# feiyuhuahuo/Yolact_minimal

Measured on AMD Instinct MI355X. Metric: img/s res101_coco 544x544 inference (bs=1/GPU, 4 requests in flight), higher is better.
Workload: dtype f32; 1 GPU; res101_coco 544x544 (the reference's "550-class" size) bs=1 inference: forward + nms + after_nms(480x640) per image, 4 independent bs=1 requests in flight on 4 HIP streams; global_batch=1, parallelism=replicas x1 (inference does not shard), weights=seeded random init, post_inputs=synthetic dense head outputs (17.8k candidates), requests_in_flight=4

## Files before the change

### include/yolact_hip.h

```cpp
#ifndef YOLACT_HIP_H
#define YOLACT_HIP_H

#include <stddef.h>
#include <stdint.h>

#ifdef __cplusplus
extern "C" {
#endif

#define YM_OK 0
#define YM_EINVAL (-1)
#define YM_ENOSPC (-2)
#define YM_ELAUNCH (-3)

#define YM_ACT_NONE 0
#define YM_ACT_RELU 1
#define YM_ACT_TANH 2
#define YM_ACT_GELU 3

typedef void* ym_stream_t;

int ym_abi_version(void);
const char* ym_last_error(void);


int ym_nchw_to_nhwc4(const float* in, float* out, int B, int C, int H, int W, ym_stream_t s);

int ym_pack_conv_weight(const float* w_oihw, float* w_packed, int Cout, int Cin, int KH, int KW,
                        int cin_pad, int k_pad, ym_stream_t s);

int ym_fold_bn(const float* gamma, const float* beta, const float* mean, const float* var, float eps,
               float* scale, float* shift, int C, ym_stream_t s);


typedef struct {
    int n_begin, n_end;
    float* out;
    int64_t batch_stride;
    int32_t pitch;
    int32_t act;
} ym_conv_seg;

typedef struct {
    const float* in;
    const float* weight;
    const float* scale;
    const float* shift;
    const float* residual;
    int32_t B, H, W, Cin, Cout, KH, KW, stride, pad, Ho, Wo, k_pad;
    int32_t nseg;
    ym_conv_seg seg[3];
    int32_t tile_m, tile_n;
    int32_t ksplit;
    int32_t kwaves;
    int32_t transposed;
    int32_t stages;
    double* bn_sum;
    double* bn_sumsq;
    int32_t* tile_counters;
    int32_t nlevels;
    int32_t level_h[5];
    int32_t level_w[5];
    int32_t tail_tiles;
    int32_t tail_ksplit;
    int32_t mma;
    int32_t bnb_relu;
    const float* bnb_y;
    const float* bnb_out;
    const float* bnb_mean;
    const float* bnb_invstd;
    const float* bnb_gamma;
    const float* bnb_beta;
    int32_t grid_wgs;
    int32_t bn_ordered;
} ym_conv_desc;

size_t ym_sizeof_conv_desc(void);
size_t ym_conv2d_workspace_bytes(const ym_conv_desc* d);
int ym_conv2d_tile_counters(const ym_conv_desc* d);
int ym_conv2d_fuses_bn_stats(const ym_conv_desc* d);
int ym_conv2d_effective_plan(const ym_conv_desc* d, int32_t out[8]);
int ym_conv2d_bn_partial_rows(const ym_conv_desc* d);
int ym_bn_partials_finish(const void* part, int rows, int C, void* sums, ym_stream_t s);
int64_t ym_unordered_sum_launches(void);
int ym_conv2d_fwd(const ym_conv_desc* d, void* workspace, size_t workspace_bytes, ym_stream_t s);

size_t ym_layernorm_bwd_workspace_bytes(int C);
int ym_layernorm_bwd(const float* dy, const float* x, const float* gamma, float eps, int64_t M, int C, float* dx, float* dgamma,
                     float* dbeta, void* workspace, size_t workspace_bytes, ym_stream_t s);
int ym_patch_merge_layernorm_bwd(const float* dy, const float* x, int B, int H, int W, int C, const float* gamma, float eps,
                                 float* dx, float* dgamma, float* dbeta, void* workspace, size_t workspace_bytes, ym_stream_t s);
int ym_drop_path_add(const float* res, const float* y, const float* rnd, float keep, float* out, int B, int64_t per_sample,
                     ym_stream_t s);
int ym_drop_path_bwd(const float* dout, const float* rnd, float keep, float* dy, int B, int64_t per_sample, ym_stream_t s);
int ym_gelu_fwd(const float* z, float* out, int64_t n, ym_stream_t s);
int ym_gelu_bwd(const float* dy, const float* z, float* dz, int64_t n, ym_stream_t s);
int ym_swin_window_attention_bwd(const float* qkv, const float* qkv_bias, const float* rel_bias_table, const float* dout, int B,
                                 int H, int W, int C, int heads, int window, int shift, float* dqkv, float* dqkv_bias_pad,
                                 float* dtable, ym_stream_t s);
int ym_adamw_step(float* param, const float* grad, float* exp_avg, float* exp_avg_sq, int64_t n, float lr, float beta1,
                  float beta2, float eps, float weight_decay, int step, ym_stream_t s);

typedef struct {
    int32_t H, W, mirror, cx, cy, cw, ch, q, px, py, r, S, final_mode, fx, fy, has_brightness, has_contrast;
    float brightness, contrast, saturation, hue, mean[3], std[3];
} ym_aug_plan;
int ym_train_aug_image(const void* img_hwc_bgr, int is_u8, const ym_aug_plan* plan, float* out_chw, ym_stream_t s);
int ym_train_aug_masks(const void* masks, int is_u8, const int32_t* keep, int k, const ym_aug_plan* plan, float* out,
                       ym_stream_t s);

size_t ym_mask_iou_workspace_bytes(int n, int g, int64_t P);
int ym_mask_iou(const float* masks_a, int n, const float* masks_b, int g, int64_t P, float* iou, void* workspace,
                size_t workspace_bytes, ym_stream_t s);
int ym_box_iou(const float* boxes_a, int n, const float* boxes_b, int g, float* iou, ym_stream_t s);
int ym_match_detections(const float* iou_box, const float* iou_mask, const int32_t* pred_cls, const int32_t* gt_cls, int n,
                        int g, const double* thresholds, int T, int num_classes, uint8_t* matched, ym_stream_t s);

int ym_rle_encode(const float* masks, int n, int H, int W, uint32_t* counts, int cap_runs, int32_t* nruns, uint8_t* str,
                  int cap_str, int32_t* str_len, void* workspace, size_t workspace_bytes, ym_stream_t s);

size_t ym_ann_to_mask_workspace_bytes(int n, int H, int W);
int ym_poly_to_mask(const double* xy, const int32_t* poly_off, const int32_t* ann_off, int n, int H, int W, uint8_t* masks,
                    void* workspace, size_t workspace_bytes, ym_stream_t s);
int ym_runs_to_mask(const uint32_t* counts, const int32_t* run_off, int n, int H, int W, uint8_t* masks, void* workspace,
                    size_t workspace_bytes, ym_stream_t s);


int ym_pack_conv_weight_dgrad(const float* w_oihw, float* w_packed, int Cout, int Cin, int KH, int KW, int cout_pad,
                              ym_stream_t s);

typedef struct {
    const float* src;
    float* dst;
    int32_t cout, cin, kh, kw, pad_a, pad_b, rows, kind;
    uint32_t first_chunk;
    uint32_t reserved;
} ym_pack_item;
int ym_pack_conv_weights_batch(const ym_pack_item* items_dev, int n_items, int total_chunks, ym_stream_t s);

typedef struct {
    const float* x;
    const float* dy;
    float* dw;
    int32_t B, H, W, Cin, Cin_real, Cout, Cout_real, KH, KW, stride, pad, Ho, Wo;
    int32_t msplit;
    int32_t accumulate;
    int32_t row_end[2];
    float* dw_seg[2];
    int32_t lds_buffers;
} ym_wgrad_desc;
size_t ym_conv2d_wgrad_workspace_bytes(const ym_wgrad_desc* d);
int ym_conv2d_wgrad(const ym_wgrad_desc* d, void* workspace, size_t workspace_bytes, ym_stream_t s);
typedef struct {
    const float* slabs;
    float* dw;
    uint32_t first_block;
    uint32_t blocks;
    uint32_t plan[14];
} ym_wgrad_reduce_item;
int ym_conv2d_wgrad_slabs(const ym_wgrad_desc* d, void* workspace, size_t workspace_bytes, ym_wgrad_reduce_item* item, ym_stream_t s);
int ym_wgrad_reduce_batch(const ym_wgrad_reduce_item* items_dev, int n_items, uint32_t total_blocks, ym_stream_t s);

size_t ym_bn_train_fwd_workspace_bytes(int64_t M, int C);
int ym_bn_train_fwd(const float* y, int64_t M, int C, const float* gamma, const float* beta, float eps, float momentum,
                    float* running_mean, float* running_var, const float* residual, int relu, float* out,
                    float* save_mean, float* save_invstd, void* workspace, size_t workspace_bytes, ym_stream_t s);
int ym_bn_train_fwd_stats(const float* y, int64_t M, int C, const float* gamma, const float* beta, float eps,
                          float momentum, float* running_mean, float* running_var, const float* residual, int relu,
                          float* out, float* save_mean, float* save_invstd, const void* stats, ym_stream_t s);

size_t ym_bn_train_bwd_workspace_bytes(int64_t M, int C);
int ym_bn_train_bwd(const float* dout, const float* out, const float* y, int64_t M, int C, const float* gamma,
                    const float* beta, const float* save_mean, const float* save_invstd, int relu, float* dy, float* dres,
                    float* dgamma, float* dbeta, void* workspace, size_t workspace_bytes, ym_stream_t s);

int ym_bn_train_bwd_apply(const float* dout, const float* out, const float* y, int64_t M, int C, const float* gamma,
                          const float* beta, const float* save_mean, const float* save_invstd, int relu, float* dy, float* dres,
                          float* dgamma, float* dbeta, const void* stats, ym_stream_t s);

int ym_head_grad_gather(const float* dclass, const float* dbox, const float* dcoef, const float* coef, int B, int N, int nc, int cd,
                        int na, int nlev, const int32_t* lev_row, const int32_t* lev_anchor, int pitch, const float* g_scale,
                        float* dz, ym_stream_t s);
int ym_scatter3(const float* src, float* d0, int n0, float* d1, int n1, float* d2, int n2, int accumulate, ym_stream_t s);

int ym_act_bias_bwd(const float* dy, const float* y, int64_t M, int C, int act, float* dz, float* dbias, void* workspace,
                    size_t workspace_bytes, ym_stream_t s);

size_t ym_mask_loss_workspace_bytes(void);
int ym_mask_loss_fwd_bwd(const float* proto, const float* coef_pos, const float* box_pos, const int32_t* gt_idx,
                         const float* gt_masks_ds, const int64_t* anchor_idx, int n, int Hp, int Wp, float wscale, float gscale,
                         double* loss_accum, float* dproto, float* dcoef_full, void* workspace, size_t workspace_bytes,
                         ym_stream_t s);
typedef struct {
    const float* proto;
    const float* coef_full;
    const float* anchor_box;
    const int64_t* anchor_gt;
    const float* gt_masks_ds;
    const int64_t* anchor_idx;
    int32_t n;
    float wscale;
    const int32_t* n_dev;
    float* dproto;
    float* dcoef_full;
} ym_mask_loss_item;
size_t ym_mask_loss_batch_workspace_bytes(int B);
int ym_mask_loss_batch(const ym_mask_loss_item* items, int B, int Hp, int Wp, float gscale, const int32_t* total_pos_dev,
                       double* loss_accum, void* workspace, size_t workspace_bytes, ym_stream_t s);

int ym_match_anchors(const float* gt_boxes_cls, int g, const float* anchors, int N, float pos_thre, float neg_thre,
                     float* offsets, int64_t* conf, float* anchor_box, int64_t* anchor_gt, void* workspace,
                     size_t workspace_bytes, ym_stream_t s);

int ym_match_anchors_batch(const float* const* gt_boxes_cls, const int32_t* g, int B, const float* anchors, int N, float pos_thre,
                           float neg_thre, float* offsets, int64_t* conf, float* anchor_box, int64_t* anchor_gt, void* workspace,
                           size_t workspace_bytes, ym_stream_t s);

size_t ym_loss_workspace_bytes(int B, int N);
int ym_class_box_loss(const float* class_p, const float* box_p, const float* offsets, const int64_t* conf, int B, int N, int C,
                      float conf_alpha, float bbox_alpha, int neg_pos_ratio, float* dclass, float* dbox, int32_t* num_pos,
                      double* loss_c, double* loss_b, void* workspace, size_t workspace_bytes, ym_stream_t s);

int ym_select_positives(const int64_t* conf, const float* keys, int B, int N, int cap, const int32_t* num_pos, int64_t* idx,
                        ym_stream_t s);

int ym_semantic_loss(const float* seg_nhwc, int P, int pitch, int num_classes, const float* gt_masks_ds, const int64_t* gt_cls,
                     int gt_cls_stride, int g, float coeff, float* dseg, double* loss_accum, ym_stream_t s);
int ym_semantic_loss_batch(const float* seg_nhwc, int B, int P, int pitch, int num_classes, const float* const* gt_masks_ds,
                           const int64_t* const* gt_cls, int gt_cls_stride, const int32_t* g, float coeff, float* dseg,
                           double* loss_accum, ym_stream_t s);

int ym_maxpool3x3s2_bwd(const float* x, const float* dy, float* dx, int B, int H, int W, int C, ym_stream_t s);
int ym_maxpool3x3s2_fwd_idx(const float* in, float* out, uint8_t* idx, int B, int H, int W, int C, ym_stream_t s);
int ym_maxpool3x3s2_bwd_idx(const uint8_t* idx, const float* dy, float* dx, int B, int H, int W, int C, ym_stream_t s);
int ym_bilinear2x_bwd(const float* dy, float* dx, int B, int H, int W, int C, int align_corners, ym_stream_t s);

int ym_sgd_step(float* param, const float* grad, float* momentum_buf, int64_t n, float lr, float momentum,
                float weight_decay, int first_step, ym_stream_t s);


int ym_maxpool3x3s2_fwd(const float* in, float* out, int B, int H, int W, int C, ym_stream_t s);
int ym_stem_conv_bn_relu_maxpool(const float* img_nchw, const float* w_packed, const float* scale, const float* shift, float* out,
                                 int B, int H, int W, int k_pad, ym_stream_t s);

int ym_bilinear2x_fwd(const float* in, float* out, int B, int H, int W, int C, int align_corners, ym_stream_t s);

int ym_softmax_rows(const float* in, float* out, int64_t rows, int C, ym_stream_t s);


int ym_layernorm(const float* x, const float* gamma, const float* beta, float eps, float* out, int64_t M, int C,
                 ym_stream_t s);

int ym_patch_merge_layernorm(const float* x, int B, int H, int W, int C, const float* gamma, const float* beta, float eps,
                             float* out, ym_stream_t s);

int ym_swin_window_attention(const float* qkv, const float* qkv_bias, const float* rel_bias_table, int B, int H, int W, int C,
                             int heads, int window, int shift, float* out, ym_stream_t s);


int ym_val_preprocess(const void* img_hwc_bgr, int is_uint8, int H, int W, int S, const float* mean_bgr,
                      const float* std_bgr, float* out_chw_rgb, ym_stream_t s);


typedef struct {
    int32_t num_anchors;
    int32_t num_classes;
    int32_t coef_dim;
    int32_t top_k;
    int32_t max_det;
    float score_thre;
    float iou_thre;
    float img_size;
} ym_nms_cfg;

size_t ym_nms_workspace_bytes(const ym_nms_cfg* cfg);

int ym_detect_fast_nms(const float* class_pred, const float* box_pred, const float* coef_pred,
                       const float* anchors, const ym_nms_cfg* cfg, int32_t* out_count, int64_t* out_ids,
                       float* out_scores, float* out_boxes, float* out_coefs, void* workspace,
                       size_t workspace_bytes, ym_stream_t s);

size_t ym_nms_batch_workspace_bytes(const ym_nms_cfg* cfg, int B);
int ym_detect_fast_nms_batch(const float* class_pred, const float* box_pred, const float* coef_pred, const float* anchors,
                             const ym_nms_cfg* cfg, int B, int32_t* out_count, int64_t* out_ids, float* out_scores,
                             float* out_boxes, float* out_coefs, void* workspace, size_t workspace_bytes, ym_stream_t s);

int ym_detect_greedy_nms(const float* class_pred, const float* box_pred, const float* coef_pred,
                         const float* anchors, const ym_nms_cfg* cfg, int32_t* out_count, int64_t* out_ids,
                         float* out_scores, float* out_boxes, float* out_coefs, void* workspace,
                         size_t workspace_bytes, ym_stream_t s);

size_t ym_greedy_nms_batch_workspace_bytes(const ym_nms_cfg* cfg, int B);
int ym_detect_greedy_nms_batch(const float* class_pred, const float* box_pred, const float* coef_pred, const float* anchors,
                               const ym_nms_cfg* cfg, int B, int32_t* out_count, int64_t* out_ids, float* out_scores,
                               float* out_boxes, float* out_coefs, void* workspace, size_t workspace_bytes, ym_stream_t s);

int ym_expf_cr(const float* x, float* y, int64_t n, ym_stream_t s);

size_t ym_greedy_nms_workspace_bytes(int n);
int ym_greedy_nms(const float* dets, int n, float thresh, uint8_t* keep_mask, int32_t* out_count,
                  void* workspace, size_t workspace_bytes, ym_stream_t s);

int ym_mask_assemble(const float* proto, const float* coefs, const float* boxes, int n, int Hp, int Wp,
                     int K, int do_crop, float* out, ym_stream_t s);

int ym_mask_resize_binarize(const float* masks, int n, int Hp, int Wp, int img_h, int img_w, float* out,
                            ym_stream_t s);

int ym_boxes_to_pixels(float* boxes_f, int32_t* boxes_px, int n, float S, ym_stream_t s);

size_t ym_after_nms_batch_workspace_bytes(int max_det, int Hp, int Wp, int img_h, int img_w);
int ym_after_nms_batch(const float* proto, const float* coefs, float* boxes, const int32_t* counts, int B, int max_det, int Hp,
                       int Wp, int K, int img_h, int img_w, int do_crop, float* masks, int32_t* boxes_px, void* workspace,
                       size_t workspace_bytes, ym_stream_t s);

#define YM_DRAW_HIDE_MASK 1
#define YM_DRAW_HIDE_BBOX 2
#define YM_DRAW_HIDE_SCORE 4
#define YM_DRAW_REAL_TIME 8
#define YM_DRAW_FONT_ADVANCE 12
#define YM_DRAW_FONT_HEIGHT 14
#define YM_DRAW_NAME_STRIDE 40
#define YM_DRAW_LABEL_MAX 44
#define YM_DRAW_MAX_DET 512
size_t ym_draw_workspace_bytes(int B, int max_det);
int ym_draw_detections_batch(const uint8_t* img, const float* masks, const int64_t* ids, const float* scores, const int32_t* boxes_px,
                             const int32_t* counts, int B, int max_det, int H, int W, const uint8_t* palette, int palette_n,
                             int num_classes, const char* names, int num_names, const uint16_t* font, int flags, float visual_thre,
                             const char* fps_text, uint8_t* out, uint8_t* cutout_total, void* workspace, size_t workspace_bytes,
                             ym_stream_t s);

int ym_draw_cutout_objects(const uint8_t* img, const float* masks, int n, int H, int W, uint8_t* out, ym_stream_t s);


int ym_after_nms_batch_packed(const float* proto, const float* coefs, float* boxes, const int32_t* counts, int B, int max_det, int Hp,
                              int Wp, int K, int img_h, int img_w, int do_crop, uint64_t* mask_bits, int32_t* boxes_px,
                              void* workspace, size_t workspace_bytes, ym_stream_t s);
int ym_pack_masks(const void* masks, int is_u8, int n, int H, int W, uint64_t* bits, ym_stream_t s);
int ym_unpack_masks(const uint64_t* bits, int n, int H, int W, float* masks, ym_stream_t s);

#define YM_RAGGED_MAX_IMAGES 32
#define YM_RAGGED_ALIGN_BYTES 256
typedef struct ym_ragged_image {
    int32_t img_h, img_w;
    int64_t offset;
} ym_ragged_image;
size_t ym_after_nms_ragged_workspace_bytes(const ym_ragged_image* images, int B, int max_det, int Hp, int Wp);
int ym_after_nms_ragged(const float* proto, const float* coefs, float* boxes, const int32_t* counts, int B, int max_det, int Hp,
                        int Wp, int K, const ym_ragged_image* images, int do_crop, float* masks, int32_t* boxes_px, void* workspace,
                        size_t workspace_bytes, ym_stream_t s);
int ym_after_nms_ragged_packed(const float* proto, const float* coefs, float* boxes, const int32_t* counts, int B, int max_det, int Hp,
                               int Wp, int K, const ym_ragged_image* images, int do_crop, uint64_t* mask_bits, int32_t* boxes_px,
                               void* workspace, size_t workspace_bytes, ym_stream_t s);

size_t ym_mask_iou_packed_workspace_bytes(int n, int g, int64_t words);
int ym_mask_iou_packed(const uint64_t* bits_a, int n, const uint64_t* bits_b, int g, int64_t words, float* iou, void* workspace,
                       size_t workspace_bytes, ym_stream_t s);
int ym_rle_encode_packed(const uint64_t* bits, int n, int H, int W, uint32_t* counts, int cap_runs, int32_t* nruns, uint8_t* str,
                         int cap_str, int32_t* str_len, void* workspace, size_t workspace_bytes, ym_stream_t s);
int ym_draw_detections_batch_packed(const uint8_t* img, const uint64_t* mask_bits, const int64_t* ids, const float* scores,
                                    const int32_t* boxes_px, const int32_t* counts, int B, int max_det, int H, int W,
                                    const uint8_t* palette, int palette_n, int num_classes, const char* names, int num_names,
                                    const uint16_t* font, int flags, float visual_thre, const char* fps_text, uint8_t* out,
                                    uint8_t* cutout_total, void* workspace, size_t workspace_bytes, ym_stream_t s);
int ym_draw_cutout_objects_packed(const uint8_t* img, const uint64_t* mask_bits, int n, int H, int W, uint8_t* out, ym_stream_t s);

#define YM_EVAL_MAX_DET 1024
#define YM_EVAL_MAX_THRESHOLDS 16
#define YM_EVAL_AP_ROWS_PER_PASS 1024
int ym_eval_match_log(const int64_t* ids, const float* scores, const int32_t* count, int n, const float* iou_box,
                      const float* iou_mask, const float* gt, int g, const double* thresholds, int T, int num_classes,
                      float* log_score, int32_t* log_class, uint32_t* log_flags, int64_t log_offset, int64_t* gt_count,
                      int32_t* class_rows, ym_stream_t s);
size_t ym_eval_ap_workspace_bytes(int64_t rows);
int ym_eval_ap(const uint32_t* log_flags, const int64_t* order, int64_t rows, const int64_t* seg, const int64_t* gt_count, int T,
               int num_classes, double* ap, uint8_t* empty, void* workspace, size_t workspace_bytes, ym_stream_t s);

#define YM_COCO_MAX_GT 512
#define YM_COCO_AREAS 4
#define YM_COCO_WORDS_PER_ROW 8
#define YM_COCO_ROWS_PER_PASS 1024
int ym_coco_iou_box(const double* dt_xywh, int n, const double* gt_xywh, int g, const uint8_t* iscrowd, double* iou, ym_stream_t s);
int ym_coco_iou_mask_packed(const uint64_t* bits_d, int n, const uint64_t* bits_g, int g, int64_t words, const uint8_t* iscrowd,
                            double* iou, int32_t* area_d, ym_stream_t s);
// ... 17 lines not shown
```

### yolact_minimal_amd/csrc/conv_common.h

```cpp
#pragma once
#include <cstdlib>
#include "ym_common.h"

namespace ymk {

constexpr int BK = 32;

struct FastDiv {
    unsigned mg, sh, d;
    __host__ static FastDiv make(unsigned d) {
        if (d == 0) d = 1;
        unsigned s = 0;
        while ((1ull << s) < d) ++s;
        return FastDiv{(unsigned)(((1ull << 32) * ((1ull << s) - d)) / d + 1), s, d};
    }
    __device__ __forceinline__ unsigned div(unsigned x) const { return (__umulhi(x, mg) + x) >> sh; }
    __device__ __forceinline__ void divmod(unsigned x, unsigned& q, unsigned& r) const { q = div(x); r = x - q * d; }
};

typedef int i32x4_t __attribute__((ext_vector_type(4)));
constexpr unsigned OOB = 0xFFFFFFF0u;
__device__ __forceinline__ f32x4 buf_ld16(__amdgpu_buffer_rsrc_t r, unsigned byte_off) {
    return __builtin_bit_cast(f32x4, __builtin_amdgcn_raw_buffer_load_b128(r, (int)byte_off, 0, 0));
}
__device__ __forceinline__ f32x4 buf_ld16_s(__amdgpu_buffer_rsrc_t r, unsigned byte_off, int soffset) {
    return __builtin_bit_cast(f32x4, __builtin_amdgcn_raw_buffer_load_b128(r, (int)byte_off, soffset, 0));
}
template <int I> struct IC { static constexpr int value = I; };
template <int I, int N, class F>
__device__ __forceinline__ void static_for(F&& f) {
    if constexpr (I < N) { f(IC<I>{}); static_for<I + 1, N>(f); }
}
constexpr int AUX_SC1 = 16;
__device__ __forceinline__ f32x4 buf_ld16_sc1(__amdgpu_buffer_rsrc_t r, unsigned byte_off) {
    return __builtin_bit_cast(f32x4, __builtin_amdgcn_raw_buffer_load_b128(r, (int)byte_off, 0, AUX_SC1));
}
__device__ __forceinline__ void buf_st16_sc1(__amdgpu_buffer_rsrc_t r, unsigned byte_off, f32x4 v) {
    __builtin_amdgcn_raw_buffer_store_b128(__builtin_bit_cast(i32x4_t, v), r, (int)byte_off, 0, AUX_SC1);
}

struct SegDev {
    float* out;
    long long bstride;
    int n0, n1, pitch, act;
};

struct ConvP {
    const float* in;
    const float* w;
    const float* scale;
    const float* shift;
    const float* residual;
    float* ws;
    double* bn_sum;
    double* bn_sumsq;
    const float* bnb_y;
    const float* bnb_out;
    const float* bnb_mean;
    const float* bnb_invstd;
    const float* bnb_gamma;
    const float* bnb_beta;
    int bnb_relu;
    int bn_ordered;
    int* counters;
    int B, H, W, Cin, Cout, KH, KW, stride, pad, Ho, Wo, Kpad;
    int M, HoWo, nkt, ksplit, kt_per_split, tiles_m, tiles_n;
    int main_blocks, main_tiles, tail_split, tail_ktps;
    FastDiv fd_ksplit, fd_tail, fd_tiles_n, fd_howo, fd_wo, fd_cin, fd_kw;
    int nlev;
    int lev_h[5], lev_w[5], lev_m[6], lev_pix[6];
    int cls;
    int M_pix;
    int cls_tile0[5];
    int cls_rows[4];
    int cls_w[4];
    FastDiv cls_fd_hw[4], cls_fd_w[4];
    int cls_kh0[4], cls_kw0[4], cls_nkw[4];
    int cls_nkt[4], cls_ktps[4], cls_tail_ktps[4];
    int n_groups;
    FastDiv fd_grp, fd_gn, fd_gn_last;
    long long* trace;
    const int* trace_epoch;
    int trace_ring;
    int trace_stride;
    int trace_rt;
    int* trace_hw;
    unsigned in_bytes, w_bytes, ws_bytes;
    int total_items;
    int nseg;
    int vec;
    SegDev seg[3];
};

__device__ __forceinline__ void ym_tile_decode(const ConvP& p, int id, int& tile_m, int& tile_n) {
    const unsigned g = p.fd_grp.div((unsigned)id);
    const unsigned r = (unsigned)id - g * p.fd_grp.d;
    const bool last = (int)g == p.n_groups - 1;
    const unsigned w = last ? p.fd_gn_last.d : p.fd_gn.d;
    const unsigned tm = last ? p.fd_gn_last.div(r) : p.fd_gn.div(r);
    tile_m = (int)tm;
    tile_n = (int)(g * p.fd_gn.d + (r - tm * w));
}

inline void ym_set_tile_order(ConvP& p, int groups, bool allow_model) {
    const int tn = p.tiles_n > 0 ? p.tiles_n : 1, tm = p.tiles_m > 0 ? p.tiles_m : 1;
    static const char* env = getenv("YM_TILE_GROUPS");
    if (groups <= 0) {
        const double a = (double)p.in_bytes, w = (double)p.w_bytes;
        if (env && env[0] == 'l') groups = (allow_model && w > a) ? tn : 1;
        else if (env && atoi(env) > 0) groups = allow_model ? atoi(env) : 1;
        else {
            groups = 1;
            double best = a + 8.0 * w;
            const bool small = a + w <= 8.0 * 1024 * 1024;
            if (allow_model && !small && w > a) groups = tn;
            for (int g = 2; g <= 8 && allow_model && small; g *= 2) {
                if (tn < g) break;
                const double t = g * a + (8.0 / g) * w;
                if (t < 0.95 * best) { best = t; groups = g; }
            }
        }
    }
    if (groups > tn) groups = tn;
    const int gw = (tn + groups - 1) / groups;
    p.n_groups = (tn + gw - 1) / gw;
    p.fd_gn = FastDiv::make((unsigned)gw);
    p.fd_gn_last = FastDiv::make((unsigned)(tn - (p.n_groups - 1) * gw));
    p.fd_grp = FastDiv::make((unsigned)(tm * gw));
}

#ifdef YM_TRACE
__device__ __forceinline__ size_t ym_trace_region(const ConvP& p) {
    if (!p.trace_epoch) return 0;
    const unsigned e = (unsigned)__hip_atomic_load(p.trace_epoch, __ATOMIC_RELAXED, __HIP_MEMORY_SCOPE_AGENT);
    return (size_t)(e % (unsigned)p.trace_ring) * (p.trace_stride ? (unsigned)p.trace_stride : gridDim.x);
}
#define YM_STAMP(i) do { if ((i) == 3) __builtin_amdgcn_s_waitcnt(0); if (p.trace && threadIdx.x == 0) { const size_t reg_ = ym_trace_region(p); p.trace[(reg_ + blockIdx.x) * 4 + (i)] = (long long)((p.trace_epoch || p.trace_rt) ? __builtin_amdgcn_s_memrealtime() : __builtin_amdgcn_s_memtime()) | ((i) == 0 ? (long long)(__builtin_amdgcn_s_getreg(0x1814) & 15) << 60 : 0ll); if ((i) == 0 && p.trace_hw) p.trace_hw[reg_ + blockIdx.x] = (int)__builtin_amdgcn_s_getreg(0xF804); } } while (0)
#else
#define YM_STAMP(i) do { } while (0)
#endif


__device__ __forceinline__ void row_to_image_pixel(const ConvP& p, int m, int& b, int& pix) {
    if (p.nlev > 0) {
        int base = 0, hw = p.lev_h[0] * p.lev_w[0], pix0 = 0;
#pragma unroll
        for (int q = 1; q < 5; ++q)
            if (q < p.nlev && m >= p.lev_m[q]) { base = p.lev_m[q]; hw = p.lev_h[q] * p.lev_w[q]; pix0 = p.lev_pix[q]; }
        const int local = m - base;
        b = local / hw;
        pix = pix0 + (local - b * hw);
    } else {
        b = (int)p.fd_howo.div((unsigned)m);
        pix = m - b * p.HoWo;
    }
}

__device__ __forceinline__ void epilogue_store(const ConvP& p, int m, int n, float acc) {
    float v = acc;
    v = __builtin_fmaf(v, p.scale ? p.scale[n] : 1.f, p.shift ? p.shift[n] : 0.f);
    if (p.residual) v += p.residual[(size_t)m * p.Cout + n];
    int b, pix;
    row_to_image_pixel(p, m, b, pix);
#pragma unroll
    for (int s = 0; s < 3; ++s) {
        if (s < p.nseg && n >= p.seg[s].n0 && n < p.seg[s].n1) {
            const SegDev& g = p.seg[s];
            g.out[(size_t)b * g.bstride + (size_t)pix * g.pitch + (n - g.n0)] = ym_apply_act(v, g.act);
        }
    }
}


enum ConvFamily { CONV_IGEMM, CONV_WAVE, CONV_WAVE_DMA, CONV_WS, CONV_PERS };
struct Plan {
    int bm, bn, ksplit, kt_per_split, tiles_m, tiles_n, nkt, M;
    int tail_tiles, tail_split, tail_ktps;
    int cls, M_pix, cls_tile0[5], cls_rows[4], cls_w[4], cls_hw[4], cls_kh0[4], cls_kw0[4], cls_nkw[4], cls_nkt[4];
    int kwaves;
    int family;
    int ring = 2;
    int mode = 0, spl = 0;
    bool dl = false, pf = false, pyramid = false;
    int grid_wgs;
    int pers_grid;
    bool pers_defer;
    bool vec, counters, fuses_bn;
    int bn_rows;
    int slots() const { return tail_tiles > 0 && tail_split > ksplit ? tail_split : ksplit; }
    size_t ws_bytes(int cout) const {
        const size_t u = ksplit > 1 ? (size_t)ksplit * M * cout * sizeof(float) : 0;
        const size_t t = tail_tiles > 0 ? (size_t)tail_tiles * tail_split * bm * bn * sizeof(float) : 0;
        return u > t ? u : t;
    }
    int grid() const { return (tiles_m * tiles_n - tail_tiles) * ksplit + tail_tiles * (tail_tiles > 0 ? tail_split : 0); }
    int stages() const {
        return ring + (family == CONV_PERS ? 40 : family == CONV_WS ? 50 : family == CONV_WAVE_DMA ? 20 : dl ? (pf ? 30 : 20) : 0);
    }
};

}

int ym_conv_plan(const ym_conv_desc* d, bool ws_aligned, ymk::Plan* pl);
int ym_cu_count();
int ym_launch_conv_wave(const ymk::ConvP& p, int tm, int tn, int kwaves, int ring, int waves_per_block, hipStream_t st);
int ym_launch_conv_pers(const ymk::ConvP& p, int bm, int bn, int mode, int ns, bool defer, int grid, hipStream_t st);
size_t ym_conv_pers_lds_bytes(int bm, int bn, int ns, bool defer);
int ym_launch_conv_ws(const ymk::ConvP& p, int bm, int bn, int nstg, int grid_wgs, hipStream_t st);
int ym_conv_ws_partial_rows(int M, int Cout, int bm, int bn, int nkt, int nstg, int grid_wgs);
size_t ym_conv_ws_lds_bytes(int bm, int bn, int nkt, int nstg);
```

### yolact_minimal_amd/csrc/conv_mfma.hip

```cpp
#include <stdlib.h>
#include <type_traits>
#include "conv_common.h"

using namespace ymk;

namespace {

constexpr int PITCH = 36;

template <int BM, int BN, int MODE, int NS, bool DL = false, bool PF = false, bool RG = false, int SPL = 0>
__global__ __launch_bounds__(256) void conv_igemm_f32(const ConvP p) {
    static_assert(SPL == 0 || (SPL <= 3 && !DL && !PF && (NS == 2 || NS == 3) && MODE != 1), "split-bf16: register staging, Cin % 32 == 0");
    constexpr int LB = SPL ? 2 : NS;
    constexpr int TM = BM / 64, TN = BN / 64;
    constexpr int AR = BM / 32, BR = BN / 32;
    constexpr int BP = 40;
    constexpr int RP = SPL ? (SPL * BP) / 2 : (DL ? 32 : PITCH);
    extern __shared__ __attribute__((aligned(16))) float smem[];
    float* As = smem;
    float* Bs = smem + LB * BM * RP;

    const int tid = threadIdx.x;
    const int lane = tid & 63, wave = __builtin_amdgcn_readfirstlane(tid >> 6);
    const int wm = wave >> 1, wn = wave & 1;
// ... 513 lines not shown
                        const f32x4 v = *reinterpret_cast<const f32x4*>(C + row * CP + col4 * 4);
                        if (fused) buf_st16_sc1(rs_ws, base + (unsigned)row * rs, v);
                        else *reinterpret_cast<f32x4*>(p.ws + (size_t)ks * slice + n + (size_t)m * p.Cout) = v;
                    }
                }
            }
            if (!fused) return;
            int& s_last = *reinterpret_cast<int*>(smem);
            asm volatile("s_waitcnt vmcnt(0)" ::: "memory");
            __syncthreads();
            if (tid == 0) {
                int* cnt = p.counters + tile_m * p.tiles_n + tile_n;
                const int old = __hip_atomic_fetch_add(cnt, 1, __ATOMIC_RELAXED, __HIP_MEMORY_SCOPE_AGENT);
                s_last = old == nks - 1;
                if (s_last) __hip_atomic_store(cnt, 0, __ATOMIC_RELAXED, __HIP_MEMORY_SCOPE_AGENT);
            }
            __syncthreads();
            if (!s_last) { YM_STAMP(3); return; }
        }
        if (n < p.Cout) {
            f32x4 sc = pre_sc, sh = pre_sh;
            if (!direct) {
                if (p.scale) sc = *reinterpret_cast<const f32x4*>(p.scale + n);
                if (p.shift) sh = *reinterpret_cast<const f32x4*>(p.shift + n);
            }
            const int act = p.seg[0].act;
            float* outb = p.seg[0].out + n;
            const bool fwd_stats = p.bn_sum != nullptr && p.bnb_y == nullptr;
            const float* resb = (p.residual && !(direct && PRE_RES)) ? p.residual + n : nullptr;
#pragma unroll
            for (int rk = 0; rk < BM / RPP; ++rk) {
                const int row = row0 + rk * RPP;
                const int m = out_row(row);
                if (m >= 0) {
                    f32x4 v;
                    if (nks > 1) {
                        const unsigned off = ws0 + (unsigned)row * rs;
                        v = buf_ld16_sc1(rs_ws, off);
                        int s2 = 1;
                        for (; s2 + 3 < nks; s2 += 4) {
                            const f32x4 a = buf_ld16_sc1(rs_ws, off + (unsigned)s2 * sb), b = buf_ld16_sc1(rs_ws, off + (unsigned)(s2 + 1) * sb);
                            const f32x4 c = buf_ld16_sc1(rs_ws, off + (unsigned)(s2 + 2) * sb), d = buf_ld16_sc1(rs_ws, off + (unsigned)(s2 + 3) * sb);
                            v += a; v += b; v += c; v += d;
                        }
                        for (; s2 < nks; ++s2) v += buf_ld16_sc1(rs_ws, off + (unsigned)s2 * sb);
                    } else if (epi_abl) {
                        v = f32x4{acc[0][0][(4 * rk) & 15], acc[0][0][(4 * rk + 1) & 15], acc[0][0][(4 * rk + 2) & 15], acc[0][0][(4 * rk + 3) & 15]};
                    } else {
                        v = *reinterpret_cast<const f32x4*>(C + row * CP + col4 * 4);
                    }
                    v = __builtin_elementwise_fma(v, sc, sh);
                    if (direct && PRE_RES) v += pre_res[PRE_RES ? rk : 0];
                    else if (resb) v += *reinterpret_cast<const f32x4*>(resb + (size_t)m * p.Cout);
#pragma unroll
                    for (int e = 0; e < 4; ++e) v[e] = ym_apply_act(v[e], act);
                    *reinterpret_cast<f32x4*>(outb + (size_t)m * p.Cout) = v;
                    if (fwd_stats) {
#pragma unroll
                        for (int e = 0; e < 4; ++e) { const double dv = v[e]; bsum[e] += dv; bsq[e] += dv * dv; }
                    }
                }
            }
            if (p.bnb_y) {
                const f32x4 b_mu = *reinterpret_cast<const f32x4*>(p.bnb_mean + n), b_is = *reinterpret_cast<const f32x4*>(p.bnb_invstd + n);
                f32x4 b_g = {1.f, 1.f, 1.f, 1.f}, b_bt = {0.f, 0.f, 0.f, 0.f};
                const bool remask = p.bnb_relu && !p.bnb_out;
                if (remask) { b_g = *reinterpret_cast<const f32x4*>(p.bnb_gamma + n); b_bt = *reinterpret_cast<const f32x4*>(p.bnb_beta + n); }
                constexpr int NR = BM / RPP, UR = 2;
#pragma unroll 1
                for (int rk0 = 0; rk0 < NR; rk0 += UR) {
                    f32x4 dv[UR], yy[UR], o[UR];
                    int mrow[UR];
#pragma unroll
                    for (int u = 0; u < UR; ++u) {
                        const int m = mrow[u] = out_row(row0 + (rk0 + u) * RPP);
                        const size_t off = (size_t)(m >= 0 ? m : 0) * p.Cout + n;
                        dv[u] = *reinterpret_cast<const f32x4*>(p.seg[0].out + off);
                        yy[u] = *reinterpret_cast<const f32x4*>(p.bnb_y + off);
                        if (p.bnb_out) o[u] = *reinterpret_cast<const f32x4*>(p.bnb_out + off);
                    }
#pragma unroll
                    for (int u = 0; u < UR; ++u) {
                        if (mrow[u] < 0) continue;
                        if (!p.bnb_out) {
#pragma unroll
                            for (int e = 0; e < 4; ++e) o[u][e] = remask ? bn_affine(yy[u][e], b_mu[e], b_is[e], b_g[e], b_bt[e]) : 1.f;
                        }
#pragma unroll
                        for (int e = 0; e < 4; ++e) {
                            const double dd = o[u][e] > 0.f ? dv[u][e] : 0.f;
                            bsum[e] += dd;
                            bsq[e] += dd * (double)((yy[u][e] - b_mu[e]) * b_is[e]);
                        }
                    }
                }
            }
        }
        if (p.bn_sum) {
            __syncthreads();
            double* R = reinterpret_cast<double*>(smem);
#pragma unroll
            for (int e = 0; e < 4; ++e) {
                R[((row0 * BN) + col4 * 4 + e) * 2 + 0] = bsum[e];
                R[((row0 * BN) + col4 * 4 + e) * 2 + 1] = bsq[e];
            }
            __syncthreads();
            if (tid < BN && n0 + tid < p.Cout) {
                double S = 0.0, Q = 0.0;
#pragma unroll
                for (int r = 0; r < RPP; ++r) { S += R[(r * BN + tid) * 2]; Q += R[(r * BN + tid) * 2 + 1]; }
                if (p.bn_ordered) {
                    double* row = p.bn_sum + (size_t)tile_m * 2 * p.Cout;
                    row[n0 + tid] = S;
                    row[p.Cout + n0 + tid] = Q;
                } else {
                    atomicAdd(p.bn_sum + n0 + tid, S);
                    atomicAdd(p.bn_sumsq + n0 + tid, Q);
                }
            }
        }
        YM_STAMP(3);
        return;
    }
    int* rowinfo = reinterpret_cast<int*>(smem);
    __syncthreads();
    if (tid < BM) {
        int b = 0, pix = 0;
        if (m0 + tid < p.M) row_to_image_pixel(p, m0 + tid, b, pix);
        rowinfo[2 * tid] = b;
        rowinfo[2 * tid + 1] = pix;
    }
    __syncthreads();
#pragma unroll
    for (int j = 0; j < TN; ++j) {
        const int n = n0 + wn * (BN / 2) + j * 32 + frag_row;
        const bool n_ok = n < p.Cout;
        float sc = 1.f, sh = 0.f;
        float* optr = nullptr;
        long long obs = 0;
        int opitch = 0, oact = 0;
        if (n_ok) {
            if (p.scale) sc = p.scale[n];
            if (p.shift) sh = p.shift[n];
#pragma unroll
            for (int s = 0; s < 3; ++s) {
                if (s < p.nseg && n >= p.seg[s].n0 && n < p.seg[s].n1) {
                    optr = p.seg[s].out + (n - p.seg[s].n0);
                    obs = p.seg[s].bstride; opitch = p.seg[s].pitch; oact = p.seg[s].act;
                }
            }
        }
#pragma unroll
        for (int i = 0; i < TM; ++i) {
            const int mb = m0 + wm * (BM / 2) + i * 32 + 4 * khalf;
            if (p.ksplit > 1) {
#pragma unroll
                for (int r = 0; r < 16; ++r) {
                    const int m = mb + (r & 3) + 8 * (r >> 2);
                    if (n_ok && m < p.M) p.ws[((size_t)ks * p.M + m) * p.Cout + n] = acc[i][j][r];
                }
            } else if (optr) {
#pragma unroll
                for (int r = 0; r < 16; ++r) {
                    const int m = mb + (r & 3) + 8 * (r >> 2);
                    if (m < p.M) {
                        float v = __builtin_fmaf(acc[i][j][r], sc, sh);
                        if (p.residual) v += p.residual[(size_t)m * p.Cout + n];
                        const int row = m - m0;
                        optr[(size_t)rowinfo[2 * row] * obs + (size_t)rowinfo[2 * row + 1] * opitch] = ym_apply_act(v, oact);
                    }
                }
            }
            __builtin_amdgcn_sched_barrier(0);
        }
    }
}

__global__ __launch_bounds__(256) void conv_splitk_reduce(const ConvP p) {
    const size_t total = (size_t)p.M * p.Cout;
    if (p.vec) {
        const size_t total4 = total / 4;
        const int act = p.seg[0].act;
        for (size_t q = (size_t)blockIdx.x * 256 + threadIdx.x; q < total4; q += (size_t)gridDim.x * 256) {
            const size_t e = q * 4;
            f32x4 v = *reinterpret_cast<const f32x4*>(p.ws + e);
            for (int s = 1; s < p.ksplit; ++s) v += *reinterpret_cast<const f32x4*>(p.ws + (size_t)s * total + e);
            const int n = (int)(e % p.Cout);
            f32x4 sc = {1.f, 1.f, 1.f, 1.f}, sh = {0.f, 0.f, 0.f, 0.f};
            if (p.scale) sc = *reinterpret_cast<const f32x4*>(p.scale + n);
            if (p.shift) sh = *reinterpret_cast<const f32x4*>(p.shift + n);
            v = __builtin_elementwise_fma(v, sc, sh);
            if (p.residual) v += *reinterpret_cast<const f32x4*>(p.residual + e);
#pragma unroll
            for (int k = 0; k < 4; ++k) v[k] = ym_apply_act(v[k], act);
            *reinterpret_cast<f32x4*>(p.seg[0].out + e) = v;
        }
        return;
    }
    for (size_t e = (size_t)blockIdx.x * 256 + threadIdx.x; e < total; e += (size_t)gridDim.x * 256) {
        float v = 0.f;
        for (int s = 0; s < p.ksplit; ++s) v += p.ws[(size_t)s * total + e];
        const int m = (int)(e / p.Cout), n = (int)(e - (size_t)m * p.Cout);
        epilogue_store(p, m, n, v);
    }
}

template <int BM, int BN, int MODE, int NS = 2, bool DL = false, bool PF = false, bool RG = false, int SPL = 0>
void launch(const ConvP& p, int grid, hipStream_t st) {
    size_t lds = SPL ? (size_t)2 * (BM + BN) * SPL * 80 : (size_t)NS * (BM + BN) * (DL ? 32 : PITCH) * sizeof(float);
    const size_t epi = (size_t)BM * (BN + 4) * sizeof(float);
    if (lds < epi) lds = epi;
    static YmLdsAttr attr = {};
    (void)ym_ensure_dyn_lds(attr, reinterpret_cast<const void*>(conv_igemm_f32<BM, BN, MODE, NS, DL, PF, RG, SPL>), lds, "conv_igemm_f32");
    hipLaunchKernelGGL((conv_igemm_f32<BM, BN, MODE, NS, DL, PF, RG, SPL>), dim3(grid), dim3(256), lds, st, p);
}

bool launch_igemm(const ConvP& p, const Plan& pl, int grid, hipStream_t st) {
#define YM_V(BM_, BN_, MODE_, NS_, DL_, PF_, RG_, SPL_)                                                                               \
    if (pl.bm == BM_ && pl.bn == BN_ && pl.mode == MODE_ && pl.ring == NS_ && pl.dl == DL_ && pl.pf == PF_ && pl.pyramid == RG_ && \
        pl.spl == SPL_) { launch<BM_, BN_, MODE_, NS_, DL_, PF_, RG_, SPL_>(p, grid, st); return true; }
    YM_V(128, 128, 0, 2, 0, 0, 0, 0)
    YM_V(128, 128, 0, 2, 1, 0, 0, 0)
    YM_V(128, 128, 0, 3, 1, 0, 0, 0)
    YM_V(128,  64, 0, 2, 0, 0, 0, 0)
    YM_V(128,  64, 0, 3, 0, 0, 0, 0)
    YM_V(128,  64, 0, 2, 1, 0, 0, 0)
    YM_V(128,  64, 0, 3, 1, 0, 0, 0)
    YM_V( 64, 128, 0, 2, 0, 0, 0, 0)
    YM_V( 64, 128, 0, 3, 0, 0, 0, 0)
    YM_V( 64, 128, 0, 2, 1, 0, 0, 0)
    YM_V( 64, 128, 0, 3, 1, 0, 0, 0)
    YM_V( 64,  64, 0, 2, 0, 0, 0, 0)
    YM_V( 64,  64, 0, 3, 0, 0, 0, 0)
    YM_V( 64,  64, 0, 2, 1, 0, 0, 0)
    YM_V( 64,  64, 0, 3, 1, 0, 0, 0)
    YM_V( 64,  64, 0, 4, 1, 0, 0, 0)
    YM_V( 64,  64, 0, 3, 1, 1, 0, 0)
    YM_V( 64,  64, 0, 4, 1, 1, 0, 0)
    YM_V(128, 128, 2, 2, 0, 0, 0, 0)
    YM_V(128, 128, 2, 2, 1, 0, 0, 0)
    YM_V(128, 128, 2, 3, 1, 0, 0, 0)
    YM_V(128,  64, 2, 2, 0, 0, 0, 0)
    YM_V(128,  64, 2, 2, 1, 0, 0, 0)
    YM_V(128,  64, 2, 3, 1, 0, 0, 0)
    YM_V( 64, 128, 2, 2, 0, 0, 0, 0)
    YM_V( 64, 128, 2, 2, 1, 0, 0, 0)
    YM_V( 64, 128, 2, 3, 1, 0, 0, 0)
    YM_V( 64,  64, 2, 2, 0, 0, 0, 0)
    YM_V( 64,  64, 2, 3, 0, 0, 0, 0)
    YM_V( 64,  64, 2, 2, 1, 0, 0, 0)
    YM_V( 64,  64, 2, 3, 1, 0, 0, 0)
    YM_V(128,  64, 1, 2, 0, 0, 0, 0)
    YM_V(128, 128, 0, 2, 0, 0, 1, 0)
    YM_V(128,  64, 0, 2, 0, 0, 1, 0)
    YM_V( 64, 128, 0, 2, 0, 0, 1, 0)
    YM_V( 64,  64, 0, 2, 0, 0, 1, 0)
    YM_V(128, 128, 0, 2, 0, 0, 0, 2)
    YM_V(128, 128, 0, 3, 0, 0, 0, 2)
    YM_V(128,  64, 0, 2, 0, 0, 0, 2)
    YM_V(128,  64, 0, 3, 0, 0, 0, 2)
    YM_V( 64, 128, 0, 2, 0, 0, 0, 2)
    YM_V( 64, 128, 0, 3, 0, 0, 0, 2)
    YM_V( 64,  64, 0, 2, 0, 0, 0, 2)
    YM_V( 64,  64, 0, 3, 0, 0, 0, 2)
    YM_V(128, 128, 0, 2, 0, 0, 0, 3)
    YM_V(128, 128, 0, 3, 0, 0, 0, 3)
    YM_V(128,  64, 0, 2, 0, 0, 0, 3)
    YM_V(128,  64, 0, 3, 0, 0, 0, 3)
    YM_V( 64, 128, 0, 2, 0, 0, 0, 3)
    YM_V( 64, 128, 0, 3, 0, 0, 0, 3)
    YM_V( 64,  64, 0, 2, 0, 0, 0, 3)
    YM_V( 64,  64, 0, 3, 0, 0, 0, 3)
    YM_V(128, 128, 2, 2, 0, 0, 0, 2)
    YM_V(128, 128, 2, 3, 0, 0, 0, 2)
    YM_V(128,  64, 2, 2, 0, 0, 0, 2)
    YM_V(128,  64, 2, 3, 0, 0, 0, 2)
    YM_V( 64, 128, 2, 2, 0, 0, 0, 2)
    YM_V( 64, 128, 2, 3, 0, 0, 0, 2)
    YM_V( 64,  64, 2, 2, 0, 0, 0, 2)
    YM_V( 64,  64, 2, 3, 0, 0, 0, 2)
    YM_V(128, 128, 2, 2, 0, 0, 0, 3)
    YM_V(128, 128, 2, 3, 0, 0, 0, 3)
    YM_V(128,  64, 2, 2, 0, 0, 0, 3)
    YM_V(128,  64, 2, 3, 0, 0, 0, 3)
    YM_V( 64, 128, 2, 2, 0, 0, 0, 3)
    YM_V( 64, 128, 2, 3, 0, 0, 0, 3)
    YM_V( 64,  64, 2, 2, 0, 0, 0, 3)
    YM_V( 64,  64, 2, 3, 0, 0, 0, 3)
#undef YM_V
    return false;
}

int fill_params(const ym_conv_desc* d, const Plan& pl, void* workspace, ConvP& p) {
    const size_t need = pl.ws_bytes(d->Cout);
    p.in = d->in; p.w = d->weight; p.scale = d->scale; p.shift = d->shift; p.residual = d->residual;
    p.ws = (float*)workspace;
    p.B = d->B; p.H = d->H; p.W = d->W; p.Cin = d->Cin; p.Cout = d->Cout; p.KH = d->KH; p.KW = d->KW;
    p.stride = d->stride; p.pad = d->pad; p.Ho = d->Ho; p.Wo = d->Wo; p.Kpad = d->k_pad;
    {
        const unsigned long long ib = (d->nlevels ? (unsigned long long)pl.M : (unsigned long long)d->B * d->H * d->W) * d->Cin * 4ull, wb = (unsigned long long)d->Cout * d->k_pad * 4ull;
        YM_REQUIRE(ib < 0xFFFFFFF0ull && wb < 0x7FFFFFF0ull, "conv: input must be < 4 GiB and the packed weight < 2 GiB (32-bit buffer offsets)");
        p.in_bytes = (unsigned)ib; p.w_bytes = (unsigned)wb;
    }
    p.nlev = d->nlevels;
    {
        int m_acc = 0, pix_acc = 0;
        for (int l = 0; l < 5; ++l) {
            const bool on = l < d->nlevels;
            p.lev_h[l] = on ? d->level_h[l] : 1; p.lev_w[l] = on ? d->level_w[l] : 1;
            p.lev_m[l] = m_acc; p.lev_pix[l] = pix_acc;
            if (on) { m_acc += d->B * d->level_h[l] * d->level_w[l]; pix_acc += d->level_h[l] * d->level_w[l]; }
        }
        p.lev_m[5] = m_acc; p.lev_pix[5] = pix_acc;
    }
    p.M = pl.M; p.HoWo = d->Ho * d->Wo; p.nkt = pl.nkt; p.ksplit = pl.ksplit; p.kt_per_split = pl.kt_per_split;
    p.M_pix = pl.M_pix; p.cls = pl.cls;
    for (int c = 0; c < 4; ++c) {
        const bool on = pl.cls != 0;
        p.cls_tile0[c] = on ? pl.cls_tile0[c] : 0; p.cls_rows[c] = on ? pl.cls_rows[c] : 0; p.cls_w[c] = on ? pl.cls_w[c] : 1;
        p.cls_fd_hw[c] = FastDiv::make((unsigned)(on ? pl.cls_hw[c] : 1)); p.cls_fd_w[c] = FastDiv::make((unsigned)(on ? pl.cls_w[c] : 1));
        p.cls_kh0[c] = on ? pl.cls_kh0[c] : 0; p.cls_kw0[c] = on ? pl.cls_kw0[c] : 0; p.cls_nkw[c] = on ? pl.cls_nkw[c] : 1;
        p.cls_nkt[c] = on ? pl.cls_nkt[c] : 0;
        p.cls_ktps[c] = on ? ym_cdiv(pl.cls_nkt[c], pl.ksplit) : 0;
        p.cls_tail_ktps[c] = on && pl.tail_tiles > 0 ? ym_cdiv(pl.cls_nkt[c], pl.tail_split) : 0;
    }
    p.cls_tile0[4] = pl.cls ? pl.cls_tile0[4] : 0;
    p.tiles_m = pl.tiles_m; p.tiles_n = pl.tiles_n; p.nseg = d->nseg;
    for (int i = 0; i < 3; ++i) {
        if (i < d->nseg) {
            p.seg[i].out = d->seg[i].out; p.seg[i].bstride = d->seg[i].batch_stride; p.seg[i].n0 = d->seg[i].n_begin;
            p.seg[i].n1 = d->seg[i].n_end; p.seg[i].pitch = d->seg[i].pitch; p.seg[i].act = d->seg[i].act;
        } else {
            p.seg[i] = SegDev{nullptr, 0, 0, 0, 0, 0};
        }
    }
    YM_REQUIRE(pl.tail_tiles == 0 || ((uintptr_t)workspace & 15) == 0, "conv: tail split needs a 16-byte aligned workspace");
    p.vec = pl.vec;
    p.bn_sum = d->bn_sum; p.bn_sumsq = d->bn_sumsq; p.bn_ordered = (d->bn_sum && d->bn_ordered) ? 1 : 0;
    p.bnb_y = d->bnb_y; p.bnb_out = d->bnb_out; p.bnb_mean = d->bnb_mean; p.bnb_invstd = d->bnb_invstd;
    p.bnb_gamma = d->bnb_gamma; p.bnb_beta = d->bnb_beta; p.bnb_relu = d->bnb_relu;
    p.trace = nullptr; p.trace_epoch = nullptr; p.trace_ring = 0; p.trace_stride = 0; p.trace_rt = 0; p.trace_hw = nullptr;
#ifdef YM_TRACE
    if (const char* e = getenv("YM_TRACE_PTR")) p.trace = (long long*)strtoull(e, nullptr, 10);
    if (const char* e = getenv("YM_TRACE_EPOCH_PTR")) p.trace_epoch = (const int*)strtoull(e, nullptr, 10);
    if (const char* e = getenv("YM_TRACE_RING")) p.trace_ring = atoi(e);
    if (const char* e = getenv("YM_TRACE_GRID")) p.trace_stride = atoi(e);
    if (const char* e = getenv("YM_TRACE_REALTIME")) p.trace_rt = atoi(e);
    if (const char* e = getenv("YM_TRACE_HW_PTR")) p.trace_hw = (int*)strtoull(e, nullptr, 10);
    if (p.trace_ring <= 0) p.trace_epoch = nullptr;
    if (const char* e = getenv("YM_PERS_ABL")) { if (!d->bn_sum) p.bnb_relu = atoi(e); }
#endif
    p.counters = pl.counters ? d->tile_counters : nullptr;
    YM_REQUIRE(!pl.cls || (p.vec && (pl.slots() == 1 || p.counters)), "conv(dgrad, stride 2): the class-ordered plan needs a 16-byte aligned workspace");
    YM_REQUIRE(pl.tail_tiles == 0 || p.counters, "conv: tail_tiles needs a plain NHWC output (vector epilogue) and a workspace < 4 GiB");
    p.main_tiles = pl.tiles_m * pl.tiles_n - pl.tail_tiles;
    p.main_blocks = p.main_tiles * pl.ksplit;
    p.tail_split = pl.tail_tiles > 0 ? pl.tail_split : 1;
    p.tail_ktps = pl.tail_tiles > 0 ? pl.tail_ktps : pl.nkt;
    p.fd_ksplit = FastDiv::make((unsigned)pl.ksplit); p.fd_tail = FastDiv::make((unsigned)p.tail_split);
    p.fd_tiles_n = FastDiv::make((unsigned)pl.tiles_n);
    ym_set_tile_order(p, 0, pl.tail_tiles == 0);
    p.fd_howo = FastDiv::make((unsigned)(d->Ho * d->Wo));
    p.fd_wo = FastDiv::make((unsigned)d->Wo); p.fd_cin = FastDiv::make((unsigned)d->Cin); p.fd_kw = FastDiv::make((unsigned)d->KW);
    p.ws_bytes = (unsigned)(need < 0xFFFFFFF0ull ? need : 0);
    p.total_items = pl.grid();
    if (d->bn_sum) {
        YM_REQUIRE((d->bn_sumsq || d->bn_ordered) && ((uintptr_t)d->bn_sum & 7) == 0 && pl.fuses_bn,
                   "conv: bn_sum given but this configuration cannot fuse the statistics (ask ym_conv2d_fuses_bn_stats)");
    }
    if (d->bnb_y) {
        YM_REQUIRE(d->bn_sum && d->bnb_mean && d->bnb_invstd && (!d->bnb_relu || d->bnb_out || (d->bnb_gamma && d->bnb_beta)),
                   "conv: bnb_y needs bn_sum / bn_sumsq, bnb_mean, bnb_invstd and (with bnb_relu) bnb_out or bnb_gamma + bnb_beta");
        YM_REQUIRE(d->Cout % 4 == 0 && ((uintptr_t)d->bnb_y & 15) == 0 && ((uintptr_t)d->bnb_out & 15) == 0,
                   "conv: bnb_y / bnb_out must be 16-byte aligned [M][Cout] tensors");
    }
    YM_REQUIRE(pl.family != CONV_WAVE_DMA || (size_t)pl.M * d->Cout * 4 < 0xFFFFFFF0ull, "conv(wave, DMA ring): the output must be < 4 GiB");
    if (pl.family == CONV_IGEMM && d->mma != 0) {
        YM_REQUIRE(d->mma == 3 || d->mma == 6, "conv: mma must be 0 (f32 MFMA), 3 (bf16x3) or 6 (bf16x6), got %d", d->mma);
        YM_REQUIRE(d->nlevels == 0 && d->Cin % 32 == 0, "conv: split-bf16 mode needs Cin %% 32 == 0 and a single-size input");
    }
    return YM_OK;
}

int launch_plan(const ConvP& p, const Plan& pl, hipStream_t st) {
    switch (pl.family) {
        case CONV_WAVE: case CONV_WAVE_DMA: return ym_launch_conv_wave(p, pl.bm, pl.bn, pl.kwaves, pl.ring, pl.grid_wgs, st);
        case CONV_WS: return ym_launch_conv_ws(p, pl.bm, pl.bn, pl.ring, pl.grid_wgs, st);
        case CONV_PERS: return ym_launch_conv_pers(p, pl.bm, pl.bn, pl.mode, pl.ring, pl.pers_defer, pl.pers_grid, st);
    }
    if (!launch_igemm(p, pl, pl.grid(), st)) {
        ym_set_error("conv: no conv_igemm_f32<%d, %d, %d, %d, %d, %d, %d, %d> is built (planner bug)", pl.bm, pl.bn, pl.mode, pl.ring, pl.dl, pl.pf, pl.pyramid, pl.spl);
        return YM_EINVAL;
    }
    int rc = ym_check_launch("conv_igemm_f32");
    if (rc == YM_OK && pl.ksplit > 1 && !p.counters) {
        const size_t total = (size_t)p.M * p.Cout;
        int rgrid = (int)((total / (p.vec ? 4 : 1) + 255) / 256);
        if (rgrid > 2048) rgrid = 2048;
        hipLaunchKernelGGL(conv_splitk_reduce, dim3(rgrid), dim3(256), 0, st, p);
        rc = ym_check_launch("conv_splitk_reduce");
    }
    return rc;
}

}

extern "C" size_t ym_sizeof_conv_desc(void) { return sizeof(ym_conv_desc); }

extern "C" size_t ym_conv2d_workspace_bytes(const ym_conv_desc* d) {
    Plan pl;
    return ym_conv_plan(d, true, &pl) == YM_OK ? pl.ws_bytes(d->Cout) : 0;
}

extern "C" int ym_conv2d_tile_counters(const ym_conv_desc* d) {
    Plan pl;
    return ym_conv_plan(d, true, &pl) == YM_OK && pl.slots() > 1 ? pl.tiles_m * pl.tiles_n : 0;
}

extern "C" int ym_conv2d_fuses_bn_stats(const ym_conv_desc* d) {
    Plan pl;
    return ym_conv_plan(d, true, &pl) == YM_OK && pl.fuses_bn ? 1 : 0;
}

extern "C" int ym_conv2d_bn_partial_rows(const ym_conv_desc* d) {
    Plan pl;
    return ym_conv_plan(d, true, &pl) == YM_OK ? pl.bn_rows : 0;
}

extern "C" int ym_conv2d_effective_plan(const ym_conv_desc* d, int32_t out[8]) {
    Plan pl;
    YM_REQUIRE(out, "conv: effective_plan needs an output row");
    if (int rc = ym_conv_plan(d, true, &pl)) return rc;
    const bool tail = pl.tail_tiles > 0;
    const int32_t row[8] = {pl.bm, pl.bn, pl.ksplit, d->kwaves, pl.stages(), tail ? pl.tail_tiles : 0, tail ? pl.tail_split : 0, pl.grid_wgs};
    for (int i = 0; i < 8; ++i) out[i] = row[i];
    return YM_OK;
}

extern "C" int ym_conv2d_fwd(const ym_conv_desc* d, void* workspace, size_t workspace_bytes, ym_stream_t s) {
    Plan pl;
    if (int rc = ym_conv_plan(d, ((uintptr_t)workspace & 15) == 0, &pl)) return rc;
    const size_t need = pl.ws_bytes(d->Cout);
    if (need > workspace_bytes || (need && !workspace)) {
        ym_set_error("conv: workspace %zu B < %zu B needed (ksplit %d)", workspace_bytes, need, pl.ksplit);
        return YM_ENOSPC;
    }
    ConvP p;
    if (int rc = fill_params(d, pl, workspace, p)) return rc;
    if (d->bn_sum && !d->bn_ordered) ym_note_unordered_sum();
    return launch_plan(p, pl, (hipStream_t)s);
}
```

### yolact_minimal_amd/csrc/conv_planner.hip

```cpp
#include <stdlib.h>
#include "conv_common.h"

using namespace ymk;

int ym_cu_count() {
    static int cus = 0;
    if (cus == 0) {
        int dev = 0, n = 0;
        if (hipGetDevice(&dev) != hipSuccess || hipDeviceGetAttribute(&n, hipDeviceAttributeMultiprocessorCount, dev) != hipSuccess || n <= 0) n = 256;
        cus = n;
    }
    return cus;
}

namespace {

bool vec_epilogue(const ym_conv_desc* d) {
    const ym_conv_seg& g = d->seg[0];
    const bool aligned = (((uintptr_t)g.out | (uintptr_t)d->residual | (uintptr_t)d->scale | (uintptr_t)d->shift) & 15) == 0;
    const bool rows_in_order = d->nlevels ? g.batch_stride == 0
                                          : g.batch_stride == (int64_t)d->Ho * d->Wo * d->Cout;
    return d->nseg == 1 && g.n_begin == 0 && g.n_end == d->Cout && g.pitch == d->Cout && rows_in_order && d->Cout % 4 == 0 && aligned;
}

int plan_tiles(const ym_conv_desc* d, Plan* pl, bool allow_cls) {
    YM_REQUIRE(d && d->in && d->weight, "conv: null descriptor / pointer");
    YM_REQUIRE(d->B > 0 && d->H > 0 && d->W > 0 && d->Cout > 0, "conv: bad shape");
    YM_REQUIRE(d->Cin == 4 || d->Cin % 32 == 0, "conv: Cin must be 4 (stem) or a multiple of 32, got %d", d->Cin);
    YM_REQUIRE(d->k_pad % BK == 0 && d->k_pad >= d->KH * d->KW * d->Cin, "conv: k_pad %d invalid", d->k_pad);
    if (d->transposed) {
        YM_REQUIRE(d->stride == 1 || d->stride == 2, "conv(dgrad): stride must be 1 or 2");
        YM_REQUIRE(d->Cin % 32 == 0 && d->kwaves == 0, "conv(dgrad): dy channels must be padded to a multiple of 32; workgroup kernel only");
        YM_REQUIRE(d->H == (d->Ho + 2 * d->pad - d->KH) / d->stride + 1 && d->W == (d->Wo + 2 * d->pad - d->KW) / d->stride + 1,
                   "conv(dgrad): H/W (dy) inconsistent with Ho/Wo (dx)");
    } else if (d->nlevels == 0) {
        YM_REQUIRE(d->Ho == (d->H + 2 * d->pad - d->KH) / d->stride + 1 && d->Wo == (d->W + 2 * d->pad - d->KW) / d->stride + 1,
                   "conv: Ho/Wo inconsistent with H/W/K/stride/pad");
    }
    long long M_levels = 0;
    if (d->nlevels != 0) {
        YM_REQUIRE(d->nlevels >= 1 && d->nlevels <= 5, "conv: nlevels must be 0..5");
        YM_REQUIRE(!d->transposed && d->kwaves == 0 && d->Cin % 32 == 0 && d->stride == 1 && d->KH == d->KW && (d->KH & 1) &&
                   d->pad == d->KH / 2, "conv(pyramid): stride 1, odd square filter, pad = K/2, Cin %% 32 == 0, workgroup kernel");
        for (int l = 0; l < d->nlevels; ++l) {
            YM_REQUIRE(d->level_h[l] > 0 && d->level_w[l] > 0, "conv(pyramid): bad level %d", l);
            M_levels += (long long)d->B * d->level_h[l] * d->level_w[l];
        }
    }
    YM_REQUIRE(d->nseg >= 1 && d->nseg <= 3, "conv: nseg must be 1..3");
    for (int s = 0; s < d->nseg; ++s)
        YM_REQUIRE(d->seg[s].out && d->seg[s].n_end > d->seg[s].n_begin && d->seg[s].n_end <= d->Cout,
                   "conv: bad segment %d", s);
    const long long M = d->nlevels ? M_levels : (long long)d->B * d->Ho * d->Wo;
    YM_REQUIRE(M * (long long)d->Cout < (1ll << 31) && (d->nlevels ? M : (long long)d->B * d->H * d->W) * d->Cin < (1ll << 31) * 1ll,
               "conv: tensor too large for 32-bit indexing");
    pl->M = (int)M;
    pl->M_pix = (int)M;
    pl->cls = 0;
    pl->nkt = d->k_pad / BK;
    pl->tail_tiles = 0; pl->tail_split = 0; pl->tail_ktps = 0;
    int bm = d->tile_m, bn = d->tile_n;
    if (bm == 0 || bn == 0) {
        const int cand[3][2] = {{128, 128}, {128, 64}, {64, 64}};
        bm = 64; bn = 64;
        for (int c = 0; c < 3; ++c) {
            const long long wgs = (long long)ym_cdiv(pl->M, cand[c][0]) * ym_cdiv(d->Cout, cand[c][1]);
            if (wgs >= 512) { bm = cand[c][0]; bn = cand[c][1]; break; }
        }
        if (d->Cin == 4) { bm = 128; bn = 64; }
    }
    pl->family = CONV_IGEMM;
    if (d->stages >= 52 && d->stages <= 54) {
        const bool shape_ok = (bm == 64 && bn == 256) || (bm == 128 && bn == 128) || (bm == 256 && bn == 64);
        const int act = d->seg[0].act;
        const bool ok = shape_ok && d->KH == 1 && d->KW == 1 && d->stride == 1 && d->pad == 0 && d->Cin % 32 == 0 && d->k_pad == d->Cin &&
                        d->nlevels == 0 && d->kwaves == 0 && d->mma == 0 && d->bnb_y == nullptr && vec_epilogue(d) &&
                        (act == YM_ACT_NONE || act == YM_ACT_RELU) && (size_t)bn * d->Cin * 4 <= (64u << 10) &&
                        ym_conv_ws_lds_bytes(bm, bn, pl->nkt, d->stages - 50) <= (160u << 10) && (unsigned long long)M * d->Cout * 4ull < 0xFFFFFFF0ull &&
                        (unsigned long long)M * d->Cin * 4ull < 0xFFFFFFF0ull;
        if (ok) {
            pl->bm = bm; pl->bn = bn; pl->tiles_m = ym_cdiv(pl->M, bm); pl->tiles_n = ym_cdiv(d->Cout, bn);
            pl->ksplit = 1; pl->kt_per_split = pl->nkt;
            pl->family = CONV_WS; pl->ring = d->stages - 50;
            return YM_OK;
        }
        bm = 64; bn = 64;
    }
    if (d->kwaves > 0) {
        YM_REQUIRE(d->Cin != 4, "conv: the wave-private kernel does not support the stem (Cin == 4)");
        YM_REQUIRE((bm == 32 || bm == 64) && (bn == 32 || bn == 64), "conv(wave): tile must be 32/64, got %dx%d", bm, bn);
        const bool dma = d->stages >= 22 && d->stages <= 24;
        pl->family = dma ? CONV_WAVE_DMA : CONV_WAVE;
        pl->ring = dma ? d->stages - 20 : 0;
        pl->bm = bm; pl->bn = bn; pl->tiles_m = ym_cdiv(pl->M, bm); pl->tiles_n = ym_cdiv(d->Cout, bn);
        pl->ksplit = 1; pl->kt_per_split = pl->nkt;
        if (d->tail_tiles > 0 && d->tail_ksplit > 1 && dma && bm == 32 && bn == 32 && d->kwaves == 4 &&
            (d->grid_wgs == 0 || d->grid_wgs == 4) && d->tile_counters && vec_epilogue(d)) {
            YM_REQUIRE(d->tail_tiles <= pl->tiles_m * pl->tiles_n, "conv(wave): tail_tiles %d > %d output tiles", d->tail_tiles, pl->tiles_m * pl->tiles_n);
            int ts = d->tail_ksplit > pl->nkt ? pl->nkt : d->tail_ksplit;
            if (ts > 8) ts = 8;
            pl->tail_ktps = ym_cdiv(pl->nkt, ts);
            pl->tail_split = ym_cdiv(pl->nkt, pl->tail_ktps);
            pl->tail_tiles = pl->tail_split > 1 ? d->tail_tiles : 0;
        }
        return YM_OK;
    }
    YM_REQUIRE((bm == 128 || bm == 64) && (bn == 128 || bn == 64), "conv: tile must be 64/128");
    YM_REQUIRE(d->Cin != 4 || (bm == 128 && bn == 64), "conv: stem mode supports the 128x64 tile only");
    pl->bm = bm; pl->bn = bn;
    {
        static int on = -1;
        if (on < 0) { const char* e = getenv("YM_DGRAD_CLASSES"); on = e ? atoi(e) : 1; }
        if (on && allow_cls && d->transposed && d->stride == 2 && d->nlevels == 0 && vec_epilogue(d)) {
            int t0 = 0, nkt_max = 0, nt_max = 0;
            for (int c = 0; c < 4; ++c) {
                const int ph = c >> 1, pw = c & 1;
                const int hc = (d->Ho - ph + 1) / 2, wc = (d->Wo - pw + 1) / 2;
                const int kh0 = (ph + d->pad) & 1, kw0 = (pw + d->pad) & 1;
                const int nkh = kh0 < d->KH ? (d->KH - kh0 + 1) / 2 : 0, nkw = kw0 < d->KW ? (d->KW - kw0 + 1) / 2 : 0;
                pl->cls_tile0[c] = t0;
                pl->cls_rows[c] = d->B * hc * wc;
                pl->cls_w[c] = wc > 0 ? wc : 1;
                pl->cls_hw[c] = hc * wc > 0 ? hc * wc : 1;
                pl->cls_kh0[c] = kh0; pl->cls_kw0[c] = kw0; pl->cls_nkw[c] = nkw > 0 ? nkw : 1;
                pl->cls_nkt[c] = nkh * nkw * (d->Cin / BK);
                if (pl->cls_nkt[c] > nkt_max) nkt_max = pl->cls_nkt[c];
                t0 += ym_cdiv(pl->cls_rows[c], bm);
                if (ym_cdiv(pl->cls_rows[c], bm) > nt_max) nt_max = ym_cdiv(pl->cls_rows[c], bm);
            }
            pl->cls_tile0[4] = t0;
            pl->cls = 1;
            pl->M = 4 * nt_max * bm;
            pl->nkt = nkt_max > 0 ? nkt_max : 1;
        }
    }
    pl->tiles_m = ym_cdiv(pl->M, bm);
    pl->tiles_n = ym_cdiv(d->Cout, bn);
    int ks = d->ksplit;
    if (ks <= 0) {
        ks = 1;
        const int wgs = pl->tiles_m * pl->tiles_n;
        if (wgs < 256) {
            ks = ym_cdiv(512, wgs);
            const int max_ks = pl->nkt / 4 > 0 ? pl->nkt / 4 : 1;
            if (ks > max_ks) ks = max_ks;
            if (ks > 16) ks = 16;
        }
    }
    if (ks > pl->nkt) ks = pl->nkt;
    if (ks < 1) ks = 1;
    pl->kt_per_split = ym_cdiv(pl->nkt, ks);
    pl->ksplit = ym_cdiv(pl->nkt, pl->kt_per_split);
    if (d->tail_tiles > 0 && d->tail_ksplit > 1 && vec_epilogue(d)) {
        YM_REQUIRE(d->tile_counters && pl->ksplit == 1 && d->Cin != 4, "conv: tail_tiles needs tile_counters, ksplit <= 1 and Cin %% 32 == 0");
        YM_REQUIRE(d->tail_tiles <= pl->tiles_m * pl->tiles_n, "conv: tail_tiles %d > %d output tiles", d->tail_tiles, pl->tiles_m * pl->tiles_n);
        int ts = d->tail_ksplit > pl->nkt ? pl->nkt : d->tail_ksplit;
        pl->tail_ktps = ym_cdiv(pl->nkt, ts);
        pl->tail_split = ym_cdiv(pl->nkt, pl->tail_ktps);
        pl->tail_tiles = pl->tail_split > 1 ? d->tail_tiles : 0;
    }
    if (pl->cls && pl->slots() > 1 && (!d->tile_counters || pl->ws_bytes(d->Cout) >= 0xFFFFFFF0ull)) return plan_tiles(d, pl, false);
    return YM_OK;
}

void plan_variant(const ym_conv_desc* d, Plan* pl) {
    const bool t64 = pl->bm == 64 && pl->bn == 64;
    const int act = d->seg[0].act;
    int stages = d->stages;
    if (stages >= 52 && stages <= 54) stages = 22;
    if (stages >= 42 && stages <= 48) {
        const int ns = stages - 40;
        if (pl->vec && t64 && d->Cin % 32 == 0 && d->nlevels == 0 && d->mma == 0 && !pl->cls && (act == YM_ACT_NONE || act == YM_ACT_RELU) &&
            (pl->slots() == 1 || pl->counters) && d->bn_sum == nullptr && (ns == 2 || ns == 3 || ns == 4 || ns == 6 || ns == 8)) {
            static int defer = -1;
            if (defer < 0) { const char* e = getenv("YM_PERS_DEFER"); defer = e ? atoi(e) : 1; }
            int per_cu = (int)((160u << 10) / ym_conv_pers_lds_bytes(64, 64, ns, defer != 0));
            if (per_cu > 4) per_cu = 4;
            if (per_cu < 1) per_cu = 1;
            int g = d->grid_wgs > 0 ? d->grid_wgs : ym_cu_count() * per_cu;
            if (g > pl->grid()) g = pl->grid();
            if (g >= 8 && g < pl->grid()) g &= ~7;
            pl->family = CONV_PERS; pl->ring = ns; pl->pers_grid = g; pl->pers_defer = defer != 0;
            pl->mode = d->transposed ? 2 : 0;
            return;
        }
        stages = ns >= 4 && t64 && !d->transposed ? 24 : (ns == 2 ? 22 : 23);
    }
    pl->mode = d->transposed ? 2 : (d->Cin == 4 ? 1 : 0);
    pl->pyramid = d->nlevels > 0;
    if (d->mma != 0) {
        pl->spl = d->mma == 3 ? 2 : 3;
        pl->ring = stages == 3 ? 3 : 2;
    } else if (!pl->pyramid && pl->mode != 1) {
        const bool has3 = pl->mode == 0 ? !(pl->bm == 128 && pl->bn == 128) : t64;
        if (pl->mode == 0 && t64 && (stages == 24 || stages == 33 || stages == 34)) { pl->dl = true; pl->pf = stages > 30; pl->ring = stages % 10; }
        else if (stages == 22 || stages == 23) { pl->dl = true; pl->ring = stages - 20; }
        else if (stages == 3 && has3) pl->ring = 3;
    }
}

}

int ym_conv_plan(const ym_conv_desc* d, bool ws_aligned, Plan* pl) {
    *pl = Plan{};
    if (int rc = plan_tiles(d, pl, true)) return rc;
    pl->kwaves = d->kwaves;
    pl->vec = vec_epilogue(d) && ws_aligned;
    pl->counters = pl->vec && pl->slots() > 1 && (d->kwaves == 0 || pl->tail_tiles > 0) && pl->ws_bytes(d->Cout) < 0xFFFFFFF0ull && d->tile_counters;
    pl->fuses_bn = pl->vec && (pl->slots() == 1 || pl->counters) && d->kwaves == 0;
    if (pl->family == CONV_IGEMM) plan_variant(d, pl);
    pl->grid_wgs = pl->family == CONV_IGEMM || pl->family == CONV_WAVE ? 0 : d->grid_wgs;
    pl->bn_rows = !pl->fuses_bn ? 0 : pl->family != CONV_WS ? pl->tiles_m
                : ym_conv_ws_partial_rows(pl->M, d->Cout, pl->bm, pl->bn, pl->nkt, pl->ring, d->grid_wgs);
    return YM_OK;
}
```

### yolact_minimal_amd/csrc/conv_wave.hip

```cpp
#include "conv_common.h"

using namespace ymk;

namespace {

constexpr int waitcnt_vm(int vm) { return (vm & 15) | ((vm >> 4) << 14) | (7 << 4) | (15 << 8); }

template <int N>
struct Frag {
    f32x4 v[N][4];
};

template <int TM, int TN, int KW, int WPB>
__device__ __forceinline__ void wave_tile_finish(const ConvP& p, float* slabs, f32x16 (&acc)[TM][TN], int wave, int lane, bool tile_ok,
                                                 int tile_local, int kslice, int m0, int n0) {
    constexpr int WM = 32 * TM, WN = 32 * TN;
    constexpr int CP = WN + 4;
    const int frag_row = lane & 31, khalf = lane >> 5;
    constexpr int C4_ = WN / 4, LANES_ = KW * 64, NPASS = (WM * C4_ + LANES_ - 1) / LANES_;
    f32x4 pre_res[NPASS];
    const bool pre = p.vec && p.residual != nullptr && tile_ok;
    if (pre) {
        const int lt_ = kslice * 64 + lane, col4_ = lt_ % C4_, row0_ = lt_ / C4_;
        const __amdgpu_buffer_rsrc_t rs_res = __builtin_amdgcn_make_buffer_rsrc((void*)p.residual, 0, (unsigned)((size_t)p.M * p.Cout * 4), 0x00020000);
#pragma unroll
        for (int k = 0; k < NPASS; ++k) {
            const int m = m0 + row0_ + k * (LANES_ / C4_), n = n0 + col4_ * 4;
            pre_res[k] = buf_ld16(rs_res, (row0_ + k * (LANES_ / C4_) < WM && m < p.M && n < p.Cout) ? (unsigned)(((size_t)m * p.Cout + n) * 4) : OOB);
        }
    }
    float* mine = slabs + (size_t)wave * WM * CP;
#pragma unroll
    for (int j = 0; j < TN; ++j)
#pragma unroll
        for (int i = 0; i < TM; ++i)
#pragma unroll
            for (int r = 0; r < 16; ++r)
                mine[(i * 32 + 4 * khalf + (r & 3) + 8 * (r >> 2)) * CP + j * 32 + frag_row] = acc[i][j][r];
    __syncthreads();
    if (!tile_ok) return;
    const float* slab0 = slabs + (size_t)(tile_local * KW) * WM * CP;
    constexpr int C4 = WN / 4;
    constexpr int LANES = KW * 64;
    const int lt = kslice * 64 + lane;
    if (p.vec) {
        const int col4 = lt % C4, row0 = lt / C4;
        const int n = n0 + col4 * 4;
        if (n < p.Cout) {
            f32x4 sc = {1.f, 1.f, 1.f, 1.f}, sh = {0.f, 0.f, 0.f, 0.f};
            if (p.scale) sc = *reinterpret_cast<const f32x4*>(p.scale + n);
            if (p.shift) sh = *reinterpret_cast<const f32x4*>(p.shift + n);
            const int act = p.seg[0].act;
#pragma unroll
            for (int k = 0; k < NPASS; ++k) {
                const int row = row0 + k * (LANES / C4);
                const int m = m0 + row;
                if (row >= WM || m >= p.M) break;
                f32x4 v = *reinterpret_cast<const f32x4*>(slab0 + row * CP + col4 * 4);
#pragma unroll
                for (int s = 1; s < KW; ++s) v += *reinterpret_cast<const f32x4*>(slab0 + (size_t)s * WM * CP + row * CP + col4 * 4);
                v = __builtin_elementwise_fma(v, sc, sh);
                if (p.residual) v += pre_res[k];
#pragma unroll
                for (int e = 0; e < 4; ++e) v[e] = ym_apply_act(v[e], act);
                *reinterpret_cast<f32x4*>(p.seg[0].out + (size_t)m * p.Cout + n) = v;
            }
        }
    } else {
        for (int e = lt; e < WM * WN; e += LANES) {
            const int row = e / WN, col = e - row * WN;
            const int m = m0 + row, n = n0 + col;
            if (m < p.M && n < p.Cout) {
                float v = slab0[row * CP + col];
#pragma unroll
                for (int s = 1; s < KW; ++s) v += slab0[(size_t)s * WM * CP + row * CP + col];
                epilogue_store(p, m, n, v);
            }
        }
    }
}

template <int TM, int TN, int KW, int WPB>
__global__ __launch_bounds__(WPB * 64) void conv_wave_f32(const ConvP p) {
    constexpr int TPB = WPB / KW;
    constexpr int WM = 32 * TM, WN = 32 * TN;
    constexpr int D = 3;
    extern __shared__ __attribute__((aligned(16))) float smem[];

    const int lane = threadIdx.x & 63;
    const int wave = __builtin_amdgcn_readfirstlane(threadIdx.x >> 6);
    const int tile_local = wave / KW, kslice = wave - tile_local * KW;
    const int frag_row = lane & 31, khalf = lane >> 5;

    const int bid = ym_xcd_remap(blockIdx.x, gridDim.x);
    const int tile = bid * TPB + tile_local;
    const int ntiles = p.tiles_m * p.tiles_n;
    const bool tile_ok = tile < ntiles;
    const int tile_m = tile_ok ? tile / p.tiles_n : 0, tile_n = tile_ok ? tile - tile_m * p.tiles_n : 0;
    const int m0 = tile_m * WM, n0 = tile_n * WN;

    int a_pix[TM], a_ih0[TM], a_iw0[TM];
#pragma unroll
    for (int i = 0; i < TM; ++i) {
        const int m = m0 + i * 32 + frag_row;
        if (tile_ok && m < p.M) {
            const int b = m / p.HoWo, rem = m - b * p.HoWo;
            const int oh = rem / p.Wo, ow = rem - oh * p.Wo;
            a_ih0[i] = oh * p.stride - p.pad;
            a_iw0[i] = ow * p.stride - p.pad;
            a_pix[i] = (b * p.H + a_ih0[i]) * p.W + a_iw0[i];
        } else {
            a_ih0[i] = -(1 << 20); a_iw0[i] = -(1 << 20); a_pix[i] = 0;
        }
    }
    const float* wrow[TN];
#pragma unroll
    for (int j = 0; j < TN; ++j) {
        const int n = n0 + j * 32 + frag_row;
        wrow[j] = (tile_ok && n < p.Cout) ? p.w + (size_t)n * p.Kpad + khalf * 4 : nullptr;
    }

    const int nt = tile_ok ? (p.nkt - kslice + KW - 1) / KW : 0;
    int kh, kw, c0;
    {
        const int k0 = kslice * BK;
        const int tap = k0 / p.Cin;
        c0 = k0 - tap * p.Cin;
        kh = tap / p.KW;
        kw = tap - kh * p.KW;
    }
    int kt_next = kslice;

    Frag<TM> fa[D];
    Frag<TN> fb[D];
    auto load_tile = [&](Frag<TM>& A, Frag<TN>& Bf) {
        const int tap_off = kh * p.W + kw;
#pragma unroll
        for (int i = 0; i < TM; ++i) {
            const int ih = a_ih0[i] + kh, iw = a_iw0[i] + kw;
            const bool ok = (unsigned)ih < (unsigned)p.H && (unsigned)iw < (unsigned)p.W;
            if (ok) {
                const float* src = p.in + (size_t)(a_pix[i] + tap_off) * p.Cin + c0 + khalf * 4;
#pragma unroll
                for (int g = 0; g < 4; ++g) A.v[i][g] = *reinterpret_cast<const f32x4*>(src + g * 8);
            } else {
#pragma unroll
                for (int g = 0; g < 4; ++g) A.v[i][g] = f32x4{0.f, 0.f, 0.f, 0.f};
            }
        }
#pragma unroll
        for (int j = 0; j < TN; ++j) {
            if (wrow[j]) {
                const float* src = wrow[j] + (size_t)kt_next * BK;
#pragma unroll
                for (int g = 0; g < 4; ++g) Bf.v[j][g] = *reinterpret_cast<const f32x4*>(src + g * 8);
            } else {
#pragma unroll
                for (int g = 0; g < 4; ++g) Bf.v[j][g] = f32x4{0.f, 0.f, 0.f, 0.f};
            }
        }
        kt_next += KW;
        c0 += BK * KW;
        while (c0 >= p.Cin) {
            c0 -= p.Cin;
            if (++kw == p.KW) { kw = 0; ++kh; }
        }
    };

    f32x16 acc[TM][TN];
#pragma unroll
    for (int i = 0; i < TM; ++i)
#pragma unroll
        for (int j = 0; j < TN; ++j)
#pragma unroll
            for (int r = 0; r < 16; ++r) acc[i][j][r] = 0.f;

    auto compute = [&](const Frag<TM>& A, const Frag<TN>& Bf) {
#pragma unroll
        for (int g = 0; g < 4; ++g)
#pragma unroll
            for (int s = 0; s < 4; ++s)
#pragma unroll
                for (int i = 0; i < TM; ++i)
#pragma unroll
                    for (int j = 0; j < TN; ++j)
                        acc[i][j] = __builtin_amdgcn_mfma_f32_32x32x2f32(A.v[i][g][s], Bf.v[j][g][s], acc[i][j], 0, 0, 0);
    };

#pragma unroll
    for (int s = 0; s < D - 1; ++s)
        if (s < nt) load_tile(fa[s], fb[s]);
    for (int t = 0; t < nt; t += D) {
#pragma unroll
        for (int u = 0; u < D; ++u) {
            if (t + u < nt) {
                if (t + u + D - 1 < nt) load_tile(fa[(u + D - 1) % D], fb[(u + D - 1) % D]);
                compute(fa[u], fb[u]);
            }
        }
    }

    wave_tile_finish<TM, TN, KW, WPB>(p, smem, acc, wave, lane, tile_ok, tile_local, kslice, m0, n0);
}

template <int TM, int TN, int KW, int NS, int WPB = 4>
__global__ __launch_bounds__(WPB * 64) void conv_wdma_f32(const ConvP p) {
    static_assert(WPB % KW == 0 && WPB <= 4, "the K waves of a tile share a workgroup");
    constexpr int TPB = WPB / KW;
    constexpr int WM = 32 * TM, WN = 32 * TN;
    constexpr int AR = 4 * TM, BR = 4 * TN;
    constexpr int RP = 32;
    constexpr int STAGE = (WM + WN) * RP;
    constexpr int D = NS - 1;
    static_assert(NS >= 2 && NS <= 4 && (AR + BR) * D < 64, "ring depth / vmcnt field");
    static_assert((size_t)STAGE >= (size_t)WM * (WN + 4), "the finished tile is staged in the wave's first ring stage");
    extern __shared__ __attribute__((aligned(16))) float smem[];

    const int lane = threadIdx.x & 63;
    const int wave = __builtin_amdgcn_readfirstlane(threadIdx.x >> 6);
    const int tile_local = wave / KW, kslice = wave - tile_local * KW;
    const int frag_row = lane & 31, khalf = lane >> 5;
    YM_STAMP(0);
    constexpr bool TAIL = TM * TN == 1 && KW == 4 && WPB == 4;
    const bool in_tail = TAIL && (int)blockIdx.x >= p.main_blocks;
    int tile, tslice = 0, tsplit = 1;
    if (in_tail) {
        unsigned q, r;
        p.fd_tail.divmod(blockIdx.x - (unsigned)p.main_blocks, q, r);
        tile = p.main_tiles + (int)q; tslice = (int)r; tsplit = p.tail_split;
    } else {
        tile = ym_xcd_remap(blockIdx.x, TAIL ? p.main_blocks : (int)gridDim.x) * TPB + tile_local;
    }
    const bool tile_ok = tile < p.tiles_m * p.tiles_n;
    int tile_m = 0, tile_n = 0;
    if (tile_ok) ym_tile_decode(p, tile, tile_m, tile_n);
    const int m0 = tile_m * WM, n0 = tile_n * WN;
    const __amdgpu_buffer_rsrc_t rs_in = __builtin_amdgcn_make_buffer_rsrc((void*)p.in, 0, p.in_bytes, 0x00020000);
    const __amdgpu_buffer_rsrc_t rs_w = __builtin_amdgcn_make_buffer_rsrc((void*)p.w, 0, p.w_bytes, 0x00020000);

    const int drow = lane >> 3;
    int a_pix[AR], a_ih0[AR], a_iw0[AR];
    unsigned a_off[AR], wrow[BR];
#pragma unroll
    for (int i = 0; i < AR; ++i) {
        const int m = m0 + 8 * i + drow;
        if (tile_ok && m < p.M) {
            unsigned ub, urem, uoh, uow;
            p.fd_howo.divmod((unsigned)m, ub, urem);
            p.fd_wo.divmod(urem, uoh, uow);
            a_ih0[i] = (int)uoh * p.stride - p.pad;
            a_iw0[i] = (int)uow * p.stride - p.pad;
            a_pix[i] = ((int)ub * p.H + a_ih0[i]) * p.W + a_iw0[i];
        } else {
            a_ih0[i] = -(1 << 20); a_iw0[i] = -(1 << 20); a_pix[i] = 0;
        }
    }
#pragma unroll
    for (int j = 0; j < BR; ++j) {
        const int n = n0 + 8 * j + drow;
        const int c4 = (lane & 7) ^ ((4 * j + (lane >> 4)) & 7);
        wrow[j] = (tile_ok && n < p.Cout) ? (unsigned)((n * p.Kpad + c4 * 4) * 4) : p.w_bytes;
    }

    const int k_lo = in_tail ? tslice * p.tail_ktps : 0, k_hi = in_tail ? min(p.nkt, k_lo + p.tail_ktps) : p.nkt;
    const int per = (k_hi - k_lo + KW - 1) / KW;
    const int kt_beg = k_lo + kslice * per, kt_end = tile_ok ? min(k_hi, kt_beg + per) : kt_beg;
    const int nt = max(0, kt_end - kt_beg);
    int kh, kw, c0;
    {
        unsigned tap, uc0, ukh, ukw;
        p.fd_cin.divmod((unsigned)(kt_beg * BK), tap, uc0);
        p.fd_kw.divmod(tap, ukh, ukw);
        c0 = (int)uc0; kh = (int)ukh; kw = (int)ukw;
    }
    bool tap_dirty = true;
    int ld_kt = kt_beg;
    float* ring = smem + (size_t)wave * NS * STAGE;

    auto dma_next = [&](int stage) __attribute__((always_inline)) {
        typedef __attribute__((address_space(3))) void* lds_ptr;
        if (tap_dirty) {
            tap_dirty = false;
#pragma unroll
            for (int i = 0; i < AR; ++i) {
                const int ih = a_ih0[i] + kh, iw = a_iw0[i] + kw;
                const bool ok = (unsigned)ih < (unsigned)p.H && (unsigned)iw < (unsigned)p.W;
                const int c4 = (lane & 7) ^ ((4 * i + (lane >> 4)) & 7);
                a_off[i] = (unsigned)(((a_pix[i] + kh * p.W + kw) * p.Cin + c4 * 4) * 4) | (ok ? 0u : OOB);
            }
        }
        float* a = ring + stage * STAGE;
        float* b = a + WM * RP;
        const int soff_a = c0 * 4, soff_b = ld_kt * BK * 4;
#pragma unroll
        for (int i = 0; i < AR; ++i)
            __builtin_amdgcn_raw_ptr_buffer_load_lds(rs_in, (lds_ptr)(a + 8 * i * RP), 16, (int)a_off[i], soff_a, 0, 0);
#pragma unroll
        for (int j = 0; j < BR; ++j) {
            const unsigned wo = wrow[j];
            __builtin_amdgcn_raw_ptr_buffer_load_lds(rs_w, (lds_ptr)(b + 8 * j * RP), 16, (int)wo, soff_b, 0, 0);
        }
        ++ld_kt;
        c0 += BK;
        if (c0 >= p.Cin) {
            c0 = 0;
            if (++kw == p.KW) { kw = 0; ++kh; }
            tap_dirty = true;
        }
    };

    typedef const __attribute__((address_space(3))) f32x4* lds_frag_ptr;
    lds_frag_ptr pa[4], pb[4];
#pragma unroll
    for (int g = 0; g < 4; ++g) {
        const int goff = ((2 * g + khalf) ^ ((frag_row >> 1) & 7)) * 4;
        pa[g] = (lds_frag_ptr)(ring + frag_row * RP + goff);
        pb[g] = (lds_frag_ptr)(ring + WM * RP + frag_row * RP + goff);
    }
    f32x16 acc[TM][TN];
#pragma unroll
    for (int i = 0; i < TM; ++i)
#pragma unroll
        for (int j = 0; j < TN; ++j)
#pragma unroll
            for (int r = 0; r < 16; ++r) acc[i][j][r] = 0.f;
    constexpr bool DUAL = TM * TN == 1;
    f32x16 acc_odd;
#pragma unroll
    for (int r = 0; r < 16; ++r) acc_odd[r] = 0.f;

    auto compute = [&](auto S) __attribute__((always_inline)) {
        constexpr int ST = decltype(S)::value;
#pragma unroll
        for (int g = 0; g < 4; ++g) {
            f32x4 fa[TM], fb[TN];
#pragma unroll
            for (int i = 0; i < TM; ++i) fa[i] = pa[g][(ST * STAGE + i * 32 * RP) / 4];
#pragma unroll
            for (int j = 0; j < TN; ++j) fb[j] = pb[g][(ST * STAGE + j * 32 * RP) / 4];
#pragma unroll
            for (int s4 = 0; s4 < 4; ++s4) {
                if constexpr (DUAL) {
                    if (s4 & 1) acc_odd = __builtin_amdgcn_mfma_f32_32x32x2f32(fa[0][s4], fb[0][s4], acc_odd, 0, 0, 0);
                    else acc[0][0] = __builtin_amdgcn_mfma_f32_32x32x2f32(fa[0][s4], fb[0][s4], acc[0][0], 0, 0, 0);
                } else {
#pragma unroll
                    for (int i = 0; i < TM; ++i)
#pragma unroll
                        for (int j = 0; j < TN; ++j)
                            acc[i][j] = __builtin_amdgcn_mfma_f32_32x32x2f32(fa[i][s4], fb[j][s4], acc[i][j], 0, 0, 0);
                }
            }
        }
    };

    constexpr int WAIT = waitcnt_vm((AR + BR) * D) & ~(15 << 8);
#pragma unroll
    for (int d = 0; d < D; ++d) dma_next(d);
#ifdef YM_TRACE
    if (p.trace) { __builtin_amdgcn_s_waitcnt(waitcnt_vm((AR + BR) * (D - 1))); YM_STAMP(1); }
#endif
#ifdef YM_TRACE
    const int abl = p.bnb_relu;
#endif
    auto tile_step = [&](auto S) __attribute__((always_inline)) {
        constexpr int ST = decltype(S)::value;
        __builtin_amdgcn_sched_barrier(0);
#ifdef YM_TRACE
        if (abl >= 1 && abl <= 3) {
            if (abl == 1) {
                dma_next((ST + D) % NS);
                __builtin_amdgcn_s_waitcnt(WAIT);
            } else if (abl == 2) {
                compute(S);
            } else {
                const f32x4 ra = {1.f, 2.f, 3.f, 4.f}, rb = {.5f, .25f, .125f, 1.f};
#pragma unroll
                for (int g = 0; g < 4; ++g)
#pragma unroll
                    for (int s4 = 0; s4 < 4; ++s4) {
                        if constexpr (DUAL) {
                            if (s4 & 1) acc_odd = __builtin_amdgcn_mfma_f32_32x32x2f32(ra[s4], rb[s4], acc_odd, 0, 0, 0);
                            else acc[0][0] = __builtin_amdgcn_mfma_f32_32x32x2f32(ra[s4], rb[s4], acc[0][0], 0, 0, 0);
                        } else {
#pragma unroll
                            for (int i = 0; i < TM; ++i)
#pragma unroll
                                for (int j = 0; j < TN; ++j)
                                    acc[i][j] = __builtin_amdgcn_mfma_f32_32x32x2f32(ra[s4], rb[s4], acc[i][j], 0, 0, 0);
                        }
                    }
            }
        } else
#endif
        {
            dma_next((ST + D) % NS);
            __builtin_amdgcn_s_waitcnt(WAIT);
            compute(S);
        }
    };
    int t = 0;
    for (; t + NS <= nt; t += NS) static_for<0, NS>([&](auto S) __attribute__((always_inline)) { tile_step(S); });
    static_for<0, NS - 1>([&](auto S) __attribute__((always_inline)) { if (t + decltype(S)::value < nt) tile_step(S); });
    if constexpr (DUAL) acc[0][0] += acc_odd;
    YM_STAMP(2);
    asm volatile("s_waitcnt vmcnt(0) lgkmcnt(0)" ::: "memory");
    __syncthreads();
    if constexpr (TAIL) {
        if (in_tail) {
            constexpr int CP = WN + 4;
            float* mine = smem + (size_t)wave * WM * CP;
#pragma unroll
            for (int r = 0; r < 16; ++r) mine[(4 * khalf + (r & 3) + 8 * (r >> 2)) * CP + frag_row] = acc[0][0][r];
            __syncthreads();
            const int lt = threadIdx.x, col4 = lt & 7, row = lt >> 3;
            const int n = n0 + col4 * 4, m = m0 + row;
            f32x4 v = *reinterpret_cast<const f32x4*>(smem + row * CP + col4 * 4);
#pragma unroll
            for (int w2 = 1; w2 < KW; ++w2) v += *reinterpret_cast<const f32x4*>(smem + (size_t)w2 * WM * CP + row * CP + col4 * 4);
            const __amdgpu_buffer_rsrc_t rs_ws = __builtin_amdgcn_make_buffer_rsrc((void*)p.ws, 0, p.ws_bytes, 0x00020000);
            const unsigned sb = WM * WN * 4;
            const unsigned ws0 = (unsigned)(tile - p.main_tiles) * (unsigned)tsplit * sb + (unsigned)(row * WN + col4 * 4) * 4;
            buf_st16_sc1(rs_ws, ws0 + (unsigned)tslice * sb, v);
            asm volatile("s_waitcnt vmcnt(0)" ::: "memory");
            __syncthreads();
            int* s_last = reinterpret_cast<int*>(smem);
            if (lt == 0) {
                int* cnt = p.counters + tile;
                const int old = __hip_atomic_fetch_add(cnt, 1, __ATOMIC_RELAXED, __HIP_MEMORY_SCOPE_AGENT);
                *s_last = old == tsplit - 1;
                if (old == tsplit - 1) __hip_atomic_store(cnt, 0, __ATOMIC_RELAXED, __HIP_MEMORY_SCOPE_AGENT);
            }
            __syncthreads();
            if (*s_last && m < p.M && n < p.Cout) {
                f32x4 part[8];
#pragma unroll
                for (int s2 = 0; s2 < 8; ++s2) part[s2] = buf_ld16_sc1(rs_ws, s2 < tsplit ? ws0 + (unsigned)s2 * sb : OOB);
                f32x4 sum = part[0];
#pragma unroll
                for (int s2 = 1; s2 < 8; ++s2) if (s2 < tsplit) sum += part[s2];
                f32x4 sc = {1.f, 1.f, 1.f, 1.f}, sh = {0.f, 0.f, 0.f, 0.f};
                if (p.scale) sc = *reinterpret_cast<const f32x4*>(p.scale + n);
                if (p.shift) sh = *reinterpret_cast<const f32x4*>(p.shift + n);
                sum = __builtin_elementwise_fma(sum, sc, sh);
                if (p.residual) sum += *reinterpret_cast<const f32x4*>(p.residual + (size_t)m * p.Cout + n);
                const int act = p.seg[0].act;
#pragma unroll
                for (int e = 0; e < 4; ++e) sum[e] = ym_apply_act(sum[e], act);
                *reinterpret_cast<f32x4*>(p.seg[0].out + (size_t)m * p.Cout + n) = sum;
            }
            YM_STAMP(3);
            return;
        }
    }
    wave_tile_finish<TM, TN, KW, WPB>(p, smem, acc, wave, lane, tile_ok, tile_local, kslice, m0, n0);
    YM_STAMP(3);
}

template <int TM, int TN, int KW, int WPB>
int launch(ConvP p, hipStream_t st) {
    constexpr int TPB = WPB / KW;
    p.tiles_m = ym_cdiv(p.M, 32 * TM);
    p.tiles_n = ym_cdiv(p.Cout, 32 * TN);
    p.ksplit = 1;
    const int grid = ym_cdiv(p.tiles_m * p.tiles_n, TPB);
    const size_t lds = (size_t)WPB * 32 * TM * (32 * TN + 4) * sizeof(float);
    static YmLdsAttr attr = {};
    if (int rc = ym_ensure_dyn_lds(attr, reinterpret_cast<const void*>(conv_wave_f32<TM, TN, KW, WPB>), lds, "conv_wave_f32")) return rc;
    hipLaunchKernelGGL((conv_wave_f32<TM, TN, KW, WPB>), dim3(grid), dim3(WPB * 64), lds, st, p);
    return ym_check_launch("conv_wave_f32");
}

template <int TM, int TN>
int dispatch_kw(const ConvP& p, int kwaves, hipStream_t st) {
    switch (kwaves) {
        case 1: return launch<TM, TN, 1, 4>(p, st);
        case 2: return launch<TM, TN, 2, 4>(p, st);
        case 4: return launch<TM, TN, 4, 4>(p, st);
        case 8:
            if constexpr (TM * TN < 4) return launch<TM, TN, 8, 8>(p, st);
            [[fallthrough]];
        default: ym_set_error("conv(wave): unsupported kwaves %d for a %dx%d wave tile", kwaves, 32 * TM, 32 * TN); return YM_EINVAL;
    }
}

template <int TM, int TN, int KW, int NS, int WPB>
int launch_dma(ConvP p, hipStream_t st) {
    constexpr int TPB = WPB / KW;
    p.tiles_m = ym_cdiv(p.M, 32 * TM);
    p.tiles_n = ym_cdiv(p.Cout, 32 * TN);
    p.fd_tiles_n = FastDiv::make((unsigned)p.tiles_n);
    ym_set_tile_order(p, 0, true);
    p.ksplit = 1;
    int grid = ym_cdiv(p.tiles_m * p.tiles_n, TPB);
    if (TM * TN == 1 && KW == 4 && WPB == 4) {
        p.main_blocks = p.main_tiles;
        grid = p.main_tiles + (p.tiles_m * p.tiles_n - p.main_tiles) * p.tail_split;
    }
    const size_t lds = (size_t)WPB * NS * (32 * TM + 32 * TN) * 32 * sizeof(float);
    static YmLdsAttr attr = {};
    if (int rc = ym_ensure_dyn_lds(attr, reinterpret_cast<const void*>(conv_wdma_f32<TM, TN, KW, NS, WPB>), lds, "conv_wdma_f32")) return rc;
    hipLaunchKernelGGL((conv_wdma_f32<TM, TN, KW, NS, WPB>), dim3(grid), dim3(WPB * 64), lds, st, p);
    return ym_check_launch("conv_wdma_f32");
}

template <int TM, int TN>
int dispatch_dma(const ConvP& p, int kwaves, int ns, int wpb, hipStream_t st) {
    if (wpb <= 0) wpb = 4;
#define YM_DMA_CASE(KW_, NS_, WPB_) if (kwaves == KW_ && ns == NS_ && wpb == WPB_) return launch_dma<TM, TN, KW_, NS_, WPB_>(p, st)
    YM_DMA_CASE(1, 2, 4); YM_DMA_CASE(1, 3, 4); YM_DMA_CASE(2, 2, 4); YM_DMA_CASE(2, 3, 4); YM_DMA_CASE(4, 2, 4); YM_DMA_CASE(4, 3, 4);
    YM_DMA_CASE(1, 2, 1); YM_DMA_CASE(1, 3, 1); YM_DMA_CASE(1, 2, 2); YM_DMA_CASE(1, 3, 2); YM_DMA_CASE(2, 2, 2); YM_DMA_CASE(2, 3, 2);
    if constexpr (TM * TN == 1) { YM_DMA_CASE(1, 4, 4); YM_DMA_CASE(2, 4, 4); YM_DMA_CASE(4, 4, 4); YM_DMA_CASE(1, 4, 1); YM_DMA_CASE(1, 4, 2); }
#undef YM_DMA_CASE
    ym_set_error("conv(wave, DMA ring): kwaves %d, ring of %d, %d waves per workgroup is not built for a %dx%d wave tile", kwaves, ns, wpb, 32 * TM, 32 * TN);
    return YM_EINVAL;
}

}

int ym_launch_conv_wave(const ConvP& p, int tm, int tn, int kwaves, int ring, int wpb, hipStream_t st) {
    if (ring > 0) {
        if (tm == 32 && tn == 32) return dispatch_dma<1, 1>(p, kwaves, ring, wpb, st);
        if (tm == 64 && tn == 32) return dispatch_dma<2, 1>(p, kwaves, ring, wpb, st);
        if (tm == 32 && tn == 64) return dispatch_dma<1, 2>(p, kwaves, ring, wpb, st);
        ym_set_error("conv(wave, DMA ring): tile must be 32x32, 64x32 or 32x64, got %dx%d", tm, tn);
        return YM_EINVAL;
    }
    if (tm == 32 && tn == 32) return dispatch_kw<1, 1>(p, kwaves, st);
    if (tm == 64 && tn == 32) return dispatch_kw<2, 1>(p, kwaves, st);
    if (tm == 32 && tn == 64) return dispatch_kw<1, 2>(p, kwaves, st);
    if (tm == 64 && tn == 64) return dispatch_kw<2, 2>(p, kwaves, st);
    ym_set_error("conv(wave): tile must be 32/64 x 32/64, got %dx%d", tm, tn);
    return YM_EINVAL;
}
```

### yolact_minimal_amd/engine.py

```python
import json
import os
import sys

import torch
import torch.nn as nn

from . import conv_launch, hip, plan_transfer
from .conv_plan import ConvPlan
from .hip import ACT_NONE, ACT_RELU, ACT_TANH, ACT_GELU


def _round_up(x, m):
    return (x + m - 1) // m * m


TUNED_PATH = os.environ.get('YM_TUNED_PATH', os.path.join(os.path.dirname(os.path.abspath(__file__)), 'tuned_gfx950.json'))
_tuned = None


def conv_mma():
    return int(os.environ.get('YM_CONV_MMA', '0') or 0)


def no_tuned():
    return os.environ.get('YM_NO_TUNED', '0') == '1'


def autotune_on():
    return os.environ.get('YM_AUTOTUNE', '0') == '1'


def user_cache_path():
    return os.environ.get('YM_TUNED_CACHE') or os.path.join(os.path.expanduser('~'), '.cache', 'yolact_minimal_amd', 'tuned_gfx950_user.json')


def tuned_table():
    global _tuned
    if _tuned is None:
        _tuned = {}
        if os.path.exists(TUNED_PATH) and not no_tuned():
            with open(TUNED_PATH) as f:
                _tuned = json.load(f)
            if autotune_on() and os.path.exists(user_cache_path()):
                try:
                    with open(user_cache_path()) as f:
                        _tuned.update({k: v for k, v in json.load(f).items() if isinstance(v, list)})
                except (OSError, ValueError) as e:
                    print(f'yolact_minimal_amd: ignoring {user_cache_path()}: {e}', file=sys.stderr)
    return _tuned


def _store_user_rows(rows):
    path = user_cache_path()
    os.makedirs(os.path.dirname(path), exist_ok=True)
    cur = {}
    if os.path.exists(path):
        try:
            with open(path) as f:
                cur = json.load(f)
        except (OSError, ValueError):
            cur = {}
    cur.update(rows)
    tmp = f'{path}.{os.getpid()}.tmp'
    with open(tmp, 'w') as f:
        json.dump(cur, f, indent=0, sort_keys=True)
    os.replace(tmp, path)


def record_rows(rows):
    tuned_table().update(rows)
    plan_transfer._index_cache.clear()
    if autotune_on():
        try:
            _store_user_rows(rows)
        except OSError as e:
            print(f'yolact_minimal_amd: could not write {user_cache_path()}: {e}', file=sys.stderr)


_build_mode = ['latency']


def _entry(sig, M=0, N=0, nkt=0, nseg=1, with_source=False):
    hit, src = conv_launch.entry(tuned_table(), sig, (M, N, nkt, nseg), _build_mode[0])
    return (hit, src) if with_source else hit


class _LinearAsConv:

    def __init__(self, lin):
        self.lin = lin
        self.in_channels, self.out_channels = lin.in_features, lin.out_features
        self.kernel_size, self.stride, self.padding = (1, 1), (1, 1), (0, 0)

    @property
    def weight(self):
        return self.lin.weight.reshape(self.out_channels, self.in_channels, 1, 1)

    @property
    def bias(self):
        return self.lin.bias


class _Conv:

    def __init__(self, name, convs, bn=None, act=ACT_NONE, stem=False):
        self.name = name
        self.convs = convs if isinstance(convs, (list, tuple)) else [convs]
        self.bn = bn
        self.act = act
        self.stem = stem
        c0 = self.convs[0]
        self.cin = c0.in_channels
        self.kh, self.kw = c0.kernel_size
        self.stride = c0.stride[0]
        self.pad = c0.padding[0]
        self.cout = sum(c.out_channels for c in self.convs)
        self.cin_pad = 4 if stem else self.cin
        self.k_pad = _round_up(self.kh * self.kw * self.cin_pad, 32)
        self.weight = self.scale = self.shift = None
        self.desc = None
        self.plan = ConvPlan()
        self.mma = 0
        self._hit = None
        self._shape = (0, 0, 0, 1)
        self.plan_source = 'heuristic'

    def refresh(self):
        packed = [hip.pack_conv_weight(c.weight.detach().float(), self.cin_pad, self.k_pad) for c in self.convs]
        self.weight = packed[0] if len(packed) == 1 else torch.cat(packed, 0).contiguous()
        if self.bn is not None:
            bn = self.bn
            self.scale, self.shift = hip.fold_bn(bn.weight.detach().float().contiguous(),
                                                 bn.bias.detach().float().contiguous(),
                                                 bn.running_mean.float().contiguous(),
                                                 bn.running_var.float().contiguous(), float(bn.eps))
        else:
            self.scale = None
            biases = [c.bias for c in self.convs]
            if all(b is None for b in biases):
                self.shift = None
            else:
                self.shift = torch.cat([b.detach().float() for b in biases]).contiguous()
        if self.desc is not None:
            self._bind_params()

    def _bind_params(self):
        d = self.desc
        d.weight = self.weight.data_ptr()
        d.scale = self.scale.data_ptr() if self.scale is not None else None
        d.shift = self.shift.data_ptr() if self.shift is not None else None

    def bind(self, x, segs, residual=None):
        b, h, w, cin = x.shape
        assert cin == self.cin_pad, (self.name, cin, self.cin_pad)
        ho = (h + 2 * self.pad - self.kh) // self.stride + 1
        wo = (w + 2 * self.pad - self.kw) // self.stride + 1
        d = self.desc = conv_launch.conv_desc(b, h, w, cin, self.cout, self.kh, self.kw, self.stride, self.pad, ho, wo, self.k_pad, segs)
        d.inp = x.data_ptr()
        d.residual = residual.data_ptr() if residual is not None else None
        self._bind_params()
        self.out_hw = (ho, wo)
        self.flops = 2.0 * b * ho * wo * self.cout * self.kh * self.kw * self.cin
        self.sig = plan_transfer.forward_key(b * ho * wo, self.cout, cin, self.kh, self.stride, len(segs), residual is not None)
        self._shape = (b * ho * wo, self.cout, self.k_pad // 32, len(segs))
        self._resolve(conv_mma())
        return ho, wo

    def _resolve(self, mma, bound=None, pyramid=False):
        d = self.desc
        self.plan, self.mma, self.plan_source, self._hit = conv_launch.infer_plan(
            tuned_table(), self.sig, self._shape, _build_mode[0], mma, not self.stem and d.Cin % 32 == 0 and d.nlevels == 0, self.plan,
            no_tuned(), pyramid, bound)
        self.plan.apply(d)
        d.mma = self.mma

    def apply_mma(self, mma):
        self._resolve(mma, (self._hit, self.plan_source))


def _bind_pyramid(layer, pyr, batch, shapes, segs):
    rows, cin = pyr.shape
    assert cin == layer.cin_pad and layer.stride == 1 and layer.pad == layer.kh // 2 and len(shapes) <= 5
    assert rows == sum(batch * h * w for h, w in shapes)
    d = layer.desc = conv_launch.conv_desc(batch, shapes[0][0], shapes[0][1], cin, layer.cout, layer.kh, layer.kw, 1, layer.pad,
                                           shapes[0][0], shapes[0][1], layer.k_pad, segs, levels=shapes)
    d.inp = pyr.data_ptr()
    layer._bind_params()
    layer.out_hw = shapes[0]
    layer.flops = 2.0 * rows * layer.cout * layer.kh * layer.kw * layer.cin
    layer.sig = plan_transfer.forward_key(rows, layer.cout, cin, layer.kh, 1, len(segs), levels=len(shapes))
    layer._shape = (rows, layer.cout, layer.k_pad // 32, len(segs))
    layer._resolve(0, pyramid=True)


class InferEngine:
    def __init__(self, net, batch, height, width, device, use_graph=None, mode='latency'):
        self.net = net
        self.mode = mode
        self.device = device
        self.B, self.H, self.W = batch, height, width
        self.num_classes = net.cfg.num_classes
        self.coef_dim = net.coef_dim
        self.na = len(net.cfg.aspect_ratios)
        if use_graph is None:
            use_graph = os.environ.get('YM_GRAPH', '1') != '0'
        self.use_graph = use_graph
        self.graph = None
        self.ops = []
        self.op_stream = {}
        self.op_deps = {}
        self._producers = {}
        self._cur_stream = 0
        self._side_streams = {}
        self._events = {}
        self.use_branches = os.environ.get('YM_BRANCHES', '0') == '1'
        self.convs = []
        self.fused_stem = None
        self._img = None
        self._weights_epoch = -1
        self._bufs = []
        hip.lib()
        prev, _build_mode[0] = _build_mode[0], mode
        try:
            with torch.cuda.device(device):
                self._build()
                if autotune_on() and not no_tuned():
                    self._autotune_missing()
        finally:
            _build_mode[0] = prev

    def _autotune_missing(self):
        have = {c.sig for c in self.convs if c.plan_source == 'table'}
        todo = {c.sig for c in self.convs} - have
        if not todo:
            return
        rows = self.autotune(iters=10, skip=have)
        for c in self.convs:
            if c.sig in rows:
                c.plan_source, c._hit = 'autotuned', ConvPlan.from_row(rows[c.sig])
        record_rows(rows)

    def _buf(self, *shape):
        t = torch.empty(*shape, device=self.device, dtype=torch.float32)
        self._bufs.append(t)
        return t

    def _add_op(self, kind, arg, inputs, outputs):
        idx = len(self.ops)
        self.ops.append((kind, arg))
        sid = self._cur_stream if self.use_branches else 0
        self.op_stream[idx] = sid
        deps = []
        for t in inputs:
            if t is None:
                continue
            for j in self._producers.get(t.data_ptr(), ()):
                if self.op_stream[j] != sid and j not in deps:
                    deps.append(j)
        if deps:
            self.op_deps[idx] = deps
        for t in outputs:
            self._producers.setdefault(t.data_ptr(), []).append(idx)
        return idx

    def _conv(self, layer, x, out=None, residual=None, segs=None, seg_outputs=None):
        b, h, w, _ = x.shape
        ho = (h + 2 * layer.pad - layer.kh) // layer.stride + 1
        wo = (w + 2 * layer.pad - layer.kw) // layer.stride + 1
        if segs is None:
            if out is None:
                out = self._buf(b, ho, wo, layer.cout)
            segs = [(0, layer.cout, out.data_ptr(), ho * wo * layer.cout, layer.cout, layer.act)]
        layer.refresh()
        layer.bind(x, segs, residual)
        self.convs.append(layer)
        self._add_op('conv', layer, [x, residual], seg_outputs if seg_outputs is not None else [out])
        return out

    def _build_swin(self):
        net, B = self.net, self.B
        bb = net.backbone
        ws = bb.window_size
        assert self.H % 4 == 0 and self.W % 4 == 0
        pe = bb.patch_embed
        x = self._conv(_Conv('backbone.patch_embed.proj', pe.proj, act=ACT_NONE, stem=True), self.x_in)
        self._add_op('layernorm', (x, pe.norm, x), [x], [x])
        feats = []
        for li, layer in enumerate(bb.layers):
            _, h, w, c = x.shape
            heads = bb.heads[li]
            for bi, blk in enumerate(layer.blocks):
                p = f'backbone.layers.{li}.blocks.{bi}'
                n1 = self._buf(B, h, w, c)
                self._add_op('layernorm', (x, blk.norm1, n1), [x], [n1])
                qkv = self._conv(_Conv(p + '.attn.qkv', _LinearAsConv(blk.attn.qkv)), n1)
                att = self._buf(B, h, w, c)
                self._add_op('attn', (qkv, blk.attn, att, (B, h, w, c, heads, ws, blk.shift_size)), [qkv], [att])
                x = self._conv(_Conv(p + '.attn.proj', _LinearAsConv(blk.attn.proj)), att, residual=x)
                n2 = self._buf(B, h, w, c)
                self._add_op('layernorm', (x, blk.norm2, n2), [x], [n2])
                hid = self._conv(_Conv(p + '.mlp.fc1', _LinearAsConv(blk.mlp.fc1), act=ACT_GELU), n2)
                x = self._conv(_Conv(p + '.mlp.fc2', _LinearAsConv(blk.mlp.fc2)), hid, residual=x)
            if li in bb.out_norm_indices:
                f = self._buf(B, h, w, c)
                self._add_op('layernorm', (x, getattr(bb, f'norm{li}'), f), [x], [f])
                feats.append(f)
            if layer.downsample is not None:
                ho, wo = (h + 1) // 2, (w + 1) // 2
                merged = self._buf(B, ho, wo, 4 * c)
                self._add_op('merge_ln', (x, layer.downsample.norm, merged), [x], [merged])
                x = self._conv(_Conv(f'backbone.layers.{li}.downsample.reduction', _LinearAsConv(layer.downsample.reduction)), merged)
        return feats

    def _build(self):
        net, B, H, W = self.net, self.B, self.H, self.W
        bb = net.backbone
        self.x_in = self._buf(B, H, W, 4)
        self.static_img = None
        if hasattr(bb, 'patch_embed'):
            c3, c4, c5 = self._build_swin()
        else:
            c3, c4, c5 = self._build_resnet()
        self._build_neck_and_heads(c3, c4, c5)

    def _build_resnet(self):
        net, B, H, W = self.net, self.B, self.H, self.W
        bb = net.backbone

        stem = _Conv('backbone.conv1', bb.conv1, bb.bn1, ACT_RELU, stem=True)
        conv1 = bb.conv1
        fusable = (conv1.out_channels == 64 and conv1.in_channels == 3 and tuple(conv1.kernel_size) == (7, 7) and
                   tuple(conv1.stride) == (2, 2) and tuple(conv1.padding) == (3, 3))
        if fusable and os.environ.get('YM_FUSED_STEM', '1') != '0':
            stem.refresh()
            ho, wo = (H + 6 - 7) // 2 + 1, (W + 6 - 7) // 2 + 1
            hp, wp = (ho + 2 - 3) // 2 + 1, (wo + 2 - 3) // 2 + 1
            stem.flops = 2.0 * B * ho * wo * stem.cout * stem.kh * stem.kw * stem.cin
            self.fused_stem = stem
            pooled = self._buf(B, hp, wp, 64)
            self._add_op('stem_pool', (stem, pooled), [], [pooled])
            x = pooled
        else:
            x = self._conv(stem, self.x_in)
            hp, wp = (x.shape[1] + 2 - 3) // 2 + 1, (x.shape[2] + 2 - 3) // 2 + 1
            pooled = self._buf(B, hp, wp, 64)
            self._add_op('maxpool', (x, pooled), [x], [pooled])
            x = pooled

        stage_outs = []
        for li, stage in enumerate(bb.layers):
            for bi, blk in enumerate(stage):
                p = f'backbone.layers.{li}.{bi}'
                y = self._conv(_Conv(p + '.conv1', blk.conv1, blk.bn1, ACT_RELU), x)
                y = self._conv(_Conv(p + '.conv2', blk.conv2, blk.bn2, ACT_RELU), y)
                if blk.downsample is not None:
                    skip = self._conv(_Conv(p + '.downsample', blk.downsample[0], blk.downsample[1], ACT_NONE), x)
                else:
                    skip = x
                x = self._conv(_Conv(p + '.conv3', blk.conv3, blk.bn3, ACT_RELU), y, residual=skip)
            stage_outs.append(x)
        return stage_outs[1:4]

    def _build_neck_and_heads(self, c3, c4, c5):
        net, B = self.net, self.B
        fpn = net.fpn
        p5_1 = self._conv(_Conv('fpn.lat_layers.2', fpn.lat_layers[2]), c5)
        u5 = self._buf(B, p5_1.shape[1] * 2, p5_1.shape[2] * 2, 256)
        self._add_op('bilinear', (p5_1, u5, False), [p5_1], [u5])
        assert u5.shape[1:3] == c4.shape[1:3], 'img_size must be divisible by 32 (reference config.py:75)'
        p4_1 = self._conv(_Conv('fpn.lat_layers.1', fpn.lat_layers[1]), c4, residual=u5)
        u4 = self._buf(B, p4_1.shape[1] * 2, p4_1.shape[2] * 2, 256)
        self._add_op('bilinear', (p4_1, u4, False), [p4_1], [u4])
        p3_1 = self._conv(_Conv('fpn.lat_layers.0', fpn.lat_layers[0]), c3, residual=u4)
        pyr_env = os.environ.get('YM_PYRAMID_HEAD', 'auto')
        pyramid = pyr_env == '1' or (pyr_env == 'auto' and B <= 2)
        h5, w5 = p5_1.shape[1:3]
        shapes = [tuple(p3_1.shape[1:3]), tuple(p4_1.shape[1:3]), (h5, w5), ((h5 + 1) // 2, (w5 + 1) // 2),
                  (((h5 + 1) // 2 + 1) // 2, ((w5 + 1) // 2 + 1) // 2)]
        rows = [B * h * w for h, w in shapes]
        pyr = self._buf(sum(rows), 256)
        views, r0 = [], 0
        for (h, w), n in zip(shapes, rows):
            views.append(pyr[r0:r0 + n].view(B, h, w, 256))
            r0 += n
        self._cur_stream = 1
        p5 = self._conv(_Conv('fpn.pred_layers.2', fpn.pred_layers[2][0], act=ACT_RELU), p5_1, out=views[2])
        p6 = self._conv(_Conv('fpn.downsample_layers.0', fpn.downsample_layers[0][0], act=ACT_RELU), p5, out=views[3])
        p7 = self._conv(_Conv('fpn.downsample_layers.1', fpn.downsample_layers[1][0], act=ACT_RELU), p6, out=views[4])
        self._cur_stream = 2
        p4 = self._conv(_Conv('fpn.pred_layers.1', fpn.pred_layers[1][0], act=ACT_RELU), p4_1, out=views[1])
        self._cur_stream = 0
        p3 = self._conv(_Conv('fpn.pred_layers.0', fpn.pred_layers[0][0], act=ACT_RELU), p3_1, out=views[0])
        levels = [p3, p4, p5, p6, p7]
        assert [tuple(lv.shape[1:3]) for lv in levels] == shapes
        level_stream = [3, 2, 1, 1, 1]

        pn = net.proto_net
        y = p3
        for i in (0, 2, 4):
            y = self._conv(_Conv(f'proto_net.proto1.{i}', pn.proto1[i], act=ACT_RELU), y)
        up = self._buf(B, y.shape[1] * 2, y.shape[2] * 2, 256)
        self._add_op('bilinear', (y, up, True), [y], [up])
        y = self._conv(_Conv('proto_net.proto2.0', pn.proto2[0], act=ACT_RELU), up)
        self.proto_out = self._conv(_Conv('proto_net.proto2.2', pn.proto2[2], act=ACT_RELU), y)

        hd = net.prediction_layers
        nc, cd, na = self.num_classes, self.coef_dim, self.na
        n_total = sum(lv.shape[1] * lv.shape[2] * na for lv in levels)
        assert n_total * 4 == len(net.anchors) or not isinstance(net.anchors, list), 'anchor count mismatch'
        self.n_anchors = n_total
        self.class_logits = self._buf(B, n_total, nc)
        self.class_pred = self._buf(B, n_total, nc)
        self.box_pred = self._buf(B, n_total, 4)
        self.coef_pred = self._buf(B, n_total, cd)
        c_conf, c_box, c_coef = na * nc, na * 4, na * cd
        if pyramid:
            self._cur_stream = 0
            up = _Conv('prediction_layers.upfeature@P3-7', hd.upfeature[0], act=ACT_RELU)
            xh = self._buf(sum(rows), 256)
            up.refresh()
            _bind_pyramid(up, pyr, B, shapes, [(0, 256, xh.data_ptr(), 0, 256, ACT_RELU)])
            self.convs.append(up)
            self._add_op('conv', up, levels, [xh])
            fused = _Conv('prediction_layers.conf|bbox|coef@P3-7', [hd.conf_layer, hd.bbox_layer, hd.coef_layer[0]])
            segs = [(0, c_conf, self.class_logits.data_ptr(), n_total * nc, c_conf, ACT_NONE),
                    (c_conf, c_conf + c_box, self.box_pred.data_ptr(), n_total * 4, c_box, ACT_NONE),
                    (c_conf + c_box, c_conf + c_box + c_coef, self.coef_pred.data_ptr(), n_total * cd, c_coef, ACT_TANH)]
            fused.refresh()
            _bind_pyramid(fused, xh, B, shapes, segs)
            self.convs.append(fused)
            self._add_op('conv', fused, [xh], [self.class_logits, self.box_pred, self.coef_pred])
        off = 0
        for li, lv in enumerate(levels if not pyramid else []):
            self._cur_stream = level_stream[li]
            xh = self._conv(_Conv(f'prediction_layers.upfeature@P{li + 3}', hd.upfeature[0], act=ACT_RELU), lv)
            fused = _Conv(f'prediction_layers.conf|bbox|coef@P{li + 3}', [hd.conf_layer, hd.bbox_layer, hd.coef_layer[0]])
            es = 4
            segs = [
                (0, c_conf, self.class_logits.data_ptr() + off * nc * es, n_total * nc, c_conf, ACT_NONE),
                (c_conf, c_conf + c_box, self.box_pred.data_ptr() + off * 4 * es, n_total * 4, c_box, ACT_NONE),
                (c_conf + c_box, c_conf + c_box + c_coef, self.coef_pred.data_ptr() + off * cd * es, n_total * cd,
                 c_coef, ACT_TANH),
            ]
            self._conv(fused, xh, segs=segs, seg_outputs=[self.class_logits, self.box_pred, self.coef_pred])
            off += lv.shape[1] * lv.shape[2] * na
        self._cur_stream = 0
        self._add_op('softmax', (self.class_logits, self.class_pred), [self.class_logits], [self.class_pred])

        self._alloc_workspaces()
        self.total_flops = sum(c.flops for c in self.convs) + (self.fused_stem.flops if self.fused_stem is not None else 0.0)
        self._weights_epoch = self.net._weights_epoch

    def _alloc_workspaces(self):
        sids = {self.op_stream.get(i, 0) for i, (kind, _) in enumerate(self.ops) if kind == 'conv'} | {0}
        fused = os.environ.get('YM_FUSED_SPLITK', '1') != '0'
        oldc = getattr(self, 'counters', {})
        self.counters = {sid: oldc[sid] if sid in oldc else torch.zeros(hip.TILE_COUNTERS, device=self.device, dtype=torch.int32)
                         for sid in sids}
        need = {sid: 256 for sid in sids}
        for i, (kind, arg) in enumerate(self.ops):
            if kind == 'conv':
                sid = self.op_stream.get(i, 0)
                arg.desc.tile_counters = self.counters[sid].data_ptr() if fused else None
                if not fused:
                    arg.desc.tail_tiles, arg.desc.tail_ksplit = 0, 0
                nb = hip.conv_workspace_bytes(arg.desc)
                need[sid] = max(need[sid], nb)
        need[0] = max(need.values())
        old = getattr(self, 'workspaces', {})
        self.workspaces = {sid: (old[sid] if sid in old and old[sid].numel() >= nb else
                                 torch.empty(nb, device=self.device, dtype=torch.uint8)) for sid, nb in need.items()}
        self.workspace = self.workspaces[0]

    def refresh_weights(self):
        for c in self.convs:
            c.refresh()
        if self.fused_stem is not None:
            self.fused_stem.refresh()
        self._weights_epoch = self.net._weights_epoch
        self.graph = None

    def retune(self):
        for c in self.convs:
            c.plan.apply(c.desc)
            c.desc.mma = c.mma
        self._alloc_workspaces()
        self.graph = None

    def set_mma(self, mma):
        prev, _build_mode[0] = _build_mode[0], self.mode
        try:
            for c in self.convs:
                c.apply_mma(mma)
        finally:
            _build_mode[0] = prev
        self.retune()

    def autotune(self, iters=10, verbose=False, mma=0, concurrent=False, skip=(), cus=256):
        results = {}
        self.autotune_detail = {}
        big_ws = torch.empty(1 << 28, device=self.device, dtype=torch.uint8)
        ev0, ev1 = torch.cuda.Event(enable_timing=True), torch.cuda.Event(enable_timing=True)
        ncopy = int(concurrent) if concurrent else 1
        if ncopy == 1 and concurrent:
            ncopy = 2
        if concurrent:
            from .pipeline import _stream_set
            sides = _stream_set(self.device, ncopy - 1)
            big_ws2 = [torch.empty(1 << 27, device=self.device, dtype=torch.uint8) for _ in sides]
            counters2 = [torch.zeros(hip.TILE_COUNTERS, device=self.device, dtype=torch.int32) for _ in sides]
            main = torch.cuda.current_stream(self.device)

        def launch(d, d2):
            hip.conv2d_fwd(d, big_ws)
            if concurrent:
                for i, side in enumerate(sides):
                    with torch.cuda.stream(side):
                        hip.conv2d_fwd(d2[i], big_ws2[i])

        def time_cfg(c, plan):
            d = c.desc
            plan.apply(d)
            d.mma = mma if (split_ok(c) and not plan.wave) else 0
            need = hip.conv_workspace_bytes(d)
            if need > big_ws.numel():
                return None
            d2 = None
            if concurrent:
                if need > big_ws2[0].numel():
                    return None
                d2 = [type(d).from_buffer_copy(d) for _ in sides]
                for i, dd in enumerate(d2):
                    if d.tile_counters:
                        dd.tile_counters = counters2[i].data_ptr()
            try:
                for _ in range(2):
                    launch(d, d2)
            except RuntimeError:
                return None
            best = 1e30
            for _ in range(3):
                torch.cuda.synchronize()
                ev0.record()
                for _ in range(iters):
                    launch(d, d2)
                if concurrent:
                    for side in sides:
                        main.wait_stream(side)
                ev1.record()
                torch.cuda.synchronize()
                best = min(best, ev0.elapsed_time(ev1) / iters * 1e3)
            return best

        def split_ok(c):
            return mma in (3, 6) and not c.stem and c.desc.Cin % 32 == 0 and c.desc.nlevels == 0

        seen = {}
        for c in self.convs:
            if mma and not split_ok(c):
                continue
            if c.sig + (f'_mma{mma}' if mma else '') in skip:
                continue
            if c.sig in seen:
                c.plan = seen[c.sig]
                c.mma = mma if (mma and not c.plan.wave) else 0
                continue
            d = c.desc
            M, nkt = d.B * d.Ho * d.Wo, d.k_pad // 32
            if d.nlevels:
                M = sum(d.B * d.level_h[l] * d.level_w[l] for l in range(d.nlevels))
            base = time_cfg(c, ConvPlan())
            cands, wave_cands = [], []
            tiles = [(128, 64)] if c.stem else [(128, 128), (128, 64), (64, 128), (64, 64)]
            for tm, tn in tiles:
                wgs = -(-M // tm) * -(-d.Cout // tn)
                for ks in (1, 2, 3, 4, 6, 8, 12, 16, 24):
                    if ks > 1 and (wgs >= 1024 or ks * 2 > nkt or wgs * ks > 8192):
                        continue
                    cands.append(ConvPlan(tm, tn, ks, 0, 2))
                    if (tm, tn) != (128, 128) and nkt // ks >= 3:
                        cands.append(ConvPlan(tm, tn, ks, 0, 3))
                    if not c.stem:
                        cands.append(ConvPlan(tm, tn, ks, 0, 22))
                        if nkt // ks >= 3:
                            cands.append(ConvPlan(tm, tn, ks, 0, 23))
                        if (tm, tn) == (64, 64) and nkt // ks >= 4:
                            cands.append(ConvPlan(tm, tn, ks, 0, 24))
                        if (tm, tn) == (64, 64) and nkt // ks >= 2:
                            cands.append(ConvPlan(tm, tn, ks, 0, 33))
                            cands.append(ConvPlan(tm, tn, ks, 0, 34))
                        if (tm, tn) == (64, 64) and d.nseg == 1 and d.tile_counters and c.act in (ACT_NONE, ACT_RELU):
                            cands.append(ConvPlan(tm, tn, ks, 0, 43))
                            cands.append(ConvPlan(tm, tn, ks, 0, 46))
                if not c.stem and d.nseg == 1 and d.tile_counters and cus < wgs <= hip.TILE_COUNTERS:
                    for r in sorted({wgs % cus, wgs % (2 * cus)} - {0}):
                        for ts in (2, 3, 4, 6, 8):
                            if ts * 2 > nkt or r * ts > 2048:
                                continue
                            for stg in ((2, 3, 22, 23) + ((33, 34) if (tm, tn) == (64, 64) else ()) if (tm, tn) != (128, 128) and nkt // ts >= 3 else (2, 22)):
                                cands.append(ConvPlan(tm, tn, 1, 0, stg, r, ts))
            if not c.stem:
                for tm, tn in ((32, 32), (64, 32), (32, 64), (64, 64)):
                    waves = -(-M // tm) * -(-d.Cout // tn)
                    for kwv in (1, 2, 4, 8):
                        if kwv > 1 and (waves >= 4096 or kwv > nkt):
                            continue
                        if kwv == 8 and tm * tn == 4096:
                            continue
                        if waves * kwv > 65536:
                            continue
                        cands.append(ConvPlan(tm, tn, 1, kwv))
                if d.Cin % 32 == 0 and d.nlevels == 0:
                    for tm, tn in ((32, 32), (64, 32), (32, 64)):
                        for kwv in (1, 2, 4):
                            if kwv <= nkt:
                                wave_cands.append(ConvPlan(tm, tn, 1, kwv, 22))
                                wave_cands += [ConvPlan(tm, tn, 1, kwv, 22, grid_wgs=wpb) for wpb in (1, 2) if wpb >= kwv and kwv < 4]
                    tiles32 = -(-M // 32) * -(-d.Cout // 32)
                    if cus < tiles32 <= hip.TILE_COUNTERS and d.nseg == 1 and d.tile_counters:
                        wave_cands += [ConvPlan(32, 32, 1, 4, 22, tiles32 % cus or cus, ts) for ts in (4, 6, 8) if ts * 2 <= nkt]
            if mma:
                cands = sorted({p._replace(stages=st) for p in cands for st in ((0, 3) if not p.wave else (0,))})
            best, p = base, ConvPlan()
            for cand in cands + ([] if mma else wave_cands):
                t = time_cfg(c, cand)
                if t is not None and t < best * 0.98:
                    best, p = t, cand
            c.plan = seen[c.sig] = p
            c.mma = mma if (mma and not p.wave) else 0
            results[c.sig + (f'_mma{mma}' if mma else '')] = p.to_row()
            self.autotune_detail[c.sig + (f'_mma{mma}' if mma else '')] = (round(best, 2), round(base, 2))
            if verbose:
                print(f'{c.sig:44s} default {base:8.1f} us -> {p.to_row()} {best:8.1f} us', flush=True)
        del big_ws
        self.retune()
        return results

    def _launch_one(self, kind, arg, ws):
        if kind == 'conv':
            hip.conv2d_fwd(arg.desc, ws)
        elif kind == 'maxpool':
            hip.maxpool3x3s2(arg[0], arg[1])
        elif kind == 'stem_pool':
            hip.stem_conv_bn_relu_maxpool(self._img, arg[0].weight, arg[0].scale, arg[0].shift, arg[1])
        elif kind == 'bilinear':
            hip.bilinear2x(arg[0], arg[1], arg[2])
        elif kind == 'softmax':
            hip.softmax_rows(arg[0], arg[1])
        elif kind == 'layernorm':
            hip.layernorm(arg[0], arg[1].weight.detach(), arg[1].bias.detach(), arg[1].eps, arg[2])
        elif kind == 'merge_ln':
            hip.patch_merge_layernorm(arg[0], arg[1].weight.detach(), arg[1].bias.detach(), arg[1].eps, arg[2])
        elif kind == 'attn':
            qkv, attn, out, (b, h, w, c, heads, win, shift) = arg
            hip.swin_window_attention(qkv, attn.qkv.bias.detach(), attn.relative_position_bias_table.detach(), b, h, w, c,
                                      heads, win, shift, out)

    def _launch_all(self, img):
        if self.fused_stem is None:
            hip.nchw_to_nhwc4(img, self.x_in)
        self._img = img
        main = torch.cuda.current_stream()
        needs_event = {j for deps in self.op_deps.values() for j in deps}
        used = set()
        for i, (kind, arg) in enumerate(self.ops):
            sid = self.op_stream.get(i, 0)
            if sid == 0:
                st = main
            else:
                st = self._side_streams.get(sid)
                if st is None:
                    st = self._side_streams[sid] = torch.cuda.Stream(device=self.device)
                used.add(sid)
            for j in self.op_deps.get(i, ()):
                st.wait_event(self._events[j])
            if sid == 0:
                self._launch_one(kind, arg, self.workspaces[0])
            else:
                with torch.cuda.stream(st):
                    self._launch_one(kind, arg, self.workspaces[sid])
            if i in needs_event:
                ev = self._events.get(i)
                if ev is None:
                    ev = self._events[i] = torch.cuda.Event()
                ev.record(st)
        for sid in used:
            main.wait_stream(self._side_streams[sid])

    def run(self, img):
        if img.dtype != torch.float32 or not img.is_contiguous():
            img = img.float().contiguous()
        if tuple(img.shape) != (self.B, 3, self.H, self.W):
            raise RuntimeError(f'engine built for {(self.B, 3, self.H, self.W)}, got {tuple(img.shape)}')
        if self._weights_epoch != self.net._weights_epoch:
            self.refresh_weights()
        if not self.use_graph:
            self._launch_all(img)
            return
        if self.graph is None:
            self.static_img = torch.empty_like(img)
            self.static_img.copy_(img)
            torch.cuda.synchronize()
            side = torch.cuda.Stream()
            side.wait_stream(torch.cuda.current_stream())
            with torch.cuda.stream(side):
                self._launch_all(self.static_img)
            torch.cuda.current_stream().wait_stream(side)
            torch.cuda.synchronize()
            try:
                g = torch.cuda.CUDAGraph()
                with torch.cuda.graph(g, capture_error_mode='thread_local'):
                    self._launch_all(self.static_img)
                self.graph = g
            except Exception as exc:
                import warnings
                warnings.warn(f'hipGraph capture failed ({exc!r}); replaying the plan eagerly')
                self.use_graph = False
                torch.cuda.synchronize()
                self._launch_all(img)
                return
        self.static_img.copy_(img)
        self.graph.replay()

    def outputs(self):
        return self.class_pred, self.box_pred, self.coef_pred, self.proto_out

    def forward(self, img):
        self.run(img)
        return tuple(t.clone() for t in self.outputs())
```

### yolact_minimal_amd/hip.py

```python
import ctypes
import os

import torch

_PKG = os.path.dirname(os.path.abspath(__file__))
LIB_PATH = os.environ.get('YM_LIB_PATH') or os.path.join(_PKG, 'libyolact_hip.so')

ACT_NONE, ACT_RELU, ACT_TANH, ACT_GELU = 0, 1, 2, 3
DRAW_HIDE_MASK, DRAW_HIDE_BBOX, DRAW_HIDE_SCORE, DRAW_REAL_TIME = 1, 2, 4, 8
DRAW_FONT_ADVANCE, DRAW_FONT_HEIGHT, DRAW_NAME_STRIDE, DRAW_LABEL_MAX, DRAW_MAX_DET = 12, 14, 40, 44, 512
EVAL_MAX_DET, EVAL_MAX_THRESHOLDS, EVAL_AP_ROWS_PER_PASS = 1024, 16, 1024
COCO_MAX_GT, COCO_AREAS, COCO_WORDS_PER_ROW, COCO_ROWS_PER_PASS = 512, 4, 8, 1024

ABI_SYMBOLS = (
    'ym_abi_version', 'ym_last_error', 'ym_nchw_to_nhwc4', 'ym_pack_conv_weight', 'ym_fold_bn',
    'ym_sizeof_conv_desc', 'ym_conv2d_workspace_bytes', 'ym_conv2d_tile_counters', 'ym_conv2d_fwd', 'ym_maxpool3x3s2_fwd', 'ym_stem_conv_bn_relu_maxpool', 'ym_bilinear2x_fwd',
    'ym_softmax_rows', 'ym_nms_workspace_bytes', 'ym_detect_fast_nms', 'ym_detect_greedy_nms',
    'ym_greedy_nms_workspace_bytes', 'ym_greedy_nms', 'ym_mask_assemble', 'ym_mask_resize_binarize',
    'ym_boxes_to_pixels', 'ym_expf_cr', 'ym_nms_batch_workspace_bytes', 'ym_detect_fast_nms_batch', 'ym_after_nms_batch_workspace_bytes',
    'ym_after_nms_batch', 'ym_head_grad_gather', 'ym_scatter3',
    'ym_greedy_nms_batch_workspace_bytes', 'ym_detect_greedy_nms_batch',
    'ym_pack_conv_weight_dgrad', 'ym_pack_conv_weights_batch', 'ym_conv2d_wgrad_workspace_bytes', 'ym_conv2d_wgrad', 'ym_conv2d_wgrad_slabs', 'ym_wgrad_reduce_batch', 'ym_bn_train_fwd',
    'ym_val_preprocess', 'ym_layernorm', 'ym_patch_merge_layernorm', 'ym_swin_window_attention',
    'ym_mask_loss_workspace_bytes', 'ym_mask_loss_fwd_bwd', 'ym_mask_loss_batch_workspace_bytes', 'ym_mask_loss_batch',
    'ym_mask_iou_workspace_bytes', 'ym_mask_iou', 'ym_box_iou', 'ym_match_detections', 'ym_rle_encode', 'ym_ann_to_mask_workspace_bytes', 'ym_poly_to_mask', 'ym_runs_to_mask', 'ym_train_aug_image', 'ym_train_aug_masks',
    'ym_layernorm_bwd_workspace_bytes', 'ym_layernorm_bwd', 'ym_patch_merge_layernorm_bwd', 'ym_gelu_fwd', 'ym_gelu_bwd',
    'ym_swin_window_attention_bwd', 'ym_adamw_step', 'ym_drop_path_add', 'ym_drop_path_bwd', 'ym_select_positives',
    'ym_match_anchors', 'ym_match_anchors_batch', 'ym_loss_workspace_bytes', 'ym_class_box_loss', 'ym_semantic_loss',
    'ym_semantic_loss_batch',
    'ym_draw_workspace_bytes', 'ym_draw_detections_batch', 'ym_draw_cutout_objects',
    'ym_after_nms_batch_packed', 'ym_pack_masks', 'ym_unpack_masks', 'ym_mask_iou_packed_workspace_bytes', 'ym_mask_iou_packed',
    'ym_rle_encode_packed', 'ym_draw_detections_batch_packed', 'ym_draw_cutout_objects_packed',
    'ym_bn_train_bwd_workspace_bytes', 'ym_bn_train_bwd', 'ym_bn_train_bwd_apply', 'ym_act_bias_bwd', 'ym_conv2d_fuses_bn_stats', 'ym_bn_train_fwd_stats', 'ym_maxpool3x3s2_bwd', 'ym_maxpool3x3s2_fwd_idx', 'ym_maxpool3x3s2_bwd_idx', 'ym_bilinear2x_bwd', 'ym_sgd_step',
    'ym_conv2d_bn_partial_rows', 'ym_conv2d_effective_plan', 'ym_bn_partials_finish', 'ym_unordered_sum_launches', 'ym_bn_train_fwd_workspace_bytes',
    'ym_eval_match_log', 'ym_eval_ap_workspace_bytes', 'ym_eval_ap',
    'ym_coco_iou_box', 'ym_coco_iou_mask_packed', 'ym_coco_match_log', 'ym_coco_accumulate_workspace_bytes', 'ym_coco_accumulate',
    'ym_after_nms_ragged_workspace_bytes', 'ym_after_nms_ragged', 'ym_after_nms_ragged_packed',
)


class ConvSeg(ctypes.Structure):
    _fields_ = [('n_begin', ctypes.c_int), ('n_end', ctypes.c_int), ('out', ctypes.c_void_p),
                ('batch_stride', ctypes.c_int64), ('pitch', ctypes.c_int32), ('act', ctypes.c_int32)]


class ConvDesc(ctypes.Structure):
    _fields_ = [('inp', ctypes.c_void_p), ('weight', ctypes.c_void_p), ('scale', ctypes.c_void_p),
                ('shift', ctypes.c_void_p), ('residual', ctypes.c_void_p),
                ('B', ctypes.c_int32), ('H', ctypes.c_int32), ('W', ctypes.c_int32), ('Cin', ctypes.c_int32),
                ('Cout', ctypes.c_int32), ('KH', ctypes.c_int32), ('KW', ctypes.c_int32),
                ('stride', ctypes.c_int32), ('pad', ctypes.c_int32), ('Ho', ctypes.c_int32),
                ('Wo', ctypes.c_int32), ('k_pad', ctypes.c_int32), ('nseg', ctypes.c_int32),
                ('seg', ConvSeg * 3), ('tile_m', ctypes.c_int32), ('tile_n', ctypes.c_int32),
                ('ksplit', ctypes.c_int32), ('kwaves', ctypes.c_int32), ('transposed', ctypes.c_int32),
                ('stages', ctypes.c_int32), ('bn_sum', ctypes.c_void_p), ('bn_sumsq', ctypes.c_void_p),
                ('tile_counters', ctypes.c_void_p), ('nlevels', ctypes.c_int32), ('level_h', ctypes.c_int32 * 5),
                ('level_w', ctypes.c_int32 * 5), ('tail_tiles', ctypes.c_int32), ('tail_ksplit', ctypes.c_int32), ('mma', ctypes.c_int32),
                ('bnb_relu', ctypes.c_int32), ('bnb_y', ctypes.c_void_p), ('bnb_out', ctypes.c_void_p),
                ('bnb_mean', ctypes.c_void_p), ('bnb_invstd', ctypes.c_void_p), ('bnb_gamma', ctypes.c_void_p),
                ('bnb_beta', ctypes.c_void_p), ('grid_wgs', ctypes.c_int32),
                ('bn_ordered', ctypes.c_int32)]


class WgradDesc(ctypes.Structure):
    _fields_ = [('x', ctypes.c_void_p), ('dy', ctypes.c_void_p), ('dw', ctypes.c_void_p),
                ('B', ctypes.c_int32), ('H', ctypes.c_int32), ('W', ctypes.c_int32), ('Cin', ctypes.c_int32),
                ('Cin_real', ctypes.c_int32), ('Cout', ctypes.c_int32), ('Cout_real', ctypes.c_int32),
                ('KH', ctypes.c_int32), ('KW', ctypes.c_int32), ('stride', ctypes.c_int32), ('pad', ctypes.c_int32),
                ('Ho', ctypes.c_int32), ('Wo', ctypes.c_int32), ('msplit', ctypes.c_int32), ('accumulate', ctypes.c_int32),
                ('row_end', ctypes.c_int32 * 2), ('dw_seg', ctypes.c_void_p * 2), ('lds_buffers', ctypes.c_int32)]


class WgradReduceItem(ctypes.Structure):
    _fields_ = [('slabs', ctypes.c_void_p), ('dw', ctypes.c_void_p), ('first_block', ctypes.c_uint32), ('blocks', ctypes.c_uint32),
                ('plan', ctypes.c_uint32 * 14)]


class AugPlanC(ctypes.Structure):
    _fields_ = [(n, ctypes.c_int32) for n in ('H', 'W', 'mirror', 'cx', 'cy', 'cw', 'ch', 'q', 'px', 'py', 'r', 'S', 'final_mode',
                                              'fx', 'fy', 'has_brightness', 'has_contrast')] + \
               [(n, ctypes.c_float) for n in ('brightness', 'contrast', 'saturation', 'hue')] + \
               [('mean', ctypes.c_float * 3), ('std', ctypes.c_float * 3)]


class PackItem(ctypes.Structure):
    _fields_ = [('src', ctypes.c_void_p), ('dst', ctypes.c_void_p)] + \
               [(n, ctypes.c_int32) for n in ('cout', 'cin', 'kh', 'kw', 'pad_a', 'pad_b', 'rows', 'kind')] + \
               [('first_chunk', ctypes.c_uint32), ('reserved', ctypes.c_uint32)]


class MaskLossItem(ctypes.Structure):
    _fields_ = [('proto', ctypes.c_void_p), ('coef_full', ctypes.c_void_p), ('anchor_box', ctypes.c_void_p),
                ('anchor_gt', ctypes.c_void_p), ('gt_masks_ds', ctypes.c_void_p), ('anchor_idx', ctypes.c_void_p),
                ('n', ctypes.c_int32), ('wscale', ctypes.c_float), ('n_dev', ctypes.c_void_p), ('dproto', ctypes.c_void_p),
                ('dcoef_full', ctypes.c_void_p)]


class NmsCfg(ctypes.Structure):
    _fields_ = [('num_anchors', ctypes.c_int32), ('num_classes', ctypes.c_int32), ('coef_dim', ctypes.c_int32),
                ('top_k', ctypes.c_int32), ('max_det', ctypes.c_int32), ('score_thre', ctypes.c_float),
                ('iou_thre', ctypes.c_float), ('img_size', ctypes.c_float)]


class RaggedImage(ctypes.Structure):
    _fields_ = [('img_h', ctypes.c_int32), ('img_w', ctypes.c_int32), ('offset', ctypes.c_int64)]


RAGGED_MAX_IMAGES = 32
RAGGED_ALIGN_BYTES = 256

_lib = None


def lib():
    global _lib
    if _lib is None:
        if not os.path.exists(LIB_PATH):
            raise RuntimeError(
                f'{LIB_PATH} is missing: build it with `python -c "import __graft_entry__ as g; g.build()"` '
                f'(or `make -C yolact_minimal_amd/csrc`). yolact_minimal_amd has no non-HIP fallback.')
        L = ctypes.CDLL(LIB_PATH)
        vp, i32, i64, f32, sz = ctypes.c_void_p, ctypes.c_int, ctypes.c_int64, ctypes.c_float, ctypes.c_size_t
        L.ym_abi_version.restype = ctypes.c_int
        L.ym_last_error.restype = ctypes.c_char_p
        L.ym_nchw_to_nhwc4.argtypes = [vp, vp, i32, i32, i32, i32, vp]
        L.ym_pack_conv_weight.argtypes = [vp, vp, i32, i32, i32, i32, i32, i32, vp]
        L.ym_fold_bn.argtypes = [vp, vp, vp, vp, f32, vp, vp, i32, vp]
        L.ym_sizeof_conv_desc.restype = sz
        if L.ym_sizeof_conv_desc() != ctypes.sizeof(ConvDesc):
            raise RuntimeError(f'libyolact_hip.so was built from a different ym_conv_desc ({L.ym_sizeof_conv_desc()} B) than '
                               f'yolact_minimal_amd/hip.py mirrors ({ctypes.sizeof(ConvDesc)} B): rebuild the library')
        L.ym_conv2d_workspace_bytes.argtypes = [ctypes.POINTER(ConvDesc)]
        L.ym_conv2d_workspace_bytes.restype = sz
        L.ym_conv2d_fwd.argtypes = [ctypes.POINTER(ConvDesc), vp, sz, vp]
        L.ym_conv2d_tile_counters.argtypes = [ctypes.POINTER(ConvDesc)]
        L.ym_maxpool3x3s2_fwd.argtypes = [vp, vp, i32, i32, i32, i32, vp]
        L.ym_stem_conv_bn_relu_maxpool.argtypes = [vp, vp, vp, vp, vp, i32, i32, i32, i32, vp]
        L.ym_bilinear2x_fwd.argtypes = [vp, vp, i32, i32, i32, i32, i32, vp]
        L.ym_softmax_rows.argtypes = [vp, vp, i64, i32, vp]
        L.ym_nms_workspace_bytes.argtypes = [ctypes.POINTER(NmsCfg)]
        L.ym_nms_workspace_bytes.restype = sz
        nms_args = [vp, vp, vp, vp, ctypes.POINTER(NmsCfg), vp, vp, vp, vp, vp, vp, sz, vp]
        L.ym_detect_fast_nms.argtypes = nms_args
        L.ym_detect_greedy_nms.argtypes = nms_args
        L.ym_greedy_nms_workspace_bytes.argtypes = [i32]
        L.ym_greedy_nms_workspace_bytes.restype = sz
        L.ym_greedy_nms.argtypes = [vp, i32, f32, vp, vp, vp, sz, vp]
        L.ym_mask_assemble.argtypes = [vp, vp, vp, i32, i32, i32, i32, i32, vp, vp]
        L.ym_mask_resize_binarize.argtypes = [vp, i32, i32, i32, i32, i32, vp, vp]
        L.ym_boxes_to_pixels.argtypes = [vp, vp, i32, f32, vp]
        L.ym_expf_cr.argtypes = [vp, vp, i64, vp]
        L.ym_nms_batch_workspace_bytes.argtypes = [ctypes.POINTER(NmsCfg), i32]
        L.ym_nms_batch_workspace_bytes.restype = sz
        L.ym_detect_fast_nms_batch.argtypes = [vp, vp, vp, vp, ctypes.POINTER(NmsCfg), i32, vp, vp, vp, vp, vp, vp, sz, vp]
        L.ym_greedy_nms_batch_workspace_bytes.argtypes = L.ym_nms_batch_workspace_bytes.argtypes
        L.ym_greedy_nms_batch_workspace_bytes.restype = sz
        L.ym_detect_greedy_nms_batch.argtypes = L.ym_detect_fast_nms_batch.argtypes
        L.ym_after_nms_batch_workspace_bytes.argtypes = [i32, i32, i32, i32, i32]
        L.ym_after_nms_batch_workspace_bytes.restype = sz
        L.ym_after_nms_batch.argtypes = [vp, vp, vp, vp, i32, i32, i32, i32, i32, i32, i32, i32, vp, vp, vp, sz, vp]
        L.ym_head_grad_gather.argtypes = [vp, vp, vp, vp, i32, i32, i32, i32, i32, i32, vp, vp, i32, vp, vp, vp]
        L.ym_scatter3.argtypes = [vp, vp, i32, vp, i32, vp, i32, i32, vp]
        L.ym_pack_conv_weight_dgrad.argtypes = [vp, vp, i32, i32, i32, i32, i32, vp]
        L.ym_pack_conv_weights_batch.argtypes = [vp, i32, i32, vp]
        L.ym_conv2d_wgrad_workspace_bytes.argtypes = [ctypes.POINTER(WgradDesc)]
        L.ym_conv2d_wgrad_workspace_bytes.restype = sz
        L.ym_conv2d_wgrad.argtypes = [ctypes.POINTER(WgradDesc), vp, sz, vp]
        L.ym_conv2d_wgrad_slabs.argtypes = [ctypes.POINTER(WgradDesc), vp, sz, ctypes.POINTER(WgradReduceItem), vp]
        L.ym_wgrad_reduce_batch.argtypes = [vp, i32, ctypes.c_uint32, vp]
        L.ym_bn_train_fwd.argtypes = [vp, i64, i32, vp, vp, f32, f32, vp, vp, vp, i32, vp, vp, vp, vp, sz, vp]
        L.ym_val_preprocess.argtypes = [vp, i32, i32, i32, i32, ctypes.POINTER(ctypes.c_float), ctypes.POINTER(ctypes.c_float), vp, vp]
        L.ym_layernorm.argtypes = [vp, vp, vp, f32, vp, i64, i32, vp]
        L.ym_patch_merge_layernorm.argtypes = [vp, i32, i32, i32, i32, vp, vp, f32, vp, vp]
        L.ym_swin_window_attention.argtypes = [vp, vp, vp, i32, i32, i32, i32, i32, i32, i32, vp, vp]
        L.ym_mask_loss_workspace_bytes.argtypes = []
        L.ym_mask_loss_workspace_bytes.restype = sz
        L.ym_mask_loss_fwd_bwd.argtypes = [vp, vp, vp, vp, vp, vp, i32, i32, i32, f32, f32, vp, vp, vp, vp, sz, vp]
        L.ym_mask_loss_batch_workspace_bytes.argtypes = [i32]
        L.ym_mask_loss_batch_workspace_bytes.restype = sz
        L.ym_mask_loss_batch.argtypes = [ctypes.POINTER(MaskLossItem), i32, i32, i32, f32, vp, vp, vp, sz, vp]
        L.ym_mask_iou_workspace_bytes.argtypes = [i32, i32, i64]
        L.ym_mask_iou_workspace_bytes.restype = sz
        L.ym_mask_iou.argtypes = [vp, i32, vp, i32, i64, vp, vp, sz, vp]
        L.ym_box_iou.argtypes = [vp, i32, vp, i32, vp, vp]
        L.ym_match_detections.argtypes = [vp, vp, vp, vp, i32, i32, vp, i32, i32, vp, vp]
        L.ym_rle_encode.argtypes = [vp, i32, i32, i32, vp, i32, vp, vp, i32, vp, vp, sz, vp]
        L.ym_ann_to_mask_workspace_bytes.argtypes = [i32, i32, i32]
        L.ym_ann_to_mask_workspace_bytes.restype = sz
        L.ym_poly_to_mask.argtypes = [vp, vp, vp, i32, i32, i32, vp, vp, sz, vp]
        L.ym_runs_to_mask.argtypes = [vp, vp, i32, i32, i32, vp, vp, sz, vp]
        L.ym_layernorm_bwd_workspace_bytes.argtypes = [i32]
        L.ym_layernorm_bwd_workspace_bytes.restype = sz
        L.ym_layernorm_bwd.argtypes = [vp, vp, vp, f32, i64, i32, vp, vp, vp, vp, sz, vp]
        L.ym_patch_merge_layernorm_bwd.argtypes = [vp, vp, i32, i32, i32, i32, vp, f32, vp, vp, vp, vp, sz, vp]
        L.ym_gelu_fwd.argtypes = [vp, vp, i64, vp]
        L.ym_gelu_bwd.argtypes = [vp, vp, vp, i64, vp]
        L.ym_swin_window_attention_bwd.argtypes = [vp, vp, vp, vp, i32, i32, i32, i32, i32, i32, i32, vp, vp, vp, vp]
        L.ym_select_positives.argtypes = [vp, vp, i32, i32, i32, vp, vp, vp]
        L.ym_drop_path_add.argtypes = [vp, vp, vp, ctypes.c_float, vp, i32, i64, vp]
        L.ym_drop_path_bwd.argtypes = [vp, vp, ctypes.c_float, vp, i32, i64, vp]
        L.ym_adamw_step.argtypes = [vp, vp, vp, vp, i64, f32, f32, f32, f32, f32, i32, vp]
        L.ym_train_aug_image.argtypes = [vp, i32, ctypes.POINTER(AugPlanC), vp, vp]
        L.ym_train_aug_masks.argtypes = [vp, i32, vp, i32, ctypes.POINTER(AugPlanC), vp, vp]
        L.ym_match_anchors.argtypes = [vp, i32, vp, i32, f32, f32, vp, vp, vp, vp, vp, sz, vp]
        L.ym_match_anchors_batch.argtypes = [vp, vp, i32, vp, i32, f32, f32, vp, vp, vp, vp, vp, sz, vp]
        L.ym_semantic_loss_batch.argtypes = [vp, i32, i32, i32, i32, vp, vp, i32, vp, f32, vp, vp, vp]
        L.ym_loss_workspace_bytes.argtypes = [i32, i32]
        L.ym_loss_workspace_bytes.restype = sz
        L.ym_class_box_loss.argtypes = [vp, vp, vp, vp, i32, i32, i32, f32, f32, i32, vp, vp, vp, vp, vp, vp, sz, vp]
        L.ym_semantic_loss.argtypes = [vp, i32, i32, i32, vp, vp, i32, i32, f32, vp, vp, vp]
        L.ym_conv2d_fuses_bn_stats.argtypes = [ctypes.POINTER(ConvDesc)]
        L.ym_conv2d_bn_partial_rows.argtypes = [ctypes.POINTER(ConvDesc)]
        L.ym_conv2d_effective_plan.argtypes = [ctypes.POINTER(ConvDesc), ctypes.POINTER(ctypes.c_int32 * 8)]
        L.ym_bn_partials_finish.argtypes = [vp, i32, i32, vp, vp]
        L.ym_unordered_sum_launches.argtypes = []
        L.ym_unordered_sum_launches.restype = ctypes.c_int64
        L.ym_bn_train_fwd_workspace_bytes.argtypes = [i64, i32]
        L.ym_bn_train_fwd_workspace_bytes.restype = sz
        L.ym_bn_train_fwd_stats.argtypes = [vp, i64, i32, vp, vp, f32, f32, vp, vp, vp, i32, vp, vp, vp, vp, vp]
        L.ym_bn_train_bwd_workspace_bytes.argtypes = [i64, i32]
        L.ym_bn_train_bwd_workspace_bytes.restype = sz
        L.ym_bn_train_bwd.argtypes = [vp, vp, vp, i64, i32, vp, vp, vp, vp, i32, vp, vp, vp, vp, vp, sz, vp]
        L.ym_bn_train_bwd_apply.argtypes = [vp, vp, vp, i64, i32, vp, vp, vp, vp, i32, vp, vp, vp, vp, vp, vp]
        L.ym_act_bias_bwd.argtypes = [vp, vp, i64, i32, i32, vp, vp, vp, sz, vp]
        L.ym_maxpool3x3s2_bwd.argtypes = [vp, vp, vp, i32, i32, i32, i32, vp]
        L.ym_maxpool3x3s2_fwd_idx.argtypes = [vp, vp, vp, i32, i32, i32, i32, vp]
        L.ym_maxpool3x3s2_bwd_idx.argtypes = [vp, vp, vp, i32, i32, i32, i32, vp]
        L.ym_bilinear2x_bwd.argtypes = [vp, vp, i32, i32, i32, i32, i32, vp]
        L.ym_sgd_step.argtypes = [vp, vp, vp, i64, f32, f32, f32, i32, vp]
        L.ym_draw_workspace_bytes.argtypes = [i32, i32]
        L.ym_draw_workspace_bytes.restype = sz
        L.ym_draw_detections_batch.argtypes = [vp, vp, vp, vp, vp, vp, i32, i32, i32, i32, vp, i32, i32, vp, i32, vp, i32, f32,
                                               ctypes.c_char_p, vp, vp, vp, sz, vp]
        L.ym_draw_cutout_objects.argtypes = [vp, vp, i32, i32, i32, vp, vp]
        L.ym_after_nms_batch_packed.argtypes = L.ym_after_nms_batch.argtypes
        L.ym_after_nms_ragged_workspace_bytes.argtypes = [ctypes.POINTER(RaggedImage), i32, i32, i32, i32]
        L.ym_after_nms_ragged_workspace_bytes.restype = sz
        L.ym_after_nms_ragged.argtypes = [vp, vp, vp, vp, i32, i32, i32, i32, i32, ctypes.POINTER(RaggedImage), i32, vp, vp, vp, sz, vp]
        L.ym_after_nms_ragged_packed.argtypes = L.ym_after_nms_ragged.argtypes
        L.ym_pack_masks.argtypes = [vp, i32, i32, i32, i32, vp, vp]
        L.ym_unpack_masks.argtypes = [vp, i32, i32, i32, vp, vp]
        L.ym_mask_iou_packed_workspace_bytes.argtypes = [i32, i32, i64]
        L.ym_mask_iou_packed_workspace_bytes.restype = sz
        L.ym_mask_iou_packed.argtypes = L.ym_mask_iou.argtypes
        L.ym_rle_encode_packed.argtypes = L.ym_rle_encode.argtypes
        L.ym_draw_detections_batch_packed.argtypes = L.ym_draw_detections_batch.argtypes
        L.ym_draw_cutout_objects_packed.argtypes = L.ym_draw_cutout_objects.argtypes
        L.ym_eval_match_log.argtypes = [vp, vp, vp, i32, vp, vp, vp, i32, vp, i32, i32, vp, vp, vp, i64, vp, vp, vp]
        L.ym_eval_ap_workspace_bytes.argtypes = [i64]
        L.ym_eval_ap_workspace_bytes.restype = sz
        L.ym_eval_ap.argtypes = [vp, vp, i64, vp, vp, i32, i32, vp, vp, vp, sz, vp]
        L.ym_coco_iou_box.argtypes = [vp, i32, vp, i32, vp, vp, vp]
        L.ym_coco_iou_mask_packed.argtypes = [vp, i32, vp, i32, i64, vp, vp, vp, vp]
        L.ym_coco_match_log.argtypes = [vp, vp, vp, i32, vp, vp, vp, vp, vp, vp, vp, vp, i32, vp, i32, vp, i32, i32, vp, vp, vp, vp, i64, vp, vp, vp]
        L.ym_coco_accumulate_workspace_bytes.argtypes = [i64]
        L.ym_coco_accumulate_workspace_bytes.restype = sz
        L.ym_coco_accumulate.argtypes = [vp, vp, vp, i64, vp, vp, vp, i32, vp, i32, i32, i32, ctypes.c_double, i32, vp, vp, vp, sz, vp]
        for name in ABI_SYMBOLS:
            fn = getattr(L, name)
            if name not in ('ym_last_error', 'ym_conv2d_workspace_bytes', 'ym_nms_workspace_bytes',
                            'ym_greedy_nms_workspace_bytes', 'ym_conv2d_wgrad_workspace_bytes',
                            'ym_sizeof_conv_desc', 'ym_bn_train_bwd_workspace_bytes', 'ym_mask_loss_workspace_bytes', 'ym_mask_loss_batch_workspace_bytes', 'ym_loss_workspace_bytes', 'ym_mask_iou_workspace_bytes', 'ym_layernorm_bwd_workspace_bytes',
                            'ym_ann_to_mask_workspace_bytes', 'ym_draw_workspace_bytes', 'ym_mask_iou_packed_workspace_bytes',
                            'ym_unordered_sum_launches', 'ym_bn_train_fwd_workspace_bytes', 'ym_greedy_nms_batch_workspace_bytes',
                            'ym_eval_ap_workspace_bytes', 'ym_coco_accumulate_workspace_bytes'):
                fn.restype = ctypes.c_int
        _lib = L
    return _lib


def check(rc, what):
    if rc != 0:
        raise RuntimeError(f'{what} failed (rc={rc}): {lib().ym_last_error().decode()}')


def stream_ptr():
    return ctypes.c_void_p(torch.cuda.current_stream().cuda_stream)


def ptr(t, dtype=torch.float32):
    if t is None:
        return None
    if not t.is_cuda or t.dtype != dtype or not t.is_contiguous():
        raise RuntimeError(f'expected a contiguous {dtype} CUDA tensor, got {t.dtype} {t.device} '
                           f'contiguous={t.is_contiguous()}')
    return ctypes.c_void_p(t.data_ptr())



def nchw_to_nhwc4(img, out):
    b, c, h, w = img.shape
    check(lib().ym_nchw_to_nhwc4(ptr(img), ptr(out), b, c, h, w, stream_ptr()), 'ym_nchw_to_nhwc4')


def pack_conv_weight(w_oihw, cin_pad, k_pad):
    cout, cin, kh, kw = w_oihw.shape
    out = torch.empty(cout, k_pad, device=w_oihw.device, dtype=torch.float32)
    check(lib().ym_pack_conv_weight(ptr(w_oihw.contiguous()), ptr(out), cout, cin, kh, kw, cin_pad, k_pad,
                                    stream_ptr()), 'ym_pack_conv_weight')
    return out


def fold_bn(gamma, beta, mean, var, eps):
    c = gamma.numel()
    scale, shift = torch.empty_like(gamma), torch.empty_like(gamma)
    check(lib().ym_fold_bn(ptr(gamma), ptr(beta), ptr(mean), ptr(var), eps, ptr(scale), ptr(shift), c,
                           stream_ptr()), 'ym_fold_bn')
    return scale, shift


def conv_workspace_bytes(desc):
    n = lib().ym_conv2d_workspace_bytes(ctypes.byref(desc))
    if n == 0 and (desc.ksplit > 1 or desc.tail_tiles > 0) and desc.kwaves == 0:
        err = lib().ym_last_error().decode()
        if err and 'conv' in err and desc.tail_tiles > 0:
            raise RuntimeError(f'ym_conv2d_workspace_bytes: {err}')
    return n


def conv_effective_plan(desc):
    from .conv_plan import ConvPlan
    row = (ctypes.c_int32 * 8)()
    check(lib().ym_conv2d_effective_plan(ctypes.byref(desc), ctypes.byref(row)), 'ym_conv2d_effective_plan')
    return ConvPlan(*row)


TILE_COUNTERS = 16384


def conv2d_fwd(desc, workspace=None):
    counters = desc.tile_counters
    if counters and lib().ym_conv2d_tile_counters(ctypes.byref(desc)) > TILE_COUNTERS:
        desc.tile_counters = None
    ws_ptr = ctypes.c_void_p(workspace.data_ptr()) if workspace is not None else None
    ws_bytes = workspace.numel() * workspace.element_size() if workspace is not None else 0
    try:
        check(lib().ym_conv2d_fwd(ctypes.byref(desc), ws_ptr, ws_bytes, stream_ptr()), 'ym_conv2d_fwd')
    finally:
        desc.tile_counters = counters


def stem_conv_bn_relu_maxpool(img, w_packed, scale, shift, out):
    b, c, h, w = img.shape
    if c != 3 or tuple(w_packed.shape) != (64, 224):
        raise RuntimeError(f'stem: expects a 3-channel image and a [64, 224] packed filter, got {tuple(img.shape)} / {tuple(w_packed.shape)}')
    check(lib().ym_stem_conv_bn_relu_maxpool(ptr(img), ptr(w_packed), ptr(scale), ptr(shift), ptr(out), b, h, w, w_packed.shape[1],
                                             stream_ptr()), 'ym_stem_conv_bn_relu_maxpool')


def maxpool3x3s2(x, out):
    b, h, w, c = x.shape
    check(lib().ym_maxpool3x3s2_fwd(ptr(x), ptr(out), b, h, w, c, stream_ptr()), 'ym_maxpool3x3s2_fwd')


def bilinear2x(x, out, align_corners):
    b, h, w, c = x.shape
    check(lib().ym_bilinear2x_fwd(ptr(x), ptr(out), b, h, w, c, int(bool(align_corners)), stream_ptr()),
          'ym_bilinear2x_fwd')


def softmax_rows(x, out):
    c = x.shape[-1]
    rows = x.numel() // c
    check(lib().ym_softmax_rows(ptr(x), ptr(out), rows, c, stream_ptr()), 'ym_softmax_rows')


def layernorm(x, gamma, beta, eps, out):
    c = x.shape[-1]
    check(lib().ym_layernorm(ptr(x), ptr(gamma), ptr(beta), float(eps), ptr(out), x.numel() // c, c, stream_ptr()), 'ym_layernorm')


def patch_merge_layernorm(x, gamma, beta, eps, out):
    b, h, w, c = x.shape
    check(lib().ym_patch_merge_layernorm(ptr(x), b, h, w, c, ptr(gamma), ptr(beta), float(eps), ptr(out), stream_ptr()),
          'ym_patch_merge_layernorm')


def swin_window_attention(qkv, qkv_bias, table, b, h, w, c, heads, window, shift, out):
    check(lib().ym_swin_window_attention(ptr(qkv), ptr(qkv_bias), ptr(table), b, h, w, c, heads, window, shift, ptr(out),
                                         stream_ptr()), 'ym_swin_window_attention')


def mask_assemble(proto, coefs, boxes, out, do_crop=True):
    hp, wp, k = proto.shape
    n = coefs.shape[0]
    check(lib().ym_mask_assemble(ptr(proto), ptr(coefs), ptr(boxes), n, hp, wp, k, int(do_crop), ptr(out),
                                 stream_ptr()), 'ym_mask_assemble')


def mask_resize_binarize(masks, img_h, img_w, out):
    n, hp, wp = masks.shape
    check(lib().ym_mask_resize_binarize(ptr(masks), n, hp, wp, img_h, img_w, ptr(out), stream_ptr()),
          'ym_mask_resize_binarize')


def expf_cr(x):
    y = torch.empty_like(x)
    check(lib().ym_expf_cr(ptr(x), ptr(y), x.numel(), stream_ptr()), 'ym_expf_cr')
    return y


def boxes_to_pixels(boxes_f, boxes_px, size):
    n = boxes_f.shape[0]
    check(lib().ym_boxes_to_pixels(ptr(boxes_f), ptr(boxes_px, torch.int32), n, float(size), stream_ptr()),
          'ym_boxes_to_pixels')
```

Before: 511.1 img/s.

## Pre-pack conv weights into MFMA fragment order and load them straight to registers

Adds a one-time packing kernel that rearranges each conv's packed filter into per-32-channel, per-K-tile 4 KiB blocks laid out in MFMA fragment order. The wave-DMA conv kernel, when the tile is one 32-wide column, then loads these fragments directly into VGPRs with buffer loads instead of staging the B operand through LDS. This cuts LDS footprint and LDS reads per K step and may raise occupancy. In exchange it costs extra VGPRs for the register ring and a second weight copy in memory. It is enabled by default via YM_WEIGHT_FRAGS.

```diff
diff --git a/include/yolact_hip.h b/include/yolact_hip.h
--- a/include/yolact_hip.h
+++ b/include/yolact_hip.h
@@ -70,7 +70,10 @@
     const float* bnb_mean;
     const float* bnb_invstd;
     const float* bnb_gamma;
+    union {
     const float* bnb_beta;
+    const float* weight_frags;
+    };
     int32_t grid_wgs;
     int32_t bn_ordered;
 } ym_conv_desc;
@@ -80,6 +83,9 @@
 int ym_conv2d_tile_counters(const ym_conv_desc* d);
 int ym_conv2d_fuses_bn_stats(const ym_conv_desc* d);
 int ym_conv2d_effective_plan(const ym_conv_desc* d, int32_t out[8]);
+size_t ym_conv_weight_frags_bytes(int Cout, int k_pad);
+int ym_pack_conv_weight_frags(const float* w_packed, float* frags, int Cout, int k_pad, ym_stream_t s);
+int ym_conv2d_uses_weight_frags(const ym_conv_desc* d);
 int ym_conv2d_bn_partial_rows(const ym_conv_desc* d);
 int ym_bn_partials_finish(const void* part, int rows, int C, void* sums, ym_stream_t s);
 int64_t ym_unordered_sum_launches(void);
diff --git a/yolact_minimal_amd/csrc/conv_common.h b/yolact_minimal_amd/csrc/conv_common.h
--- a/yolact_minimal_amd/csrc/conv_common.h
+++ b/yolact_minimal_amd/csrc/conv_common.h
@@ -48,6 +48,8 @@
 struct ConvP {
     const float* in;
     const float* w;
+    const float* wfrag;
+    unsigned wfrag_bytes;
     const float* scale;
     const float* shift;
     const float* residual;
@@ -203,6 +205,8 @@
 
 int ym_conv_plan(const ym_conv_desc* d, bool ws_aligned, ymk::Plan* pl);
 int ym_cu_count();
+bool ym_conv_uses_weight_frags(const ym_conv_desc* d, const ymk::Plan& pl);
+constexpr int YM_WFRAG_BLOCK_BYTES = 4096, YM_WFRAG_PAD_BLOCKS = 3;
 int ym_launch_conv_wave(const ymk::ConvP& p, int tm, int tn, int kwaves, int ring, int waves_per_block, hipStream_t st);
 int ym_launch_conv_pers(const ymk::ConvP& p, int bm, int bn, int mode, int ns, bool defer, int grid, hipStream_t st);
 size_t ym_conv_pers_lds_bytes(int bm, int bn, int ns, bool defer);
diff --git a/yolact_minimal_amd/csrc/conv_mfma.hip b/yolact_minimal_amd/csrc/conv_mfma.hip
--- a/yolact_minimal_amd/csrc/conv_mfma.hip
+++ b/yolact_minimal_amd/csrc/conv_mfma.hip
@@ -839,6 +839,11 @@
         YM_REQUIRE(ib < 0xFFFFFFF0ull && wb < 0x7FFFFFF0ull, "conv: input must be < 4 GiB and the packed weight < 2 GiB (32-bit buffer offsets)");
         p.in_bytes = (unsigned)ib; p.w_bytes = (unsigned)wb;
     }
+    p.wfrag = nullptr; p.wfrag_bytes = 0;
+    if (ym_conv_uses_weight_frags(d, pl)) {
+        p.wfrag = d->weight_frags;
+        p.wfrag_bytes = (unsigned)(((size_t)(d->Cout / 32) * pl.nkt + YM_WFRAG_PAD_BLOCKS) * YM_WFRAG_BLOCK_BYTES);
+    }
     p.nlev = d->nlevels;
     {
         int m_acc = 0, pix_acc = 0;
@@ -974,6 +979,11 @@
     return YM_OK;
 }
 
+extern "C" int ym_conv2d_uses_weight_frags(const ym_conv_desc* d) {
+    Plan pl;
+    return d && ym_conv_plan(d, true, &pl) == YM_OK && ym_conv_uses_weight_frags(d, pl) ? 1 : 0;
+}
+
 extern "C" int ym_conv2d_fwd(const ym_conv_desc* d, void* workspace, size_t workspace_bytes, ym_stream_t s) {
     Plan pl;
     if (int rc = ym_conv_plan(d, ((uintptr_t)workspace & 15) == 0, &pl)) return rc;
diff --git a/yolact_minimal_amd/csrc/conv_planner.hip b/yolact_minimal_amd/csrc/conv_planner.hip
--- a/yolact_minimal_amd/csrc/conv_planner.hip
+++ b/yolact_minimal_amd/csrc/conv_planner.hip
@@ -11,6 +11,13 @@
         cus = n;
     }
     return cus;
+}
+
+bool ym_conv_uses_weight_frags(const ym_conv_desc* d, const Plan& pl) {
+    if (d->transposed != 0 || d->bnb_y != nullptr || d->weight_frags == nullptr) return false;
+    const unsigned long long bytes = ((unsigned long long)(d->Cout / 32) * pl.nkt + YM_WFRAG_PAD_BLOCKS) * YM_WFRAG_BLOCK_BYTES;
+    return pl.family == CONV_WAVE_DMA && pl.bn == 32 && d->Cout % 32 == 0 && d->nlevels == 0 && d->mma == 0 &&
+           ((uintptr_t)d->weight_frags & 15) == 0 && bytes < 0x7FFFFFF0ull;
 }
 
 namespace {
diff --git a/yolact_minimal_amd/csrc/conv_wave.hip b/yolact_minimal_amd/csrc/conv_wave.hip
--- a/yolact_minimal_amd/csrc/conv_wave.hip
+++ b/yolact_minimal_amd/csrc/conv_wave.hip
@@ -203,17 +203,19 @@
     wave_tile_finish<TM, TN, KW, WPB>(p, smem, acc, wave, lane, tile_ok, tile_local, kslice, m0, n0);
 }
 
-template <int TM, int TN, int KW, int NS, int WPB = 4>
+template <int TM, int TN, int KW, int NS, int WPB = 4, bool WF = false>
 __global__ __launch_bounds__(WPB * 64) void conv_wdma_f32(const ConvP p) {
     static_assert(WPB % KW == 0 && WPB <= 4, "the K waves of a tile share a workgroup");
+    static_assert(!WF || TN == 1, "fragment-ordered filter images: one 32-channel tile column per wave");
     constexpr int TPB = WPB / KW;
     constexpr int WM = 32 * TM, WN = 32 * TN;
     constexpr int AR = 4 * TM, BR = 4 * TN;
     constexpr int RP = 32;
-    constexpr int STAGE = (WM + WN) * RP;
+    constexpr int STAGE = (WM + (WF ? 0 : WN)) * RP;
     constexpr int D = NS - 1;
     static_assert(NS >= 2 && NS <= 4 && (AR + BR) * D < 64, "ring depth / vmcnt field");
-    static_assert((size_t)STAGE >= (size_t)WM * (WN + 4), "the finished tile is staged in the wave's first ring stage");
+    static_assert(D <= YM_WFRAG_PAD_BLOCKS, "run-ahead of the filter image");
+    static_assert((size_t)WPB * NS * STAGE >= (size_t)WPB * WM * (WN + 4), "the finished tiles are staged where the workgroup's rings were");
     extern __shared__ __attribute__((aligned(16))) float smem[];
 
     const int lane = threadIdx.x & 63;
@@ -236,11 +238,12 @@
     if (tile_ok) ym_tile_decode(p, tile, tile_m, tile_n);
     const int m0 = tile_m * WM, n0 = tile_n * WN;
     const __amdgpu_buffer_rsrc_t rs_in = __builtin_amdgcn_make_buffer_rsrc((void*)p.in, 0, p.in_bytes, 0x00020000);
-    const __amdgpu_buffer_rsrc_t rs_w = __builtin_amdgcn_make_buffer_rsrc((void*)p.w, 0, p.w_bytes, 0x00020000);
+    const __amdgpu_buffer_rsrc_t rs_w = WF ? __builtin_amdgcn_make_buffer_rsrc((void*)p.wfrag, 0, p.wfrag_bytes, 0x00020000)
+                                           : __builtin_amdgcn_make_buffer_rsrc((void*)p.w, 0, p.w_bytes, 0x00020000);
 
     const int drow = lane >> 3;
     int a_pix[AR], a_ih0[AR], a_iw0[AR];
-    unsigned a_off[AR], wrow[BR];
+    unsigned a_off[AR], wrow[WF ? 1 : BR];
 #pragma unroll
     for (int i = 0; i < AR; ++i) {
         const int m = m0 + 8 * i + drow;
@@ -255,11 +258,15 @@
             a_ih0[i] = -(1 << 20); a_iw0[i] = -(1 << 20); a_pix[i] = 0;
         }
     }
-#pragma unroll
-    for (int j = 0; j < BR; ++j) {
-        const int n = n0 + 8 * j + drow;
-        const int c4 = (lane & 7) ^ ((4 * j + (lane >> 4)) & 7);
-        wrow[j] = (tile_ok && n < p.Cout) ? (unsigned)((n * p.Kpad + c4 * 4) * 4) : p.w_bytes;
+    if constexpr (WF) {
+        wrow[0] = (unsigned)lane * 16;
+    } else {
+#pragma unroll
+        for (int j = 0; j < BR; ++j) {
+            const int n = n0 + 8 * j + drow;
+            const int c4 = (lane & 7) ^ ((4 * j + (lane >> 4)) & 7);
+            wrow[j] = (tile_ok && n < p.Cout) ? (unsigned)((n * p.Kpad + c4 * 4) * 4) : p.w_bytes;
+        }
     }
 
     const int k_lo = in_tail ? tslice * p.tail_ktps : 0, k_hi = in_tail ? min(p.nkt, k_lo + p.tail_ktps) : p.nkt;
@@ -276,8 +283,11 @@
     bool tap_dirty = true;
     int ld_kt = kt_beg;
     float* ring = smem + (size_t)wave * NS * STAGE;
-
-    auto dma_next = [&](int stage) __attribute__((always_inline)) {
+    int wf_soff = WF ? ((n0 >> 5) * p.nkt + min(kt_beg, k_hi)) * YM_WFRAG_BLOCK_BYTES : 0;
+    f32x4 wf[WF ? NS : 1][TN][4];
+
+    auto dma_next = [&](auto SG) __attribute__((always_inline)) {
+        constexpr int stage = decltype(SG)::value;
         typedef __attribute__((address_space(3))) void* lds_ptr;
         if (tap_dirty) {
             tap_dirty = false;
@@ -290,15 +300,24 @@
             }
         }
         float* a = ring + stage * STAGE;
-        float* b = a + WM * RP;
+        [[maybe_unused]] float* b = a + WM * RP;
         const int soff_a = c0 * 4, soff_b = ld_kt * BK * 4;
 #pragma unroll
         for (int i = 0; i < AR; ++i)
             __builtin_amdgcn_raw_ptr_buffer_load_lds(rs_in, (lds_ptr)(a + 8 * i * RP), 16, (int)a_off[i], soff_a, 0, 0);
-#pragma unroll
-        for (int j = 0; j < BR; ++j) {
-            const unsigned wo = wrow[j];
-            __builtin_amdgcn_raw_ptr_buffer_load_lds(rs_w, (lds_ptr)(b + 8 * j * RP), 16, (int)wo, soff_b, 0, 0);
+        if constexpr (WF) {
+            const unsigned wo = wrow[0];
+#pragma unroll
+            for (int j = 0; j < TN; ++j)
+#pragma unroll
+                for (int g = 0; g < 4; ++g) wf[stage][j][g] = buf_ld16_s(rs_w, wo + g * 1024, wf_soff);
+            wf_soff += YM_WFRAG_BLOCK_BYTES;
+        } else {
+#pragma unroll
+            for (int j = 0; j < BR; ++j) {
+                const unsigned wo = wrow[j];
+                __builtin_amdgcn_raw_ptr_buffer_load_lds(rs_w, (lds_ptr)(b + 8 * j * RP), 16, (int)wo, soff_b, 0, 0);
+            }
         }
         ++ld_kt;
         c0 += BK;
@@ -337,7 +356,10 @@
 #pragma unroll
             for (int i = 0; i < TM; ++i) fa[i] = pa[g][(ST * STAGE + i * 32 * RP) / 4];
 #pragma unroll
-            for (int j = 0; j < TN; ++j) fb[j] = pb[g][(ST * STAGE + j * 32 * RP) / 4];
+            for (int j = 0; j < TN; ++j) {
+                if constexpr (WF) fb[j] = wf[ST][j][g];
+                else fb[j] = pb[g][(ST * STAGE + j * 32 * RP) / 4];
+            }
 #pragma unroll
             for (int s4 = 0; s4 < 4; ++s4) {
                 if constexpr (DUAL) {
@@ -355,8 +377,7 @@
     };
 
     constexpr int WAIT = waitcnt_vm((AR + BR) * D) & ~(15 << 8);
-#pragma unroll
-    for (int d = 0; d < D; ++d) dma_next(d);
+    static_for<0, D>([&](auto S) __attribute__((always_inline)) { dma_next(S); });
 #ifdef YM_TRACE
     if (p.trace) { __builtin_amdgcn_s_waitcnt(waitcnt_vm((AR + BR) * (D - 1))); YM_STAMP(1); }
 #endif
@@ -369,7 +390,7 @@
 #ifdef YM_TRACE
         if (abl >= 1 && abl <= 3) {
             if (abl == 1) {
-                dma_next((ST + D) % NS);
+                dma_next(IC<(ST + D) % NS>{});
                 __builtin_amdgcn_s_waitcnt(WAIT);
             } else if (abl == 2) {
                 compute(S);
@@ -394,7 +415,7 @@
         } else
 #endif
         {
-            dma_next((ST + D) % NS);
+            dma_next(IC<(ST + D) % NS>{});
             __builtin_amdgcn_s_waitcnt(WAIT);
             compute(S);
         }
@@ -403,6 +424,14 @@
     for (; t + NS <= nt; t += NS) static_for<0, NS>([&](auto S) __attribute__((always_inline)) { tile_step(S); });
     static_for<0, NS - 1>([&](auto S) __attribute__((always_inline)) { if (t + decltype(S)::value < nt) tile_step(S); });
     if constexpr (DUAL) acc[0][0] += acc_odd;
+    if constexpr (WF) {
+#pragma unroll
+        for (int s = 0; s < NS; ++s)
+#pragma unroll
+            for (int j = 0; j < TN; ++j)
+#pragma unroll
+                for (int g = 0; g < 4; ++g) asm volatile("" :: "v"(wf[s][j][g]));
+    }
     YM_STAMP(2);
     asm volatile("s_waitcnt vmcnt(0) lgkmcnt(0)" ::: "memory");
     __syncthreads();
@@ -484,7 +513,7 @@
     }
 }
 
-template <int TM, int TN, int KW, int NS, int WPB>
+template <int TM, int TN, int KW, int NS, int WPB, bool WF = false>
 int launch_dma(ConvP p, hipStream_t st) {
     constexpr int TPB = WPB / KW;
     p.tiles_m = ym_cdiv(p.M, 32 * TM);
@@ -497,17 +526,19 @@
         p.main_blocks = p.main_tiles;
         grid = p.main_tiles + (p.tiles_m * p.tiles_n - p.main_tiles) * p.tail_split;
     }
-    const size_t lds = (size_t)WPB * NS * (32 * TM + 32 * TN) * 32 * sizeof(float);
+    const size_t lds = (size_t)WPB * NS * (32 * TM + (WF ? 0 : 32 * TN)) * 32 * sizeof(float);
     static YmLdsAttr attr = {};
-    if (int rc = ym_ensure_dyn_lds(attr, reinterpret_cast<const void*>(conv_wdma_f32<TM, TN, KW, NS, WPB>), lds, "conv_wdma_f32")) return rc;
-    hipLaunchKernelGGL((conv_wdma_f32<TM, TN, KW, NS, WPB>), dim3(grid), dim3(WPB * 64), lds, st, p);
+    if (int rc = ym_ensure_dyn_lds(attr, reinterpret_cast<const void*>(conv_wdma_f32<TM, TN, KW, NS, WPB, WF>), lds, "conv_wdma_f32")) return rc;
+    hipLaunchKernelGGL((conv_wdma_f32<TM, TN, KW, NS, WPB, WF>), dim3(grid), dim3(WPB * 64), lds, st, p);
     return ym_check_launch("conv_wdma_f32");
 }
 
 template <int TM, int TN>
 int dispatch_dma(const ConvP& p, int kwaves, int ns, int wpb, hipStream_t st) {
     if (wpb <= 0) wpb = 4;
-#define YM_DMA_CASE(KW_, NS_, WPB_) if (kwaves == KW_ && ns == NS_ && wpb == WPB_) return launch_dma<TM, TN, KW_, NS_, WPB_>(p, st)
+#define YM_DMA_CASE(KW_, NS_, WPB_) if (kwaves == KW_ && ns == NS_ && wpb == WPB_) { \
+        if constexpr (TN == 1) { if (p.wfrag) return launch_dma<TM, TN, KW_, NS_, WPB_, true>(p, st); } \
+        return launch_dma<TM, TN, KW_, NS_, WPB_>(p, st); }
     YM_DMA_CASE(1, 2, 4); YM_DMA_CASE(1, 3, 4); YM_DMA_CASE(2, 2, 4); YM_DMA_CASE(2, 3, 4); YM_DMA_CASE(4, 2, 4); YM_DMA_CASE(4, 3, 4);
     YM_DMA_CASE(1, 2, 1); YM_DMA_CASE(1, 3, 1); YM_DMA_CASE(1, 2, 2); YM_DMA_CASE(1, 3, 2); YM_DMA_CASE(2, 2, 2); YM_DMA_CASE(2, 3, 2);
     if constexpr (TM * TN == 1) { YM_DMA_CASE(1, 4, 4); YM_DMA_CASE(2, 4, 4); YM_DMA_CASE(4, 4, 4); YM_DMA_CASE(1, 4, 1); YM_DMA_CASE(1, 4, 2); }
@@ -516,6 +547,34 @@
     return YM_EINVAL;
 }
 
+__global__ __launch_bounds__(256) void pack_weight_frags(const float* __restrict__ w, f32x4* __restrict__ frags, int nkt, int kpad, unsigned real_f4, unsigned total_f4) {
+    const unsigned i = blockIdx.x * 256u + threadIdx.x;
+    if (i >= total_f4) return;
+    f32x4 v = {0.f, 0.f, 0.f, 0.f};
+    if (i < real_f4) {
+        const unsigned blk = i >> 8, g = (i >> 6) & 3, l = i & 63;
+        const unsigned nt = blk / (unsigned)nkt, kt = blk - nt * (unsigned)nkt;
+        v = *reinterpret_cast<const f32x4*>(w + (size_t)(nt * 32 + (l & 31)) * kpad + kt * 32 + 8 * g + 4 * (l >> 5));
+    }
+    frags[i] = v;
+}
+
+}
+
+extern "C" size_t ym_conv_weight_frags_bytes(int Cout, int k_pad) {
+    if (Cout <= 0 || k_pad <= 0 || Cout % 32 || k_pad % 32) return 0;
+    return ((size_t)(Cout / 32) * (k_pad / 32) + YM_WFRAG_PAD_BLOCKS) * YM_WFRAG_BLOCK_BYTES;
+}
+
+extern "C" int ym_pack_conv_weight_frags(const float* w_packed, float* frags, int Cout, int k_pad, ym_stream_t s) {
+    YM_REQUIRE(w_packed && frags, "pack_conv_weight_frags: null pointer");
+    YM_REQUIRE(Cout > 0 && k_pad > 0 && Cout % 32 == 0 && k_pad % 32 == 0, "pack_conv_weight_frags: Cout %d and k_pad %d must be multiples of 32", Cout, k_pad);
+    YM_REQUIRE((((uintptr_t)w_packed | (uintptr_t)frags) & 15) == 0, "pack_conv_weight_frags: pointers must be 16-byte aligned");
+    const size_t total = ym_conv_weight_frags_bytes(Cout, k_pad) / 16, real = (size_t)Cout * k_pad / 4;
+    YM_REQUIRE(total < 0x7FFFFFFFull / 16, "pack_conv_weight_frags: image must be < 2 GiB");
+    hipLaunchKernelGGL(pack_weight_frags, dim3((unsigned)((total + 255) / 256)), dim3(256), 0, (hipStream_t)s, w_packed, reinterpret_cast<f32x4*>(frags),
+                       k_pad / 32, k_pad, (unsigned)real, (unsigned)total);
+    return ym_check_launch("pack_weight_frags");
 }
 
 int ym_launch_conv_wave(const ConvP& p, int tm, int tn, int kwaves, int ring, int wpb, hipStream_t st) {
diff --git a/yolact_minimal_amd/engine.py b/yolact_minimal_amd/engine.py
--- a/yolact_minimal_amd/engine.py
+++ b/yolact_minimal_amd/engine.py
@@ -20,6 +20,10 @@
 
 def conv_mma():
     return int(os.environ.get('YM_CONV_MMA', '0') or 0)
+
+
+def weight_frags_on():
+    return os.environ.get('YM_WEIGHT_FRAGS', '1') != '0'
 
 
 def no_tuned():
@@ -118,6 +122,7 @@
         self.cin_pad = 4 if stem else self.cin
         self.k_pad = _round_up(self.kh * self.kw * self.cin_pad, 32)
         self.weight = self.scale = self.shift = None
+        self.frags = None
         self.desc = None
         self.plan = ConvPlan()
         self.mma = 0
@@ -128,6 +133,7 @@
     def refresh(self):
         packed = [hip.pack_conv_weight(c.weight.detach().float(), self.cin_pad, self.k_pad) for c in self.convs]
         self.weight = packed[0] if len(packed) == 1 else torch.cat(packed, 0).contiguous()
+        self.frags = None
         if self.bn is not None:
             bn = self.bn
             self.scale, self.shift = hip.fold_bn(bn.weight.detach().float().contiguous(),
@@ -149,6 +155,17 @@
         d.weight = self.weight.data_ptr()
         d.scale = self.scale.data_ptr() if self.scale is not None else None
         d.shift = self.shift.data_ptr() if self.shift is not None else None
+        self._sync_frags()
+
+    def _sync_frags(self, plan=None):
+        d, plan = self.desc, self.plan if plan is None else plan
+        want = (weight_frags_on() and plan.wave_dma and plan.tile_n == 32 and self.cout % 32 == 0 and d.nlevels == 0
+                and self.weight is not None)
+        if not want:
+            self.frags = None
+        elif self.frags is None:
+            self.frags = hip.pack_conv_weight_frags(self.weight)
+        d.weight_frags = self.frags.data_ptr() if want else None
 
     def bind(self, x, segs, residual=None):
         b, h, w, cin = x.shape
@@ -173,6 +190,7 @@
             no_tuned(), pyramid, bound)
         self.plan.apply(d)
         d.mma = self.mma
+        self._sync_frags()
 
     def apply_mma(self, mma):
         self._resolve(mma, (self._hit, self.plan_source))
@@ -484,6 +502,7 @@
         for c in self.convs:
             c.plan.apply(c.desc)
             c.desc.mma = c.mma
+            c._sync_frags()
         self._alloc_workspaces()
         self.graph = None
 
@@ -521,6 +540,7 @@
         def time_cfg(c, plan):
             d = c.desc
             plan.apply(d)
+            c._sync_frags(plan)
             d.mma = mma if (split_ok(c) and not plan.wave) else 0
             need = hip.conv_workspace_bytes(d)
             if need > big_ws.numel():
diff --git a/yolact_minimal_amd/hip.py b/yolact_minimal_amd/hip.py
--- a/yolact_minimal_amd/hip.py
+++ b/yolact_minimal_amd/hip.py
@@ -36,6 +36,7 @@
     'ym_eval_match_log', 'ym_eval_ap_workspace_bytes', 'ym_eval_ap',
     'ym_coco_iou_box', 'ym_coco_iou_mask_packed', 'ym_coco_match_log', 'ym_coco_accumulate_workspace_bytes', 'ym_coco_accumulate',
     'ym_after_nms_ragged_workspace_bytes', 'ym_after_nms_ragged', 'ym_after_nms_ragged_packed',
+    'ym_conv_weight_frags_bytes', 'ym_pack_conv_weight_frags', 'ym_conv2d_uses_weight_frags',
 )
 
 
@@ -44,7 +45,12 @@
                 ('batch_stride', ctypes.c_int64), ('pitch', ctypes.c_int32), ('act', ctypes.c_int32)]
 
 
+class _BetaOrFrags(ctypes.Union):
+    _fields_ = [('bnb_beta', ctypes.c_void_p), ('weight_frags', ctypes.c_void_p)]
+
+
 class ConvDesc(ctypes.Structure):
+    _anonymous_ = ('_beta_or_frags',)
     _fields_ = [('inp', ctypes.c_void_p), ('weight', ctypes.c_void_p), ('scale', ctypes.c_void_p),
                 ('shift', ctypes.c_void_p), ('residual', ctypes.c_void_p),
                 ('B', ctypes.c_int32), ('H', ctypes.c_int32), ('W', ctypes.c_int32), ('Cin', ctypes.c_int32),
@@ -58,7 +64,7 @@
                 ('level_w', ctypes.c_int32 * 5), ('tail_tiles', ctypes.c_int32), ('tail_ksplit', ctypes.c_int32), ('mma', ctypes.c_int32),
                 ('bnb_relu', ctypes.c_int32), ('bnb_y', ctypes.c_void_p), ('bnb_out', ctypes.c_void_p),
                 ('bnb_mean', ctypes.c_void_p), ('bnb_invstd', ctypes.c_void_p), ('bnb_gamma', ctypes.c_void_p),
-                ('bnb_beta', ctypes.c_void_p), ('grid_wgs', ctypes.c_int32),
+                ('_beta_or_frags', _BetaOrFrags), ('grid_wgs', ctypes.c_int32),
                 ('bn_ordered', ctypes.c_int32)]
 
 
@@ -213,6 +219,10 @@
         L.ym_conv2d_bn_partial_rows.argtypes = [ctypes.POINTER(ConvDesc)]
         L.ym_conv2d_effective_plan.argtypes = [ctypes.POINTER(ConvDesc), ctypes.POINTER(ctypes.c_int32 * 8)]
         L.ym_bn_partials_finish.argtypes = [vp, i32, i32, vp, vp]
+        L.ym_conv_weight_frags_bytes.argtypes = [i32, i32]
+        L.ym_conv_weight_frags_bytes.restype = sz
+        L.ym_pack_conv_weight_frags.argtypes = [vp, vp, i32, i32, vp]
+        L.ym_conv2d_uses_weight_frags.argtypes = [ctypes.POINTER(ConvDesc)]
         L.ym_unordered_sum_launches.argtypes = []
         L.ym_unordered_sum_launches.restype = ctypes.c_int64
         L.ym_bn_train_fwd_workspace_bytes.argtypes = [i64, i32]
@@ -263,7 +273,7 @@
                             'ym_sizeof_conv_desc', 'ym_bn_train_bwd_workspace_bytes', 'ym_mask_loss_workspace_bytes', 'ym_mask_loss_batch_workspace_bytes', 'ym_loss_workspace_bytes', 'ym_mask_iou_workspace_bytes', 'ym_layernorm_bwd_workspace_bytes',
                             'ym_ann_to_mask_workspace_bytes', 'ym_draw_workspace_bytes', 'ym_mask_iou_packed_workspace_bytes',
                             'ym_unordered_sum_launches', 'ym_bn_train_fwd_workspace_bytes', 'ym_greedy_nms_batch_workspace_bytes',
-                            'ym_eval_ap_workspace_bytes', 'ym_coco_accumulate_workspace_bytes'):
+                            'ym_eval_ap_workspace_bytes', 'ym_coco_accumulate_workspace_bytes', 'ym_conv_weight_frags_bytes'):
                 fn.restype = ctypes.c_int
         _lib = L
     return _lib
@@ -323,6 +333,20 @@
     row = (ctypes.c_int32 * 8)()
     check(lib().ym_conv2d_effective_plan(ctypes.byref(desc), ctypes.byref(row)), 'ym_conv2d_effective_plan')
     return ConvPlan(*row)
+
+
+def pack_conv_weight_frags(w_packed):
+    cout, k_pad = w_packed.shape
+    nbytes = lib().ym_conv_weight_frags_bytes(cout, k_pad)
+    if nbytes == 0:
+        raise RuntimeError(f'pack_conv_weight_frags: Cout {cout} and k_pad {k_pad} must be multiples of 32')
+    out = torch.empty(nbytes // 4, device=w_packed.device, dtype=torch.float32)
+    check(lib().ym_pack_conv_weight_frags(ptr(w_packed), ptr(out), cout, k_pad, stream_ptr()), 'ym_pack_conv_weight_frags')
+    return out
+
+
+def conv_uses_weight_frags(desc):
+    return lib().ym_conv2d_uses_weight_frags(ctypes.byref(desc)) == 1
 
 
 TILE_COUNTERS = 16384
```

Result: no change. 516.0 img/s (median of 6 runs) (+0.9%).
